# tomstrident/GAN-based-Video-Style-Transfer

Measured on AMD Instinct MI355X. Metric: frames/sec: CycleGAN train step (G+D+flow-warp loss) 256x256, higher is better.
Workload: dtype fp32; 1 GPU; C2: CycleGANCon optimize_parameters, resnet_9blocks G + basic PatchGAN D, ngf=ndf=64, 256x256, B_local=4, pool_size=50, flow-warp temporal loss; global_batch=4, height=256, width=256, parallelism=dp1

## Files before the change

gan-based-video-style-transfer_amd/csrc/common.h:

```cpp
#pragma once
#include <hip/hip_runtime.h>
#include <stdint.h>
#include <stdio.h>
#include <string.h>

#include "../../include/vst_hip.h"

typedef float f32x16 __attribute__((ext_vector_type(16)));
typedef float f32x4v __attribute__((ext_vector_type(4)));

namespace vst {

void set_error(const char* fmt, ...);

inline int check_launch(const char* what) {
  hipError_t e = hipGetLastError();
  if (e != hipSuccess) {
    set_error("%s: %s", what, hipGetErrorString(e));
    return VST_EHIP;
  }
  return VST_OK;
}

#define VST_NUM_CUS 256

#define VST_REQUIRE(cond, ...)            \
  do {                                    \
    if (!(cond)) {                        \
      ::vst::set_error(__VA_ARGS__);      \
      return VST_EINVAL;                  \
    }                                     \
  } while (0)

__device__ __forceinline__ int xcd_tile(int L, int T) {
  const int x = L & 7, k = L >> 3, q = T >> 3, r = T & 7;
  return x * q + (x < r ? x : r) + k;
}

__device__ __forceinline__ int reflect_idx(int i, int n) {
  i = i < 0 ? -i : i;
  return i >= n ? 2 * n - 2 - i : i;
}

__host__ __device__ __forceinline__ int dgrad_border_rows_of(int h, int w, int H, int W, int* b0) {
  const int sw = W - 2, sh = H - 2, S4 = ((2 * sw + 2 * sh + 3) / 4) * 4;
  const bool rh = h == 1 || h == H - 2, rw = w == 1 || w == W - 2;
  if (rh && rw) {
    *b0 = S4 + 4 * ((h == 1 ? 0 : 2) + (w == 1 ? 0 : 1));
    return 3;
  }
  const int kw = w == 0 ? 0 : (w == W - 1 ? sw - 1 : w - 1);
  const int kh = h == 0 ? 0 : (h == H - 1 ? sh - 1 : h - 1);
  if (h == 1) { *b0 = kw; return 1; }
  if (h == H - 2) { *b0 = sw + kw; return 1; }
  if (w == 1) { *b0 = 2 * sw + kh; return 1; }
  if (w == W - 2) { *b0 = 2 * sw + sh + kh; return 1; }
  return 0;
}

struct BorderSlabs {
  int ks, Mb, Lt, Ll;
};

__host__ __device__ __forceinline__ int dgrad_border_slab_rows(int n, int h, int w, int H, int W, int Lt, int Ll,
                                                               int* rows) {
  if (Ll == 0) {
    int b0;
    const int nr = dgrad_border_rows_of(h, w, H, W, &b0);
    for (int r = 0; r < nr; ++r) rows[r] = n * Lt + b0 + r;
    return nr;
  }
  int nr = 0;
  if (h == 1 || h == H - 2) {
    const int base = (h == 1 ? 0 : Lt) + n * (W + 2);
    rows[nr++] = base + w + 1;
    if (w == 1) rows[nr++] = base;
    if (w == W - 2) rows[nr++] = base + W + 1;
  }
  if (w == 1) rows[nr++] = 2 * Lt + n * H + h;
  if (w == W - 2) rows[nr++] = 2 * Lt + Ll + n * H + h;
  return nr;
}

__device__ __forceinline__ float apply_act(float v, int act, float slope) {
  if (act == VST_ACT_RELU) return v > 0.f ? v : 0.f;
  if (act == VST_ACT_LRELU) return v > 0.f ? v : v * slope;
  if (act == VST_ACT_TANH) return tanhf(v);
  return v;
}

__device__ __forceinline__ float act_grad_from_out(float y, int act, float slope) {
  if (act == VST_ACT_RELU) return y > 0.f ? 1.f : 0.f;
  if (act == VST_ACT_LRELU) return y > 0.f ? 1.f : slope;
  if (act == VST_ACT_TANH) return 1.f - y * y;
  return 1.f;
}

__device__ __forceinline__ float wave_sum(float v) {
#pragma unroll
  for (int o = 32; o > 0; o >>= 1) v += __shfl_xor(v, o, 64);
  return v;
}
__device__ __forceinline__ double wave_sum_d(double v) {
#pragma unroll
  for (int o = 32; o > 0; o >>= 1) v += __shfl_xor(v, o, 64);
  return v;
}

__device__ __forceinline__ void add_f4(float4& a, const float4& b) {
  a.x += b.x; a.y += b.y; a.z += b.z; a.w += b.w;
}

inline int ceil_div(long a, long b) { return (int)((a + b - 1) / b); }

int skinny_out_launch(int mode, const float* in, const float* wp, const float* bias,
                      const float* addend, float* out, int N, int Hi, int Wi, int Cin, int Ho,
                      int Wo, int R, int S, int st, int pad, int reflect, int act, float slope,
                      hipStream_t s, int co_real = 4);
void rk_fprop_launch(const float* x, const float* wp, const float* bias, float* y, int N, int H, int W,
                     int C, int Ho, int Wo, int Cop, int R, int S, int st, int padh, int padw, int reflect,
                     int act, float slope, int kind, int math, hipStream_t s);
long rk_cp_ld(long P);
bool bf_convT_phases_ok(int C, int Cop, int math);
int bf_convT_phases_launch(const float* x, const void* const ws[4], const float* bias, float* y, int N, int H, int W,
                           int C, int Cop, int act, float slope, int math, hipStream_t s, int full = 0);
int bf_fprop_launch(const float* x, const void* wsplit, long wps, const float* bias, float* y, int N,
                    int H, int W, int C, int Ho, int Wo, int Cop, int R, int S, int st, int padh, int padw,
                    int reflect, int act, float slope, int math, int kind, hipStream_t s,
                    double* part = nullptr, float* tws = nullptr, size_t tws_floats = 0, const float* addend = nullptr,
                    int oph = 0);
bool tap64_ok(int Cx, int R, int W, int math);
int tap64_launch(const float* x, const void* wsplit, long wps, const float* bias, float* y, int N, int H, int W,
                 int pad, int reflect, int act, float slope, int math, hipStream_t s);
bool c4_direct_ok(int C, int Cop, int R, int S, int st, int Ho, int Wo, int math);
int c4_direct_launch(const float* x, const void* wsplit, long wps, const float* bias, float* y, int N, int H, int W,
                     int Ho, int Wo, int R, int S, int pad, int reflect, int act, float slope, int math, double* part,
                     hipStream_t s);
bool bf_dgrad_refl1_ok(int N, int H, int W, int Cy, int Cx, int math);
size_t bf_dgrad_refl1_ws_floats(int N, int H, int W, int Cy, int Cx, int math);
size_t bf_dgrad_refl1_slabs(int N, int H, int W, int Cy, int Cx, int math, BorderSlabs* b);
int bf_dgrad_refl1_launch(const float* dy, const void* wsplit, long wps, const float* addend, float* dx, int N, int H,
                          int W, int Cy, int Cx, int math, hipStream_t s, float* ws, size_t ws_floats, bool add_border);
bool bf_dgrad_refl1_inb_ok(int N, int H, int W, int Cy, int Cx, int math);
int bf_dgrad_refl1_inb_slices(int H, int W);
int bf_dgrad_refl1_inb_launch(const float* dy, const void* wsplit, long wps, const float* addend, float* dx, int N,
                              int H, int W, int Cy, int Cx, int math, hipStream_t s, float* ws, size_t ws_floats,
                              const float* z, const float* st, double* part, int act, float slope,
                              const __bf16* apl = nullptr, long pps = 0);
size_t bf_fprop_ws_floats(long M, int Cop, int C, int R, int S, int math);
int bf_tail_ks(long M, int Cop, int m_split, int nk);
void bf_split_plan(long M, int Cop, int C, int R, int S, int math, int kind, int* m_first, int* ks_out);
void bf_plan(long M, int Cop, int math, int kind, int* kind_out, int* m_split_out, int* tail_out);
void bf_nhwc_to_planes(const float* x, void* y, long P, int Cs, int np, hipStream_t s, int row_in = 0,
                       int row_out = 0);
void bf_wgrad_launch(const float* xt, const void* dyp, float* slab, int N, int H, int W, int Cx, int Ho,
                     int Wo, int Cyp, int S, int pad, int st, int Mw, int chunk, int nsplit, int kind, int math,
                     hipStream_t s);
void bf_wgrad_geom(int kind, int math, int* bm, int* bn, int* bk, int* slots);
bool bf_wgrad_nhwc_ok(int kind, int Wo, int Cx, int Cyp);
void bf_wgrad_nhwc_launch(const float* x, const void* dy, long pps, bool bf32, float* slab, int N, int H, int W,
                          int Cx, int Ho, int Wo, int Cyp, int S, int pad, int st, int reflect, int Mw, int chunk,
                          int nsplit, int kind, hipStream_t s, float* dwd = nullptr, int dco = 0, int dacc = 0);

void rk_tile_geom(int kind, int math, int* bm, int* bn, int* bk, int* slots);
void rk_nhwc_to_cp(const float* x, float* y, long P, int Cs, int pack, hipStream_t s);
void rk_nhwc_to_cp_pad(const float* x, float* y, int N, int H, int W, int Cs, int pad, int reflect,
                       int phase, int pack, hipStream_t s, int extra = 0);
void rk_wgrad_launch(const float* xt, const float* dyt, float* slab, int N, int H, int W, int Cx,
                     int Ho, int Wo, int Cyp, int S, int pad, int st, int Mw, int chunk,
                     int nsplit, int kind, int math, hipStream_t s);
void rk_tconv_launch(const float* in, const float* wp, const float* bias, const float* addend,
                     float* out, int N, int Hi, int Wi, int Cy, int Ho, int Wo, int Cx, int R, int S,
                     int st, int pad, int reflect, int act, float slope, int kind, int math,
                     hipStream_t s);
extern const bool g_head;
bool head_ok(int Cin, int R, int S, int st, int reflect, int Wo);
int head_fwd_launch(const float* x, const float* wp, const float* bias, float* out, int N, int Hi, int Wi, int Cin,
                    int Ho, int Wo, int R, int S, int pad, int act, float slope, hipStream_t s);
size_t head_wgrad_ws_floats(int N, int Hi, int Cin, int R, int S);
bool head_tap_ok(int Cin);
size_t head_tap_ws_floats(int N, int Hi, int Wi);
int head_tap_fwd_launch(const float* x, const float* wp, const float* bias, float* out, float* ws, int N, int Hi,
                        int Wi, int Cin, int Ho, int Wo, int R, int S, int pad, int act, float slope, hipStream_t s);
int head_wgrad_launch(const float* x, const float* dy, float* dw, float* ws, int N, int Hi, int Wi, int Cin, int Ci,
                      int Ho, int Wo, int R, int S, int pad, long si, int accumulate, hipStream_t s,
                      float* db = nullptr);
extern const bool g_img_wgrad;
bool img_wgrad_ok(int Cx, int Cyp, int R, int S, int st, int reflect, int Ci, int Wo);
size_t img_wgrad_ws_floats(int N, int Ho, int Wo);
int img_wgrad_launch(const float* x, const float* dy, float* dw, float* db, float* ws, int N, int H, int W, int Ho,
                     int Wo, int Cyp, int R, int S, int st, int pad, int Co, int Ci, long so, long si, int accumulate,
                     hipStream_t s);
int head_dgrad_launch(const float* dy, const float* wp, const float* addend, float* dx, int N, int Hd, int Wd, int Cx,
                      int H, int W, int R, int S, int pad, hipStream_t s);
int skinny_wgrad_launch(const float* x, const float* dy, float* slab, int H, int W, int Cx, int Ho,
                        int Wo, int S, int st, int pad, int reflect, int Mw, int P, int chunk,
                        int nsplit, hipStream_t s);

}
```

gan-based-video-style-transfer_amd/csrc/conv_bf.hip:

```cpp
#include <type_traits>

#include "common.h"

#ifndef VST_BF_X6K3
#define VST_BF_X6K3 0
#endif
#ifndef VST_BF_MINB
#define VST_BF_MINB 1
#endif
#ifndef VST_BF_X6_256
#define VST_BF_X6_256 1
#endif
#ifndef VST_BF_KSLICE
#define VST_BF_KSLICE 1
#endif
#ifndef VST_BF_TAIL_KIND
#define VST_BF_TAIL_KIND 8
#endif
#ifndef VST_BF_TAIL
#define VST_BF_TAIL 1
#endif
#ifndef VST_BF_SCHED
#define VST_BF_SCHED 1
#endif
// ... 158 lines not shown
  }
}

template <class T>
__device__ __forceinline__ void mma_frag(const Frag<T>& f, f32x16 (&acc)[T::MI][T::NI]) {
#pragma unroll
  for (int i = 0; i < T::MI; ++i)
#pragma unroll
    for (int j = 0; j < T::NI; ++j) {
#if VST_BF_FAKE16
#define VST_MF(pA, pB)                                                                                   \
  {                                                                                                      \
    f32x4v q0 = {acc[i][j][0], acc[i][j][1], acc[i][j][2], acc[i][j][3]};                                 \
    f32x4v q1 = {acc[i][j][4], acc[i][j][5], acc[i][j][6], acc[i][j][7]};                                 \
    q0 = __builtin_amdgcn_mfma_f32_16x16x32_bf16(f.a[pA][i], f.b[pB][j], q0, 0, 0, 0);                  \
    q1 = __builtin_amdgcn_mfma_f32_16x16x32_bf16(f.b[pB][j], f.a[pA][i], q1, 0, 0, 0);                  \
    acc[i][j][0] = q0[0]; acc[i][j][1] = q0[1]; acc[i][j][2] = q0[2]; acc[i][j][3] = q0[3];              \
    acc[i][j][4] = q1[0]; acc[i][j][5] = q1[1]; acc[i][j][6] = q1[2]; acc[i][j][7] = q1[3];              \
  }
#else
#define VST_MF(pA, pB) acc[i][j] = __builtin_amdgcn_mfma_f32_32x32x16_bf16(f.a[pA][i], f.b[pB][j], acc[i][j], 0, 0, 0)
#endif
      if constexpr (T::NP == 3) {
        VST_MF(2, 0); VST_MF(0, 2); VST_MF(1, 1); VST_MF(1, 0); VST_MF(0, 1); VST_MF(0, 0);
      } else {
        VST_MF(1, 0); VST_MF(0, 1); VST_MF(0, 0);
      }
#undef VST_MF
    }
}

#ifndef VST_BF_GLDS_B
#define VST_BF_GLDS_B 1
#endif
template <class T>
__device__ __forceinline__ void store_stage(char* st, const float4 (&ra)[T::A_LD][2],
                                            const u32x4_t (&rbv)[T::B_LD][T::NP], int rb, int kq,
                                            bool with_b = true, bool with_a = true) {
  char* Bs = st + T::A_BYTES;
#pragma unroll
  for (int j = 0; j < T::A_LD; ++j) {
    if (!with_a) break;
    uint4 s[T::NP];
    split8<T::NP>(ra[j][0], ra[j][1], s);
    const int off = swz_off<T>(rb + T::RPP * j, kq);
#pragma unroll
    for (int p = 0; p < T::NP; ++p) *reinterpret_cast<uint4*>(st + p * T::A_PLANE + off) = s[p];
  }
  if (!with_b) return;
#pragma unroll
  for (int j = 0; j < T::B_LD; ++j) {
    const int off = swz_off<T>(rb + T::RPP * j, kq);
#pragma unroll
    for (int p = 0; p < T::NP; ++p) *reinterpret_cast<u32x4_t*>(Bs + p * T::B_PLANE + off) = rbv[j][p];
  }
}

template <class T>
__device__ __forceinline__ void sched_group(bool first, bool after_barrier) {
  constexpr int NM = T::MI * T::NI * (T::NP == 3 ? 6 : 3) * (VST_BF_FAKE16 ? 2 : 1);
  constexpr int NR = T::NP * (T::MI + T::NI);
  constexpr int NV = T::A_LD * 2 + T::B_LD * T::NP;
  constexpr int NW = T::A_LD * T::NP + T::B_LD * T::NP;
  if (first && !after_barrier) {
    if (VST_BF_SCHED < 2) return;
#pragma unroll
    for (int i = 0; i < NM; ++i) {
      __builtin_amdgcn_sched_group_barrier(0x008, 1, 0);
      if (i < NR) __builtin_amdgcn_sched_group_barrier(0x100, 1, 0);
      if (i < NV) __builtin_amdgcn_sched_group_barrier(0x020, 1, 0);
      __builtin_amdgcn_sched_group_barrier(0x002, 4, 0);
      if (i >= NM - NW - 1 && i < NM - 1) __builtin_amdgcn_sched_group_barrier(0x200, 1, 0);
    }
  } else {
#pragma unroll
    for (int i = 0; i < NM; ++i) {
      __builtin_amdgcn_sched_group_barrier(0x008, 1, 0);
      if (i < NR) __builtin_amdgcn_sched_group_barrier(0x100, 1, 0);
      __builtin_amdgcn_sched_group_barrier(0x002, 2, 0);
    }
  }
}

template <class T, class LoadAll, class Adv, class Prep>
__device__ __forceinline__ void main_loop(char* smem, int nk, f32x16 (&acc)[T::MI][T::NI],
                                          float4 (&ra)[2][T::A_LD][2], u32x4_t (&rbv)[2][T::B_LD][T::NP],
                                          int rb, int kq, LoadAll load_all, Adv adv, Prep prep) {
  constexpr int G = T::BK / 16;
  const int t = threadIdx.x, lane = t & 63, wave = t >> 6;
  const int wm0 = (wave / T::WAVES_N) * T::WM, wn0 = (wave % T::WAVES_N) * T::WN;
  if (nk <= 0) return;
  if (VST_BF_PRIO && wave >= T::NW / 2) __builtin_amdgcn_s_setprio(1);
  load_all(0);
  prep(0);
  store_stage<T>(smem, ra[0], rbv[0], rb, kq);
  adv(nk > 1);
  load_all(1);
  __syncthreads();
  Frag<T> fr[2];
  read_frag<T>(fr[0], smem, 0, wm0, wn0, lane);
  auto step = [&](int kt, auto par) __attribute__((always_inline)) {
    constexpr int P = decltype(par)::value;
    const char* cur = smem + P * T::STAGE;
    char* nxt = smem + (P ^ 1) * T::STAGE;
#pragma unroll
    for (int g = 0; g < G; ++g) {
      const int fi = (P * G + g) & 1;
      if (g + 1 < G) read_frag<T>(fr[fi ^ 1], cur, g + 1, wm0, wn0, lane);
      if (g == 0) {
        adv(kt + 2 < nk);
        load_all(P);
        if (!VST_BF_STORE_LATE) {
          prep(P ^ 1);
          store_stage<T>(nxt, ra[P ^ 1], rbv[P ^ 1], rb, kq);
        }
      }
      if (g == G - 1) {
        if (VST_BF_STORE_LATE) {
          prep(P ^ 1);
          store_stage<T>(nxt, ra[P ^ 1], rbv[P ^ 1], rb, kq);
        }
        __builtin_amdgcn_sched_barrier(0);
        __syncthreads();
        read_frag<T>(fr[fi ^ 1], nxt, 0, wm0, wn0, lane);
      }
      mma_frag<T>(fr[fi], acc);
      if (VST_BF_SCHED) sched_group<T>(g == 0, g == G - 1);
    }
  };
  int kt = 0;
  for (; kt + 1 < nk; kt += 2) {
    step(kt, std::integral_constant<int, 0>());
    step(kt + 1, std::integral_constant<int, 1>());
  }
  if (kt < nk) step(kt, std::integral_constant<int, 0>());
}

template <class T>
struct Plane16 {
  bf16x8_t a[T::MI16], b[T::NI16];
};

template <class T>
__device__ __forceinline__ void read_plane16(Plane16<T>& f, const char* __restrict__ st, int p, int wm0, int wn0,
                                             int lane) {
  const char* As = st + p * T::A_PLANE;
  const char* Bs = st + T::A_BYTES + p * T::B_PLANE;
  const int c = lane >> 4, li = lane & 15;
#pragma unroll
  for (int i = 0; i < T::MI16; ++i)
    f.a[i] = *reinterpret_cast<const bf16x8_t*>(As + swz_off<T>(wm0 + 16 * i + li, c));
#pragma unroll
  for (int j = 0; j < T::NI16; ++j)
    f.b[j] = *reinterpret_cast<const bf16x8_t*>(Bs + swz_off<T>(wn0 + 16 * j + li, c));
}

template <class T>
__device__ __forceinline__ void mma16(const Plane16<T>& A, const Plane16<T>& B, f32x4v (&acc)[T::MI16][T::NI16]) {
#pragma unroll
  for (int i = 0; i < T::MI16; ++i)
#pragma unroll
    for (int j = 0; j < T::NI16; ++j)
      acc[i][j] = __builtin_amdgcn_mfma_f32_16x16x32_bf16(A.a[i], B.b[j], acc[i][j], 0, 0, 0);
}

template <int NM, int NR, int NV, int NVALU, int NW>
__device__ __forceinline__ void sched16() {
#pragma unroll
  for (int i = 0; i < NM; ++i) {
    __builtin_amdgcn_sched_group_barrier(0x008, 1, 0);
    if (i < NR) __builtin_amdgcn_sched_group_barrier(0x100, 1, 0);
    if (i < NV) __builtin_amdgcn_sched_group_barrier(0x020, 1, 0);
    if (NVALU) __builtin_amdgcn_sched_group_barrier(0x002, NVALU, 0);
    if (i >= NM - NW - 1 && i < NM - 1) __builtin_amdgcn_sched_group_barrier(0x200, 1, 0);
  }
}

struct NoDma {
  static constexpr bool active = false, a_active = false;
  __device__ __forceinline__ void operator()(char*) const {}
};
template <class F, bool A = false>
struct DmaB {
  static constexpr bool active = true, a_active = A;
  F f;
  __device__ __forceinline__ void operator()(char* st) const { f(st); }
};
typedef __attribute__((address_space(3))) void lds_void;

template <class T, class LoadAll, class Adv, class Prep, class DmaB>
__device__ __forceinline__ void main_loop16(char* smem, int nk, f32x4v (&acc)[T::MI16][T::NI16],
                                            float4 (&ra)[2][T::A_LD][2], u32x4_t (&rbv)[2][T::B_LD][T::NP],
                                            int rb, int kq, LoadAll load_all, Adv adv, Prep prep, DmaB dmab) {
  const int t = threadIdx.x, lane = t & 63, wave = t >> 6;
  const int wm0 = (wave / T::WAVES_N) * T::WM, wn0 = (wave % T::WAVES_N) * T::WN;
  if (nk <= 0) return;
  constexpr int NM = T::MI16 * T::NI16, NR = T::MI16 + T::NI16;
  constexpr int NV = T::A_LD * 2 + T::B_LD * T::NP, NW = T::A_LD * T::NP + T::B_LD * T::NP;
  if (VST_M16_PRIO && wave >= T::NW / 2) __builtin_amdgcn_s_setprio(1);
  dmab(smem);
  load_all(0);
  prep(0);
  store_stage<T>(smem, ra[0], rbv[0], rb, kq, !dmab.active, !dmab.a_active);
  adv(nk > 1);
  load_all(1);
  __syncthreads();
  Plane16<T> hi, mid, lo;
  read_plane16<T>(mid, smem, 1, wm0, wn0, lane);
  auto step = [&](int kt, auto par) __attribute__((always_inline)) {
    constexpr int P = decltype(par)::value;
    const char* cur = smem + P * T::STAGE;
    char* nxt = smem + (P ^ 1) * T::STAGE;
    constexpr bool SA = VST_M16_STORE == 1, RA = VST_M16_RDLO == 1;
    dmab(nxt);
    if (VST_M16_LOADEARLY) {
      adv(kt + 2 < nk);
      load_all(P);
      __builtin_amdgcn_sched_barrier(0);
    }
    read_plane16<T>(hi, cur, 0, wm0, wn0, lane);
    if (RA) read_plane16<T>(lo, cur, 2, wm0, wn0, lane);
    if (!VST_M16_LOADEARLY) {
      adv(kt + 2 < nk);
      load_all(P);
    }
    if (SA) {
      prep(P ^ 1);
      store_stage<T>(nxt, ra[P ^ 1], rbv[P ^ 1], rb, kq, !dmab.active, !dmab.a_active);
    }
    mma16<T>(mid, mid, acc);
    if (VST_M16_SCHED) sched16<NM, RA ? 2 * NR : NR, NV, SA ? 4 : 0, SA ? NW : 0>();
    if (VST_M16_LOADFIRST) __builtin_amdgcn_sched_barrier(0);
    if (!RA) read_plane16<T>(lo, cur, 2, wm0, wn0, lane);
    if (!SA) {
      prep(P ^ 1);
      store_stage<T>(nxt, ra[P ^ 1], rbv[P ^ 1], rb, kq, !dmab.active, !dmab.a_active);
    }
    mma16<T>(mid, hi, acc);
    mma16<T>(hi, mid, acc);
    if (VST_M16_SCHED) sched16<2 * NM, RA ? 0 : NR, 0, SA ? 0 : 2, SA ? 0 : NW>();
    __builtin_amdgcn_sched_barrier(0);
    __syncthreads();
    read_plane16<T>(mid, nxt, 1, wm0, wn0, lane);
    mma16<T>(hi, hi, acc);
    mma16<T>(lo, hi, acc);
    mma16<T>(hi, lo, acc);
    if (VST_M16_SCHED) sched16<3 * NM, NR, 0, 0, 0>();
  };
  int kt = 0;
  for (; kt + 1 < nk; kt += 2) {
    step(kt, std::integral_constant<int, 0>());
    step(kt + 1, std::integral_constant<int, 1>());
  }
  if (kt < nk) step(kt, std::integral_constant<int, 0>());
}

template <int MI, int NI>
__device__ __forceinline__ void zero_acc4(f32x4v (&acc)[MI][NI]) {
#pragma unroll
  for (int i = 0; i < MI; ++i)
#pragma unroll
    for (int j = 0; j < NI; ++j) acc[i][j] = f32x4v{0.f, 0.f, 0.f, 0.f};
}

template <int MI, int NI>
__device__ __forceinline__ void zero_acc(f32x16 (&acc)[MI][NI]) {
#pragma unroll
  for (int i = 0; i < MI; ++i)
#pragma unroll
    for (int j = 0; j < NI; ++j)
#pragma unroll
      for (int r = 0; r < 16; ++r) acc[i][j][r] = 0.f;
}

__device__ __forceinline__ int remap_mtile(int bx, int nx) {
  if ((nx & 7) != 0) return bx;
  return (bx & 7) * (nx >> 3) + (bx >> 3);
}

__device__ __forceinline__ void tile_of(int L, int Mt, int Nt, int& mt, int& nt) {
  const int t = xcd_tile(L, Mt * Nt);
  mt = t / Nt;
  nt = t - mt * Nt;
}

struct InbArgs {
  const float* z;
  const float* st;
  double* part;
  int act;
  float slope;
  int ns;
};

__device__ __forceinline__ void inb_term(float g, float z, float mean, float rstd, int act, float slope, float& gd,
                                         float& xh) {
  xh = (z - mean) * rstd;
  float d = 1.f;
  if (act == VST_ACT_RELU) d = xh > 0.f ? 1.f : 0.f;
  else if (act == VST_ACT_LRELU) d = xh > 0.f ? 1.f : slope;
  gd = g * d;
}

__host__ __device__ __forceinline__ int dgrad_border_rows(int H, int W) {
  return ((2 * (W - 2) + 2 * (H - 2) + 3) / 4) * 4 + 16;
}

__host__ __device__ __forceinline__ void dgrad_border_pos(int b, int H, int W, int& qh, int& qw, int& th, int& tw) {
  const int sw = W - 2, sh = H - 2, S = 2 * sw + 2 * sh, S4 = (S + 3) / 4 * 4;
  qh = qw = th = tw = -100;
  if (b < 2 * sw) {
    const int k = b < sw ? b : b - sw;
    tw = k == 0 ? 0 : (k == sw - 1 ? W - 1 : k + 1);
    qw = tw;
    qh = b < sw ? -1 : H;
    th = b < sw ? 1 : H - 2;
    return;
  }
  if (b < S) {
    const int b2 = b - 2 * sw, k = b2 < sh ? b2 : b2 - sh;
    th = k == 0 ? 0 : (k == sh - 1 ? H - 1 : k + 1);
    qh = th;
    qw = b2 < sh ? -1 : W;
    tw = b2 < sh ? 1 : W - 2;
    return;
  }
  if (b < S4) return;
  const int g = (b - S4) >> 2, r = (b - S4) & 3;
  if (r == 3) return;
  const int top = g < 2, left = (g & 1) == 0;
  th = top ? 1 : H - 2;
  tw = left ? 1 : W - 2;
  const int ph = top ? -1 : H, pw = left ? -1 : W;
  if (r == 0) { qh = ph; qw = tw; }
  else if (r == 1) { qh = ph; qw = pw; }
  else { qh = th; qw = pw; }
}

__global__ __launch_bounds__(256) void dgrad_border_add_k(const float* __restrict__ slab, int ks, int Mb, int C,
                                                          float* __restrict__ dx, int H, int W, int NB) {
  const int t = threadIdx.x;
  const int c = blockIdx.y * 64 + (t & 15) * 4;
  const int m = blockIdx.x * 16 + (t >> 4);
  if (m >= Mb || c >= C) return;
  const int n = m / NB, b = m - n * NB;
  int qh, qw, th, tw;
  dgrad_border_pos(b, H, W, qh, qw, th, tw);
  if (th < 0) return;
  const int S4 = NB - 16;
  if (b >= S4 && ((b - S4) & 3) != 0) return;
  const int nr = b >= S4 ? 3 : 1;
  const long zst = (long)Mb * C;
  float4 v = make_float4(0.f, 0.f, 0.f, 0.f);
  for (int r = 0; r < nr; ++r) {
    const float* base = slab + (long)(m + r) * C + c;
    float4 u[16];
#pragma unroll
    for (int z = 0; z < 16; ++z)
      if (z < ks) u[z] = *reinterpret_cast<const float4*>(base + z * zst);
    float4 acc = make_float4(0.f, 0.f, 0.f, 0.f);
#pragma unroll
    for (int z = 0; z < 16; ++z)
      if (z < ks) add_f4(acc, u[z]);
    add_f4(v, acc);
  }
  float4* d = reinterpret_cast<float4*>(dx + (((long)n * H + th) * W + tw) * C + c);
  float4 o = *d;
  add_f4(o, v);
  *d = o;
}

__host__ __device__ __forceinline__ int border5_seg_rows(int n_img, int len, int bm) {
  return (n_img * len + bm - 1) / bm * bm;
}

__global__ __launch_bounds__(256) void dgrad_border5_add_k(const float* __restrict__ slab, int ks, int Mb, int C,
                                                           float* __restrict__ dx, int N, int H, int W, int Lt,
                                                           int Ll) {
  const int t = threadIdx.x;
  const int c = blockIdx.y * 64 + (t & 15) * 4;
  const int T = 2 * W + 2 * H;
  const int m = blockIdx.x * 16 + (t >> 4);
  if (m >= N * T || c >= C) return;
  const int n = m / T, b = m - n * T;
  int th, tw;
  if (b < 2 * W) {
    th = b < W ? 1 : H - 2;
    tw = b < W ? b : b - W;
  } else {
    const int b2 = b - 2 * W;
    th = b2 < H ? b2 : b2 - H;
    tw = b2 < H ? 1 : W - 2;
    if (th == 1 || th == H - 2) return;
  }
  int rows[3];
  const int nr = dgrad_border_slab_rows(n, th, tw, H, W, Lt, Ll, rows);
  const long zst = (long)Mb * C;
  float4 v = make_float4(0.f, 0.f, 0.f, 0.f);
  for (int r = 0; r < nr; ++r) {
    const float* base = slab + (long)rows[r] * C + c;
    float4 u[16];
#pragma unroll
    for (int z = 0; z < 16; ++z)
      if (z < ks) u[z] = *reinterpret_cast<const float4*>(base + z * zst);
    float4 acc = make_float4(0.f, 0.f, 0.f, 0.f);
#pragma unroll
    for (int z = 0; z < 16; ++z)
      if (z < ks) add_f4(acc, u[z]);
    add_f4(v, acc);
  }
  float4* d = reinterpret_cast<float4*>(dx + (((long)n * H + th) * W + tw) * C + c);
  float4 o = *d;
  add_f4(o, v);
  *d = o;
}

__device__ __forceinline__ void border5_target(int b, int W, int H, int& th, int& tw, bool& live) {
  live = true;
  if (b < 2 * W) {
    th = b < W ? 1 : H - 2;
    tw = b < W ? b : b - W;
  } else {
    const int b2 = b - 2 * W;
    th = b2 < H ? b2 : b2 - H;
    tw = b2 < H ? 1 : W - 2;
    if (th == 1 || th == H - 2) live = false;
  }
}

__global__ __launch_bounds__(256) void dgrad_border5_add_inb_k(const float* __restrict__ slab, int ks, int Mb, int C,
                                                               float* __restrict__ dx, int H, int W, int Lt, int Ll,
                                                               InbArgs inb, int first_slice) {
  __shared__ double red[2][16][65];
  const int t = threadIdx.x, c4 = (t & 15) * 4, sub = t >> 4;
  const int c = blockIdx.z * 64 + c4, n = blockIdx.y;
  const int T = 2 * W + 2 * H;
  const int b = blockIdx.x * 16 + sub;
  double a0[4] = {0, 0, 0, 0}, a1[4] = {0, 0, 0, 0};
  int th = 0, tw = 0;
  bool live = false;
  if (b < T && c < C) border5_target(b, W, H, th, tw, live);
  if (live) {
    int rows[3];
    const int nr = dgrad_border_slab_rows(n, th, tw, H, W, Lt, Ll, rows);
    const long zst = (long)Mb * C;
    float4 v = make_float4(0.f, 0.f, 0.f, 0.f);
    for (int r = 0; r < nr; ++r) {
      const float* base = slab + (long)rows[r] * C + c;
      float4 u[16];
#pragma unroll
      for (int z = 0; z < 16; ++z)
        if (z < ks) u[z] = *reinterpret_cast<const float4*>(base + z * zst);
      float4 acc = make_float4(0.f, 0.f, 0.f, 0.f);
#pragma unroll
      for (int z = 0; z < 16; ++z)
        if (z < ks) add_f4(acc, u[z]);
      add_f4(v, acc);
    }
    const long e = (((long)n * H + th) * W + tw) * C + c;
    float4* d = reinterpret_cast<float4*>(dx + e);
    const float4 o0 = *d;
    float4 o = o0;
    add_f4(o, v);
    *d = o;
    const float4 zz = *reinterpret_cast<const float4*>(inb.z + e);
    const float4 s0 = reinterpret_cast<const float4*>(inb.st)[((long)n * C + c) / 2];
    const float4 s1 = reinterpret_cast<const float4*>(inb.st)[((long)n * C + c) / 2 + 1];
    const float mu[4] = {s0.x, s0.z, s1.x, s1.z}, rs[4] = {s0.y, s0.w, s1.y, s1.w};
    const float g0[4] = {o0.x, o0.y, o0.z, o0.w}, g1[4] = {o.x, o.y, o.z, o.w}, zv[4] = {zz.x, zz.y, zz.z, zz.w};
#pragma unroll
    for (int k = 0; k < 4; ++k) {
      float d0, d1, xh;
      inb_term(g0[k], zv[k], mu[k], rs[k], inb.act, inb.slope, d0, xh);
      inb_term(g1[k], zv[k], mu[k], rs[k], inb.act, inb.slope, d1, xh);
      a0[k] = (double)d1 - (double)d0;
      a1[k] = (double)d1 * xh - (double)d0 * xh;
    }
  }
#pragma unroll
  for (int k = 0; k < 4; ++k) {
    red[0][sub][c4 + k] = a0[k];
    red[1][sub][c4 + k] = a1[k];
  }
  __syncthreads();
  if (t < 192) {
    const int v = t >> 6, cc = t & 63, nn = blockIdx.z * 64 + cc;
    if (nn >= C) return;
    double acc = 0.0;
    if (v < 2)
      for (int q = 0; q < 16; ++q) acc += red[v][q][cc];
    inb.part[(((long)n * inb.ns + first_slice + blockIdx.x) * C + nn) * 3 + v] = acc;
  }
}

__device__ __forceinline__ int phase_row(int mm, int oph, int Ho, int Wo) {
  const bool full = oph > 4;
  const int q = full ? oph - 5 : oph - 1, a = q >> 1, b = q & 1;
  const int hw = Ho * Wo, n = mm / hw, rem = mm - n * hw, ph = rem / Wo, pw = rem - ph * Wo;
  const int H = full ? Ho - 1 : Ho - a, W = full ? Wo - 1 : Wo - b;
  const int i = ph - a, j = pw - b;
  if (i < 0 || j < 0 || i >= H || j >= W) return -1;
  return (n * 2 * H + 2 * i + a) * 2 * W + 2 * j + b;
}

__device__ __attribute__((aligned(256))) float g_zero_page[64];

template <class T, bool KSL, int REFL, bool SPLIT, bool APRE = false>
__device__ __forceinline__ void conv_fprop_bf_body(
    int bid, const float* __restrict__ x, const __bf16* __restrict__ ws, long wps, const float* __restrict__ bias,
    float* __restrict__ y, int H, int W, int C, int Ho, int Wo, int Cop, int S, int st, int padh,
    int padw, int reflect, int act, float slope, int M, int Ktot, int m_base, double* __restrict__ part,
    int spk, float* __restrict__ slab, const float* __restrict__ addend, int oph,
    InbArgs inb = InbArgs{}, const __bf16* __restrict__ apl = nullptr, long pps = 0) {
  static_assert(!SPLIT || KSL, "split-K needs the channel-slice-major K walk");
  static_assert(REFL < 4 || (SPLIT && KSL), "border rows run as split-K slabs");
  __shared__ __attribute__((aligned(16))) char smem[2 * T::STAGE];
  constexpr int A_LD = T::A_LD, B_LD = T::B_LD, RPP = T::RPP, NP = T::NP;
  const int t = threadIdx.x, lane = t & 63, wave = t >> 6;
  int mt_, nt_;
  const int Mt_ = (M - m_base + T::BM - 1) / T::BM, Nt_ = (Cop + T::BN - 1) / T::BN;
  const int zs = SPLIT ? bid / (Mt_ * Nt_) : 0;
  tile_of(SPLIT ? bid - zs * Mt_ * Nt_ : bid, Mt_, Nt_, mt_, nt_);
  const int m0 = m_base + mt_ * T::BM, n0 = nt_ * T::BN;
  const int kq = t % T::KC, rb = t / T::KC;
  const float* zp = g_zero_page;

  constexpr bool C4 = REFL == 3;
  const int seg = REFL != 5 ? 0 : (m0 < Ho ? 0 : (m0 < 2 * Ho ? 1 : (m0 < 2 * Ho + Wo ? 2 : 3)));
  const int Sx = REFL != 5 ? S : (seg < 2 ? 3 : 1);
  int hb[A_LD], wb[A_LD], pb[A_LD], aoff[A_LD], aoff2[C4 ? A_LD : 1];
#pragma unroll
  for (int j = 0; j < A_LD; ++j) {
    const int m = m0 + rb + RPP * j;
    const int mm = m < M ? m : 0;
    if constexpr (REFL == 5) {
      const int L = seg < 2 ? W + 2 : H;
      const int r = mm - (seg == 0 ? 0 : (seg == 1 ? Ho : (seg == 2 ? 2 * Ho : 2 * Ho + Wo)));
      const int n = r / L, k = r - n * L;
      const bool live = (unsigned)r < (unsigned)(st * L);
      hb[j] = !live ? -1000000 : (seg == 0 ? 0 : (seg == 1 ? H - 1 : k - 1));
      wb[j] = seg < 2 ? k - 2 : (seg == 2 ? 0 : W - 1);
      pb[j] = live ? n * H * W * C : 0;
      continue;
    }
    if constexpr (REFL == 4) {
      const int n = mm / Wo;
      int qh, qw, th, tw;
      dgrad_border_pos(mm - n * Wo, H, W, qh, qw, th, tw);
      hb[j] = qh - padh;
      wb[j] = qw - padw;
      pb[j] = n * H * W * C;
      continue;
    }
    const int hw = Ho * Wo;
    const int n = mm / hw, rem = mm - n * hw, ho = rem / Wo, wo = rem - ho * Wo;
    hb[j] = ho * st - padh;
    wb[j] = wo * st - padw;
    pb[j] = n * H * W * C;
  }
  const bool refl = REFL >= 2 ? reflect != 0 : REFL == 1;
  const int WC = W * C;
  auto tap_rows_to = [&](int* dst, int kr, int ks) __attribute__((always_inline)) {
#pragma unroll
    for (int j = 0; j < A_LD; ++j) {
      int hi = hb[j] + kr, wi = wb[j] + ks;
      if (refl) {
        hi = reflect_idx(hi, H);
        wi = reflect_idx(wi, W);
        dst[j] = pb[j] + __mul24(hi, WC) + __mul24(wi, C);
      } else {
        const bool ok = (unsigned)hi < (unsigned)H && (unsigned)wi < (unsigned)W;
        dst[j] = ok ? pb[j] + __mul24(hi, WC) + __mul24(wi, C) : -1;
      }
    }
  };
  auto tap_rows = [&](int kr, int ks) __attribute__((always_inline)) {
    tap_rows_to(aoff, kr, ks);
    if constexpr (C4) {
      const bool wrap = ks + 1 == S;
      tap_rows_to(aoff2, wrap ? kr + 1 : kr, wrap ? 0 : ks + 1);
    }
  };
  const __bf16* wrow[B_LD];
#pragma unroll
  for (int j = 0; j < B_LD; ++j) {
    const int n = n0 + rb + RPP * j;
    wrow[j] = ws + (long)(n < Cop ? n : Cop - 1) * (REFL == 5 ? 3 * Ktot : Ktot);
  }

  const int kq8 = 8 * kq;
  int tr = 0, ts = 0, ksb = 0;
  int kcur = kq8, kc = kq8 % C, kr = 0, ks = 0;
  const int Rk = KSL ? Ktot / (Sx * C) : 0;
  const int nk_all = (Ktot + T::BK - 1) / T::BK;
  int k0 = 0, nk = nk_all;
  if (SPLIT) {
    k0 = zs * spk;
    nk = min(spk, nk_all - k0);
    const int taps = Rk * Sx, tap = k0 % taps;
    tr = tap / Sx;
    ts = tap - tr * Sx;
    ksb = (k0 / taps) * T::BK;
  }
  if (KSL) {
    tap_rows(tr, ts);
  } else {
    const int rs = kq8 / C;
    kr = rs / S;
    ks = rs - kr * S;
    tap_rows(kr, ks);
  }

  float4 ra[2][A_LD][2];
  u32x4_t rbv[2][B_LD][NP];
  constexpr bool GLDS = VST_BF_GLDS_B && T::M16 && KSL && !C4 && REFL != 5;
  constexpr bool GLDS_A = (APRE || VST_BF_FAKE_ADMA) && GLDS;
  constexpr bool APRE_REG = APRE && !GLDS_A;
  static_assert(!APRE || GLDS_A || REFL == 5, "pre-split A: the x6 M16 channel-slice kernels with LDS-DMA B, or REFL 5");
  const __bf16* apl_ = VST_BF_FAKE_ADMA ? reinterpret_cast<const __bf16*>(x) : apl;
  const long pps_ = VST_BF_FAKE_ADMA ? (long)(M / (Ho * Wo)) * H * W * C / 2 : pps;
  auto load_all = [&](int set) __attribute__((always_inline)) {
    const bool kin = KSL || kcur < Ktot;
    const int ka = KSL ? ksb + kq8 : kc;
    const int tap5 = seg == 0 ? 6 + ts : (seg == 1 ? ts : 3 * tr + (seg == 2 ? 2 : 0));
    const int kb = KSL ? (REFL == 5 ? tap5 : tr * S + ts) * C + ksb + kq8 : (kin ? kcur : 0);
    if constexpr (C4) {
      const bool kin2 = kcur + 4 < Ktot;
#pragma unroll
      for (int j = 0; j < A_LD; ++j) {
        const float* p0 = (kin && aoff[j] >= 0) ? x + aoff[j] : zp;
        const float* p1 = (kin2 && aoff2[j] >= 0) ? x + aoff2[j] : zp;
        ra[set][j][0] = *reinterpret_cast<const float4*>(p0);
        ra[set][j][1] = *reinterpret_cast<const float4*>(p1);
      }
      const __bf16* zb = reinterpret_cast<const __bf16*>(zp);
#pragma unroll
      for (int j = 0; j < B_LD; ++j) {
#pragma unroll
        for (int p = 0; p < NP; ++p) {
          const __bf16* q = wrow[j] + p * wps + kb;
          const uint2 lo = *reinterpret_cast<const uint2*>(q);
          const uint2 hi = *reinterpret_cast<const uint2*>(kin2 ? q + 4 : zb);
          rbv[set][j][p] = u32x4_t{lo.x, lo.y, hi.x, hi.y};
        }
      }
      return;
    }
#pragma unroll
    for (int j = 0; j < A_LD; ++j) {
      if constexpr (GLDS_A) break;
      const bool tap0 = KSL && tr == 0 && ts == 0;
      const bool fake = VST_BF_FAKE_ZA == 1 || (VST_BF_FAKE_ZA == 2 && !tap0) || (VST_BF_FAKE_ZA == 3 && tap0);
      if constexpr (APRE_REG) {
        const bool live = kin && aoff[j] >= 0;
        const __bf16* q = live ? apl + aoff[j] + ka : reinterpret_cast<const __bf16*>(zp);
        const long ps = live ? pps : 0;
        const u32x4_t h = *reinterpret_cast<const u32x4_t*>(q), m = *reinterpret_cast<const u32x4_t*>(q + ps),
                      l = *reinterpret_cast<const u32x4_t*>(q + 2 * ps);
        float v[8];
#pragma unroll
        for (int e = 0; e < 4; ++e) {
          v[2 * e] = (__uint_as_float(h[e] << 16) + __uint_as_float(m[e] << 16)) + __uint_as_float(l[e] << 16);
          v[2 * e + 1] = (__uint_as_float(h[e] & 0xffff0000u) + __uint_as_float(m[e] & 0xffff0000u)) +
                         __uint_as_float(l[e] & 0xffff0000u);
        }
        ra[set][j][0] = make_float4(v[0], v[1], v[2], v[3]);
        ra[set][j][1] = make_float4(v[4], v[5], v[6], v[7]);
        continue;
      }
      const float* p = (kin && aoff[j] >= 0 && !fake) ? x + (VST_BF_FAKE_ZA == 4 ? 0 : aoff[j]) + ka : zp;
      ra[set][j][0] = *reinterpret_cast<const float4*>(p);
      ra[set][j][1] = *reinterpret_cast<const float4*>(p + 4);
    }
    if constexpr (GLDS) return;
#pragma unroll
    for (int j = 0; j < B_LD; ++j) {
#pragma unroll
      for (int p = 0; p < NP; ++p)
        rbv[set][j][p] = *reinterpret_cast<const u32x4_t*>(
            VST_BF_FAKE_ZB == 1 ? reinterpret_cast<const __bf16*>(zp)
                                : (VST_BF_FAKE_ZB == 2 ? ws : wrow[j]) + p * wps + kb);
    }
  };
  auto dma_b = [&](char* st) __attribute__((always_inline)) {
    if constexpr (GLDS_A) {
      const __bf16* zb = reinterpret_cast<const __bf16*>(zp);
#pragma unroll
      for (int j = 0; j < A_LD; ++j) {
        const int row = rb + RPP * j;
        const int csrc = (t % T::KC) ^ T::swz(row);
        const int wrow0 = __builtin_amdgcn_readfirstlane(row - (lane / T::KC));
        const bool live = aoff[j] >= 0;
        const __bf16* src = live ? apl_ + aoff[j] + ksb + 8 * csrc : zb + 8 * csrc;
#pragma unroll
        for (int p = 0; p < NP; ++p) {
#if defined(__HIP_DEVICE_COMPILE__)
          __builtin_amdgcn_global_load_lds(src + (live ? p * pps_ : 0), (lds_void*)(st + p * T::A_PLANE + wrow0 * T::ROWB),
                                           16, 0, 0);
#endif
        }
      }
    }
    const int kbase = (tr * S + ts) * C + ksb;
#pragma unroll
    for (int j = 0; j < B_LD; ++j) {
      const int row = rb + RPP * j;
      const int csrc = (t % T::KC) ^ T::swz(row);
      const int wrow0 = __builtin_amdgcn_readfirstlane(row - (lane / T::KC));
#pragma unroll
      for (int p = 0; p < NP; ++p) {
#if defined(__HIP_DEVICE_COMPILE__)
        __builtin_amdgcn_global_load_lds(wrow[j] + p * wps + kbase + 8 * csrc,
                                         (lds_void*)(st + T::A_BYTES + p * T::B_PLANE + wrow0 * T::ROWB), 16, 0, 0);
#endif
      }
    }
  };
  auto adv = [&](bool go) __attribute__((always_inline)) {
    if (KSL) {
      const int ts1 = ts + 1;
      const bool w1 = ts1 == Sx;
      const int tr1 = tr + (w1 ? 1 : 0);
      const bool w2 = w1 && tr1 == Rk;
      ts = go ? (w1 ? 0 : ts1) : ts;
      tr = go ? (w2 ? 0 : tr1) : tr;
      ksb = go ? ksb + (w2 ? T::BK : 0) : ksb;
      tap_rows(tr, ts);
      return;
    }
    if (!go) return;
    kcur += T::BK;
    kc += T::BK;
    if (kc >= C) {
      do {
        kc -= C;
        if (++ks == S) { ks = 0; ++kr; }
      } while (kc >= C);
      tap_rows(kr, ks);
    }
  };

  auto prep = [](int) __attribute__((always_inline)) {};
  const int wm0 = (wave / T::WAVES_N) * T::WM, wn0 = (wave % T::WAVES_N) * T::WN;
  if constexpr (T::M16) {
    f32x4v acc[T::MI16][T::NI16];
    zero_acc4(acc);
    if constexpr (GLDS)
      main_loop16<T>(smem, nk, acc, ra, rbv, rb, kq, load_all, adv, prep, DmaB<decltype(dma_b), GLDS_A>{dma_b});
    else
      main_loop16<T>(smem, nk, acc, ra, rbv, rb, kq, load_all, adv, prep, NoDma{});
    if constexpr (SPLIT) {
      float* sl = slab + (long)zs * (M - m_base) * Cop;
#pragma unroll
      for (int i = 0; i < T::MI16; ++i)
#pragma unroll
        for (int j = 0; j < T::NI16; ++j) {
          const int n = n0 + wn0 + 16 * j + (lane & 15);
#pragma unroll
          for (int r = 0; r < 4; ++r) {
            const int mm = m0 + wm0 + 16 * i + 4 * (lane >> 4) + r;
            if (n < Cop && mm < M) sl[(long)(mm - m_base) * Cop + n] = acc[i][j][r];
          }
        }
      return;
    }
    constexpr bool LFIT = T::BM * (T::BN + 16) * 4 <= 2 * T::STAGE;
    const bool LEPI = LFIT && (VST_BF_LDS_EPI || addend != nullptr || oph != 0 || inb.part != nullptr);
    constexpr int LDE = T::BN + 16;
    float* ept = reinterpret_cast<float*>(smem);
    constexpr int IC4 = T::BN / 4, IRW = 64 / (IC4 > 0 ? IC4 : 1);
    constexpr bool IOK = LFIT && 64 % IC4 == 0 && T::BM == 32 * T::NW && IC4 >= 4;
    float4 izr[IOK ? 32 / IRW : 1], iar[IOK ? 32 / IRW : 1];
    if constexpr (IOK) {
      if (inb.part) {
        const int n = n0 + 4 * (lane % IC4);
#pragma unroll
        for (int k = 0; k < 32 / IRW; ++k) {
          const int mm = m0 + 32 * wave + lane / IC4 + IRW * k;
          const bool ok = n < Cop && mm < M;
          izr[k] = ok ? *reinterpret_cast<const float4*>(inb.z + (long)mm * Cop + n) : make_float4(0.f, 0.f, 0.f, 0.f);
          iar[k] = (ok && addend) ? *reinterpret_cast<const float4*>(addend + (long)mm * Cop + n)
                                  : make_float4(0.f, 0.f, 0.f, 0.f);
        }
      }
    }
    if (LEPI) __syncthreads();
#pragma unroll
    for (int g = 0; g < T::MI16 / 2; ++g)
#pragma unroll
      for (int j = 0; j < T::NI16; ++j) {
        const int n = n0 + wn0 + 16 * j + (lane & 15);
        const bool nok = n < Cop;
        const float bv = (bias && nok) ? bias[n] : 0.f;
        double s1 = 0.0, s2 = 0.0;
#pragma unroll
        for (int h = 0; h < 2; ++h)
#pragma unroll
          for (int r = 0; r < 4; ++r) {
            const int mm = m0 + wm0 + 16 * (2 * g + h) + 4 * (lane >> 4) + r;
            const float ad = (!LEPI && addend && nok && mm < M) ? addend[(long)mm * Cop + n] : 0.f;
            const float v = apply_act(acc[2 * g + h][j][r] + bv, act, slope) + ad;
            if (LEPI)
              ept[(mm - m0) * LDE + (n - n0)] = v;
            else if (nok && mm < M && (!oph || phase_row(mm, oph, Ho, Wo) >= 0))
              y[(long)(oph ? phase_row(mm, oph, Ho, Wo) : mm) * Cop + n] = v;
            s1 += v;
            s2 += (double)v * v;
          }
        if (part) {
          s1 += __shfl_xor(s1, 16);
          s2 += __shfl_xor(s2, 16);
          s1 += __shfl_xor(s1, 32);
          s2 += __shfl_xor(s2, 32);
          const int g0 = m0 + wm0 + 32 * g;
          if (lane < 16 && nok && g0 < M) {
            const int hw = Ho * Wo, img = g0 / hw, z = (g0 - img * hw) >> 5;
            double* d = part + (((long)img * (hw >> 5) + z) * Cop + n) * 2;
            d[0] = s1;
            d[1] = s2;
          }
        }
      }
    if (LEPI) {
      __syncthreads();
      constexpr int C4 = T::BN / 4;
      if constexpr (IOK) {
        if (inb.part) {
          constexpr int RW = IRW;
          const int c = 4 * (lane % C4), n = n0 + c, hw = Ho * Wo;
          const int gm0 = m0 + 32 * wave;
          if (gm0 < M) {
            const int img = gm0 / hw;
            float4 s0 = make_float4(0.f, 0.f, 0.f, 0.f), s1 = s0;
            if (n < Cop) {
              s0 = reinterpret_cast<const float4*>(inb.st)[((long)img * Cop + n) / 2];
              s1 = reinterpret_cast<const float4*>(inb.st)[((long)img * Cop + n) / 2 + 1];
            }
            const float mu[4] = {s0.x, s0.z, s1.x, s1.z}, rs[4] = {s0.y, s0.w, s1.y, s1.w};
            double a0[4] = {0, 0, 0, 0}, a1[4] = {0, 0, 0, 0}, a2[4] = {0, 0, 0, 0};
#pragma unroll
            for (int k = 0; k < 32 / RW; ++k) {
              const int row = 32 * wave + lane / C4 + RW * k, mm = m0 + row;
              if (n < Cop && mm < M) {
                float4 v = *reinterpret_cast<const float4*>(ept + row * LDE + c);
                add_f4(v, iar[k]);
                *reinterpret_cast<float4*>(y + (long)mm * Cop + n) = v;
                const float gv[4] = {v.x, v.y, v.z, v.w}, zv[4] = {izr[k].x, izr[k].y, izr[k].z, izr[k].w};
#pragma unroll
                for (int e = 0; e < 4; ++e) {
                  float gd, xh;
                  inb_term(gv[e], zv[e], mu[e], rs[e], inb.act, inb.slope, gd, xh);
                  a0[e] += gd;
                  a1[e] += (double)gd * xh;
                  a2[e] += xh;
                }
              }
            }
#pragma unroll
            for (int off = C4; off < 64; off <<= 1)
#pragma unroll
              for (int e = 0; e < 4; ++e) {
                a0[e] += __shfl_xor(a0[e], off);
                a1[e] += __shfl_xor(a1[e], off);
                a2[e] += __shfl_xor(a2[e], off);
              }
            if (lane < C4 && n < Cop) {
              double* d = inb.part + (((long)img * inb.ns + ((gm0 - img * hw) >> 5)) * Cop + n) * 3;
#pragma unroll
              for (int e = 0; e < 4; ++e) {
                d[3 * e] = a0[e];
                d[3 * e + 1] = a1[e];
                d[3 * e + 2] = a2[e];
              }
            }
          }
          return;
        }
      }
#pragma unroll 4
      for (int idx = t; idx < T::BM * C4; idx += T::NT) {
        const int row = idx / C4, c = 4 * (idx - row * C4);
        const int mm = m0 + row, n = n0 + c;
        const int orow = oph ? phase_row(mm, oph, Ho, Wo) : mm;
        if (mm < M && n < Cop && orow >= 0) {
          float4 v = *reinterpret_cast<const float4*>(ept + row * LDE + c);
          if (addend) add_f4(v, *reinterpret_cast<const float4*>(addend + (long)mm * Cop + n));
          *reinterpret_cast<float4*>(y + (long)orow * Cop + n) = v;
        }
      }
    }
    return;
  }
  f32x16 acc[T::MI][T::NI];
  zero_acc(acc);
  main_loop<T>(smem, nk, acc, ra, rbv, rb, kq, load_all, adv, prep);
  if constexpr (SPLIT) {
    float* sl = slab + (long)zs * (M - m_base) * Cop;
#pragma unroll
    for (int i = 0; i < T::MI; ++i)
#pragma unroll
      for (int j = 0; j < T::NI; ++j) {
        const int n = n0 + wn0 + 32 * j + (lane & 31);
#pragma unroll
        for (int r = 0; r < 16; ++r) {
          const int mm = m0 + wm0 + 32 * i + (r & 3) + 8 * (r >> 2) + 4 * (lane >> 5);
          if (n < Cop && mm < M) sl[(long)(mm - m_base) * Cop + n] = acc[i][j][r];
        }
      }
    return;
  }

#pragma unroll
  for (int i = 0; i < T::MI; ++i)
#pragma unroll
    for (int j = 0; j < T::NI; ++j) {
      const int n = n0 + wn0 + 32 * j + (lane & 31);
      const bool nok = n < Cop;
      const float bv = (bias && nok) ? bias[n] : 0.f;
      double s1 = 0.0, s2 = 0.0;
#pragma unroll
      for (int r = 0; r < 16; ++r) {
        const int mm = m0 + wm0 + 32 * i + (r & 3) + 8 * (r >> 2) + 4 * (lane >> 5);
        const float ad = (addend && nok && mm < M) ? addend[(long)mm * Cop + n] : 0.f;
        const float v = apply_act(acc[i][j][r] + bv, act, slope) + ad;
        if (nok && mm < M && (!oph || phase_row(mm, oph, Ho, Wo) >= 0))
          y[(long)(oph ? phase_row(mm, oph, Ho, Wo) : mm) * Cop + n] = v;
        s1 += v;
        s2 += (double)v * v;
      }
      if (part) {
        s1 += __shfl_xor(s1, 32);
        s2 += __shfl_xor(s2, 32);
        const int g0 = m0 + wm0 + 32 * i;
        if (lane < 32 && nok && g0 < M) {
          const int hw = Ho * Wo, img = g0 / hw, z = (g0 - img * hw) >> 5;
          double* d = part + (((long)img * (hw >> 5) + z) * Cop + n) * 2;
          d[0] = s1;
          d[1] = s2;
        }
      }
    }
}

template <class T, bool KSL, int REFL, bool SPLIT = false, bool APRE = false>
__global__ __launch_bounds__(T::NT, T::MINB) void conv_fprop_bf_k(
    const float* __restrict__ x, const __bf16* __restrict__ ws, long wps, const float* __restrict__ bias,
    float* __restrict__ y, int H, int W, int C, int Ho, int Wo, int Cop, int S, int st, int padh,
    int padw, int reflect, int act, float slope, int M, int Ktot, int m_base, double* __restrict__ part,
    int spk = 0, float* __restrict__ slab = nullptr, const float* __restrict__ addend = nullptr, int oph = 0,
    const __bf16* __restrict__ apl = nullptr, long pps = 0) {
  conv_fprop_bf_body<T, KSL, REFL, SPLIT, APRE>(blockIdx.x, x, ws, wps, bias, y, H, W, C, Ho, Wo, Cop, S, st, padh,
                                                padw, reflect, act, slope, M, Ktot, m_base, part, spk, slab, addend, oph,
                                                InbArgs{}, apl, pps);
}

template <class T, bool APRE = false>
__global__ __launch_bounds__(T::NT, T::MINB) void conv_fprop_bf_inb_k(
    const float* __restrict__ x, const __bf16* __restrict__ ws, long wps, float* __restrict__ y, int H, int W, int C,
    int Cop, const float* __restrict__ addend, int M, int Ktot, InbArgs inb, const __bf16* __restrict__ apl = nullptr,
    long pps = 0) {
  conv_fprop_bf_body<T, true, 0, false, APRE>(blockIdx.x, x, ws, wps, nullptr, y, H, W, C, H, W, Cop, 3, 1, 1, 1, 0,
                                              VST_ACT_NONE, 0.f, M, Ktot, 0, nullptr, 0, nullptr, addend, 0, inb, apl, pps);
}

struct PhaseJobs {
  const __bf16* ws[4];
  int t0[5];
};

template <class T>
__global__ __launch_bounds__(T::NT, T::MINB) void conv_convT_phases_k(const float* __restrict__ x, PhaseJobs jobs,
                                                                      const float* __restrict__ bias,
                                                                      float* __restrict__ y, int N, int H, int W,
                                                                      int C, int Cop, int act, float slope,
                                                                      int full) {
  const int bid = blockIdx.x;
  const int j = bid < jobs.t0[1] ? 0 : (bid < jobs.t0[2] ? 1 : (bid < jobs.t0[3] ? 2 : 3));
  const int ph = j == 0 ? 3 : (j == 1 ? 1 : (j == 2 ? 2 : 0));
  const int a = ph >> 1, b = ph & 1;
  const int t0 = j == 0 ? jobs.t0[0] : (j == 1 ? jobs.t0[1] : (j == 2 ? jobs.t0[2] : jobs.t0[3]));
  const __bf16* ws = j == 0 ? jobs.ws[0] : (j == 1 ? jobs.ws[1] : (j == 2 ? jobs.ws[2] : jobs.ws[3]));
  const int R = full ? 2 : 1 + a, S = full ? 2 : 1 + b, pah = full ? 1 : a, paw = full ? 1 : b;
  const int Ho = H + (full ? 1 : a), Wo = W + (full ? 1 : b), M = N * Ho * Wo, K = R * S * C;
  const int tiles = (M + T::BM - 1) / T::BM * ((Cop + T::BN - 1) / T::BN);
  if (bid - t0 >= tiles) return;
  conv_fprop_bf_body<T, true, 0, false>(bid - t0, x, ws, (long)Cop * K, bias, y, H, W, C, Ho, Wo, Cop, S, 1, pah,
                                        paw, 0, act, slope, M, K, 0, nullptr, 0, nullptr, nullptr,
                                        (full ? 5 : 1) + 2 * a + b);
}

template <class T, bool W1>
__global__ __launch_bounds__(T::NT, T::MINB) void conv_wgrad_bf_k(
    const float* __restrict__ xt, const __bf16* __restrict__ dyp, long dps, float* __restrict__ slab, int H,
    int W, int Cx, int Ho, int Wo, int Cyp, int S, int pad, int st, int Mw, int P, int chunk, long ldx,
    long ldy) {
  __shared__ __attribute__((aligned(16))) char smem[2 * T::STAGE];
  constexpr int A_LD = T::A_LD, B_LD = T::B_LD, RPP = T::RPP, NP = T::NP;
  typedef float f4u __attribute__((ext_vector_type(4), aligned(4)));
  const int t = threadIdx.x, lane = t & 63, wave = t >> 6;
  const int Mt = (Mw + T::BM - 1) / T::BM, Nt = (Cyp + T::BN - 1) / T::BN, Zt = (P + chunk - 1) / chunk;
  int mx, ny, zz;
  {
    const int tt = xcd_tile(blockIdx.x, Mt * Nt * Zt);
    zz = tt / (Mt * Nt);
    const int rem = tt - zz * Mt * Nt;
    ny = rem / Mt;
    mx = rem - ny * Mt;
  }
  const int m0 = mx * T::BM, n0 = ny * T::BN;
  const int pbeg = zz * chunk, pend = min(P, pbeg + chunk);
  const int kq = t % T::KC, rb = t / T::KC;
  const float* zp = g_zero_page;
  const __bf16* zpb = reinterpret_cast<const __bf16*>(g_zero_page);
  const int Hp = H + 2 * pad, Wp = W + 2 * pad;
  const float* xrow[A_LD];
#pragma unroll
  for (int j = 0; j < A_LD; ++j) {
    const int m = m0 + rb + RPP * j;
    const int mm = m < Mw ? m : Mw - 1;
    const int tap = mm / Cx, ci = mm - tap * Cx;
    const int r = tap / S, s_ = tap - r * S;
    xrow[j] = xt + (long)ci * ldx + r * Wp + (st == 1 ? s_ : (s_ & 1) * (Wp >> 1) + (s_ >> 1));
  }
  const __bf16* drow[B_LD];
#pragma unroll
  for (int j = 0; j < B_LD; ++j) {
    const int n = n0 + rb + RPP * j;
    drow[j] = dyp + (long)(n < Cyp ? n : Cyp - 1) * ldy;
  }
  int kp = pbeg + 8 * kq, pho, pwo;
  long poff;
  {
    const int hw = Ho * Wo;
    const int pn = kp / hw;
    const int rem = kp - pn * hw;
    pho = rem / Wo;
    pwo = rem - pho * Wo;
    poff = ((long)pn * Hp + st * pho) * Wp + pwo;
  }
  float4 ra[2][A_LD][2];
  u32x4_t rbv[2][B_LD][NP];
  auto load_all = [&](int set) __attribute__((always_inline)) {
    const bool live = kp < pend;
#pragma unroll
    for (int j = 0; j < A_LD; ++j) {
      const float* p = live ? xrow[j] + poff : zp;
      const f4u u0 = *reinterpret_cast<const f4u*>(p);
      const f4u u1 = *reinterpret_cast<const f4u*>(p + 4);
      ra[set][j][0] = make_float4(u0.x, u0.y, u0.z, u0.w);
      ra[set][j][1] = make_float4(u1.x, u1.y, u1.z, u1.w);
    }
#pragma unroll
    for (int j = 0; j < B_LD; ++j) {
      const __bf16* q = live ? drow[j] + kp : zpb;
      const long ps = live ? dps : 0;
#pragma unroll
      for (int p = 0; p < NP; ++p) rbv[set][j][p] = *reinterpret_cast<const u32x4_t*>(q + p * ps);
    }
  };
  const long row_step = (long)st * Wp - Wo, img_step = (long)(Hp - st * Ho) * Wp;
  auto adv = [&](bool go) __attribute__((always_inline)) {
    if (W1 && VST_WG_SELECT) {
      const int pw1 = pwo + T::BK;
      const bool e1 = pw1 >= Wo;
      const int ph1 = pho + (e1 ? 1 : 0);
      const bool e2 = ph1 == Ho;
      const long po1 = poff + T::BK + (e1 ? row_step : 0) + (e2 ? img_step : 0);
      kp = go ? kp + T::BK : kp;
      pwo = go ? (e1 ? pw1 - Wo : pw1) : pwo;
      pho = go ? (e2 ? 0 : ph1) : pho;
      poff = go ? po1 : poff;
      return;
    }
    if (!go) return;
    kp += T::BK;
    pwo += T::BK;
    poff += T::BK;
    while (pwo >= Wo) {
      pwo -= Wo;
      poff += st * Wp - Wo;
      if (++pho == Ho) { pho = 0; poff += (long)(Hp - st * Ho) * Wp; }
    }
  };
  const int nk = pend > pbeg ? (pend - pbeg + T::BK - 1) / T::BK : 0;
  const int wm0 = (wave / T::WAVES_N) * T::WM, wn0 = (wave % T::WAVES_N) * T::WN;
  float* sl = slab + (long)zz * Mw * Cyp;
  if constexpr (T::M16) {
    f32x4v acc[T::MI16][T::NI16];
    zero_acc4(acc);
    main_loop16<T>(smem, nk, acc, ra, rbv, rb, kq, load_all, adv, [](int) {}, NoDma{});
#pragma unroll
    for (int i = 0; i < T::MI16; ++i)
#pragma unroll
      for (int j = 0; j < T::NI16; ++j) {
        const int n = n0 + wn0 + 16 * j + (lane & 15);
        if (n >= Cyp) continue;
#pragma unroll
        for (int r = 0; r < 4; ++r) {
          const int mm = m0 + wm0 + 16 * i + 4 * (lane >> 4) + r;
          if (mm < Mw) sl[(long)mm * Cyp + n] = acc[i][j][r];
        }
      }
    return;
  }
  f32x16 acc[T::MI][T::NI];
  zero_acc(acc);
  main_loop<T>(smem, nk, acc, ra, rbv, rb, kq, load_all, adv, [](int) {});

#pragma unroll
  for (int i = 0; i < T::MI; ++i)
#pragma unroll
    for (int j = 0; j < T::NI; ++j) {
      const int n = n0 + wn0 + 32 * j + (lane & 31);
      if (n >= Cyp) continue;
#pragma unroll
      for (int r = 0; r < 16; ++r) {
        const int mm = m0 + wm0 + 32 * i + (r & 3) + 8 * (r >> 2) + 4 * (lane >> 5);
        if (mm < Mw) sl[(long)mm * Cyp + n] = acc[i][j][r];
      }
    }
}

constexpr int KM_PITCH = 272, KM_GROUP = 32 * KM_PITCH;
__device__ __forceinline__ int km_off(int grp, int row, int col) { return grp * KM_GROUP + KM_PITCH * row + 2 * col; }
template <class T>
struct KmGeom {
  static constexpr int A_PLANE = (T::BM / 128) * KM_GROUP, B_PLANE = (T::BN / 128) * KM_GROUP;
  static constexpr int A_BYTES = T::NP * A_PLANE, STAGE = T::NP * (A_PLANE + B_PLANE);
  static_assert(2 * STAGE <= 160 * 1024, "LDS");
};

template <class T>
__device__ __forceinline__ void store_stage_km(char* st, const float4 (&ra)[T::A_LD][2],
                                               const u32x4_t (&rbv)[T::B_LD][T::NP], int t) {
  using G = KmGeom<T>;
  char* Bs = st + G::A_BYTES;
  constexpr int AC = T::BM / 8, BC = T::BN / 8;
#pragma unroll
  for (int j = 0; j < T::A_LD; ++j) {
    const int c = t + T::NT * j, k = c / AC, mc = c % AC;
    uint4 sp[T::NP];
    split8<T::NP>(ra[j][0], ra[j][1], sp);
    const int off = km_off(mc >> 4, k, 8 * (mc & 15));
#pragma unroll
    for (int p = 0; p < T::NP; ++p) *reinterpret_cast<uint4*>(st + p * G::A_PLANE + off) = sp[p];
  }
#pragma unroll
  for (int j = 0; j < T::B_LD; ++j) {
    const int c = t + T::NT * j, k = c / BC, nc = c % BC;
    const int off = km_off(nc >> 4, k, 8 * (nc & 15));
#pragma unroll
    for (int p = 0; p < T::NP; ++p) *reinterpret_cast<u32x4_t*>(Bs + p * G::B_PLANE + off) = rbv[j][p];
  }
}

template <class T>
__device__ __forceinline__ void store_stage_km(char* st, const float4 (&ra)[T::A_LD][2],
                                               const float4 (&rbf)[T::B_LD][2], int t) {
  using G = KmGeom<T>;
  char* Bs = st + G::A_BYTES;
  constexpr int AC = T::BM / 8, BC = T::BN / 8;
#pragma unroll
  for (int j = 0; j < T::A_LD; ++j) {
    const int c = t + T::NT * j, k = c / AC, mc = c % AC;
    uint4 sp[T::NP];
    split8<T::NP>(ra[j][0], ra[j][1], sp);
    const int off = km_off(mc >> 4, k, 8 * (mc & 15));
#pragma unroll
    for (int p = 0; p < T::NP; ++p) *reinterpret_cast<uint4*>(st + p * G::A_PLANE + off) = sp[p];
  }
#pragma unroll
  for (int j = 0; j < T::B_LD; ++j) {
    const int c = t + T::NT * j, k = c / BC, nc = c % BC;
    uint4 sp[T::NP];
    split8<T::NP>(rbf[j][0], rbf[j][1], sp);
    const int off = km_off(nc >> 4, k, 8 * (nc & 15));
#pragma unroll
    for (int p = 0; p < T::NP; ++p) *reinterpret_cast<uint4*>(Bs + p * G::B_PLANE + off) = sp[p];
  }
}

typedef __bf16 bf16x4_t __attribute__((ext_vector_type(4)));
typedef __attribute__((address_space(3))) bf16x4_t lds_bf16x4;

__device__ __forceinline__ bf16x8_t read_km16(const char* __restrict__ img, int cb, int lane) {
  const int g = lane >> 4, q = (lane >> 2) & 3, pp = lane & 3;
  const char* a0 = img + km_off(cb >> 7, 8 * g + q, (cb & 127) + 4 * pp);
  const char* a1 = a0 + 4 * KM_PITCH;
  bf16x4_t lo = {}, hi = {};
#if defined(__HIP_DEVICE_COMPILE__)
  lo = __builtin_amdgcn_ds_read_tr16_b64_v4bf16((lds_bf16x4*)(a0));
  hi = __builtin_amdgcn_ds_read_tr16_b64_v4bf16((lds_bf16x4*)(a1));
#endif
  return __builtin_shufflevector(lo, hi, 0, 1, 2, 3, 4, 5, 6, 7);
}

template <class T>
__device__ __forceinline__ void read_plane16_km(Plane16<T>& f, const char* __restrict__ st, int p, int wm0, int wn0,
                                                int lane) {
  using G = KmGeom<T>;
  const char* As = st + p * G::A_PLANE;
  const char* Bs = st + G::A_BYTES + p * G::B_PLANE;
#pragma unroll
  for (int i = 0; i < T::MI16; ++i) f.a[i] = read_km16(As, wm0 + 16 * i, lane);
#pragma unroll
  for (int j = 0; j < T::NI16; ++j) f.b[j] = read_km16(Bs, wn0 + 16 * j, lane);
}

template <class T, class RB, class LoadAll, class Adv>
__device__ __forceinline__ void main_loop16_km(char* smem, int nk, f32x4v (&acc)[T::MI16][T::NI16],
                                               float4 (&ra)[2][T::A_LD][2], RB (&rbv)[2], LoadAll load_all,
                                               Adv adv) {
  constexpr int STAGE = KmGeom<T>::STAGE;
  const int t = threadIdx.x, lane = t & 63, wave = t >> 6;
  const int wm0 = (wave / T::WAVES_N) * T::WM, wn0 = (wave % T::WAVES_N) * T::WN;
  if (nk <= 0) return;
  load_all(0);
  store_stage_km<T>(smem, ra[0], rbv[0], t);
  adv(nk > 1);
  load_all(1);
  __syncthreads();
  Plane16<T> hi, mid, lo;
  read_plane16_km<T>(mid, smem, 1, wm0, wn0, lane);
  auto step = [&](int kt, auto par) __attribute__((always_inline)) {
    constexpr int P = decltype(par)::value;
    const char* cur = smem + P * STAGE;
    char* nxt = smem + (P ^ 1) * STAGE;
    read_plane16_km<T>(hi, cur, 0, wm0, wn0, lane);
    adv(kt + 2 < nk);
    load_all(P);
    mma16<T>(mid, mid, acc);
    read_plane16_km<T>(lo, cur, 2, wm0, wn0, lane);
    store_stage_km<T>(nxt, ra[P ^ 1], rbv[P ^ 1], t);
    mma16<T>(mid, hi, acc);
    mma16<T>(hi, mid, acc);
    __builtin_amdgcn_sched_barrier(0);
    __syncthreads();
    read_plane16_km<T>(mid, nxt, 1, wm0, wn0, lane);
    mma16<T>(hi, hi, acc);
    mma16<T>(lo, hi, acc);
    mma16<T>(hi, lo, acc);
  };
  int kt = 0;
  for (; kt + 1 < nk; kt += 2) {
    step(kt, std::integral_constant<int, 0>());
    step(kt + 1, std::integral_constant<int, 1>());
  }
  if (kt < nk) step(kt, std::integral_constant<int, 0>());
}

template <class T, bool BF32>
__global__ __launch_bounds__(T::NT, T::MINB) void conv_wgrad_nhwc_k(
    const float* __restrict__ x, const void* __restrict__ dyv, long pps, float* __restrict__ slab, int H, int W,
    int Cx, int Ho, int Wo, int Cyp, int S, int pad, int st, int reflect, int Mw, int P, int chunk,
    float* __restrict__ dwd, int dco, int dacc) {
  static_assert(T::M16 && T::BK == 32 && T::BM % 128 == 0 && T::BN % 128 == 0, "k-major images of 128 columns");
  static_assert((T::NT % (T::BM / 8)) == 0 && (T::NT % (T::BN / 8)) == 0, "a thread's chunk column is fixed");
  __shared__ __attribute__((aligned(16))) char smem[2 * KmGeom<T>::STAGE];
  constexpr int A_LD = T::A_LD, B_LD = T::B_LD, NP = T::NP, AC = T::BM / 8, BC = T::BN / 8;
  const int t = threadIdx.x, lane = t & 63, wave = t >> 6;
  const int Mt = (Mw + T::BM - 1) / T::BM, Nt = (Cyp + T::BN - 1) / T::BN, Zt = (P + chunk - 1) / chunk;
  int mx, ny, zz;
  {
    const int tt = xcd_tile(blockIdx.x, Mt * Nt * Zt);
    zz = tt / (Mt * Nt);
// ... 160 lines not shown
  __syncthreads();
  if (t < 192) {
    const int v = t >> 6, c = t & 63, nn = blockIdx.y * 64 + c;
    if (nn >= Cop) return;
    double acc = 0.0;
    for (int q = 0; q < 16; ++q) acc += red[v][q][c];
    inb.part[(((long)img * inb.ns + ((g0 - img * hw) >> 5)) * Cop + nn) * 3 + v] = acc;
  }
}

__global__ __launch_bounds__(256) void fprop_splitk_reduce_k(const float* __restrict__ slab, int ks, int m_base, int M,
                                                             int Cop, const float* __restrict__ bias, int act,
                                                             float slope, float* __restrict__ y,
                                                             double* __restrict__ part, int hw,
                                                             const float* __restrict__ addend = nullptr) {
  __shared__ double red[2][16][65];
  const int t = threadIdx.x, c4 = (t & 15) * 4, sub = t >> 4;
  const int n = blockIdx.y * 64 + c4;
  const long rows = M - m_base, zst = rows * Cop;
  const int r0 = blockIdx.x * 32;
  double s1[4] = {0, 0, 0, 0}, s2[4] = {0, 0, 0, 0};
  if (n < Cop) {
    const float4 bv = bias ? make_float4(bias[n], bias[n + 1], bias[n + 2], bias[n + 3]) : make_float4(0.f, 0.f, 0.f, 0.f);
#pragma unroll
    for (int h = 0; h < 2; ++h) {
      const long r = r0 + sub + 16 * h;
      if (r >= rows) break;
      float4 v = bv;
      for (int z0 = 0; z0 < ks; z0 += 8) {
        float4 q[8];
#pragma unroll
        for (int u = 0; u < 8; ++u)
          q[u] = z0 + u < ks ? *reinterpret_cast<const float4*>(slab + (z0 + u) * zst + r * Cop + n)
                             : make_float4(0.f, 0.f, 0.f, 0.f);
#pragma unroll
        for (int u = 0; u < 8; ++u) {
          if (z0 + u >= ks) break;
          add_f4(v, q[u]);
        }
      }
      float o[4] = {apply_act(v.x, act, slope), apply_act(v.y, act, slope), apply_act(v.z, act, slope),
                    apply_act(v.w, act, slope)};
      if (addend) {
        const float4 a = *reinterpret_cast<const float4*>(addend + (m_base + r) * Cop + n);
        o[0] += a.x;
        o[1] += a.y;
        o[2] += a.z;
        o[3] += a.w;
      }
      *reinterpret_cast<float4*>(y + (m_base + r) * Cop + n) = make_float4(o[0], o[1], o[2], o[3]);
#pragma unroll
      for (int e = 0; e < 4; ++e) {
        s1[e] += o[e];
        s2[e] += (double)o[e] * o[e];
      }
    }
  }
  if (!part) return;
#pragma unroll
  for (int e = 0; e < 4; ++e) {
    red[0][sub][c4 + e] = s1[e];
    red[1][sub][c4 + e] = s2[e];
  }
  __syncthreads();
  if (t < 128) {
    const int v = t >> 6, c = t & 63, nn = blockIdx.y * 64 + c;
    if (nn >= Cop) return;
    double acc = 0.0;
    for (int q = 0; q < 16; ++q) acc += red[v][q][c];
    const int g0 = m_base + r0, img = g0 / hw, zg = (g0 - img * hw) >> 5;
    part[(((long)img * (hw >> 5) + zg) * Cop + nn) * 2 + v] = acc;
  }
}

template <int NP>
__global__ __launch_bounds__(256) void nhwc_to_cp_planes_k(const float* __restrict__ x, __bf16* __restrict__ y,
                                                           long P, int Cs, long ld, int rin, int rout) {
  __shared__ float tile[64][65];
  const long p0 = (long)blockIdx.x * 64;
  const int c0 = blockIdx.y * 64;
  const int t = threadIdx.x;
#pragma unroll
  for (int it = 0; it < 4; ++it) {
    const int idx = t + 256 * it, pr = idx >> 4, c4 = (idx & 15) * 4;
    float4 v = make_float4(0.f, 0.f, 0.f, 0.f);
    long q = p0 + pr;
    bool ok = q < P && c0 + c4 < Cs;
    if (rout > 0) {
      const long row = q / rout;
      const int col = (int)(q - row * rout);
      ok = ok && col < rin;
      q = row * rin + col;
    }
    if (ok) v = *reinterpret_cast<const float4*>(x + q * Cs + c0 + c4);
    tile[pr][c4] = v.x;
    tile[pr][c4 + 1] = v.y;
    tile[pr][c4 + 2] = v.z;
    tile[pr][c4 + 3] = v.w;
  }
  __syncthreads();
  const long plane = (long)Cs * ld;
#pragma unroll
  for (int it = 0; it < 4; ++it) {
    const int idx = t + 256 * it, cr = idx >> 4, p4 = (idx & 15) * 4;
    if (c0 + cr >= Cs || p0 + p4 >= P) continue;
    float r[4] = {tile[p4][cr], tile[p4 + 1][cr], tile[p4 + 2][cr], tile[p4 + 3][cr]};
    __bf16* dst = y + (long)(c0 + cr) * ld + p0 + p4;
#pragma unroll
    for (int p = 0; p < NP; ++p) {
      const uint32_t q0 = pack2(r[0], r[1]), q1 = pack2(r[2], r[3]);
      if (p0 + p4 + 3 < P) {
        *reinterpret_cast<uint2*>(dst + p * plane) = make_uint2(q0, q1);
      } else {
        const uint16_t h[4] = {(uint16_t)q0, (uint16_t)(q0 >> 16), (uint16_t)q1, (uint16_t)(q1 >> 16)};
        for (int e = 0; e < 4 && p0 + p4 + e < P; ++e)
          reinterpret_cast<uint16_t*>(dst + p * plane)[e] = h[e];
      }
      if (p + 1 < NP) {
        r[0] -= __uint_as_float(q0 << 16);
        r[1] -= __uint_as_float(q0 & 0xffff0000u);
        r[2] -= __uint_as_float(q1 << 16);
        r[3] -= __uint_as_float(q1 & 0xffff0000u);
      }
    }
  }
}

__global__ void split3_k(const float* __restrict__ w, __bf16* __restrict__ out, long n) {
  const long i = (long)blockIdx.x * blockDim.x + threadIdx.x;
  if (i >= n) return;
  const float v = w[i];
  const __bf16 h = (__bf16)v;
  const float r = v - (float)h;
  const __bf16 m = (__bf16)r;
  out[i] = h;
  out[n + i] = m;
  out[2 * n + i] = (__bf16)(r - (float)m);
}

}

#define VST_BF_DISPATCH(kind, np, L)                                   \
  switch (kind) {                                                      \
    case 1: L(128, 64, 64, 32, 32, np) break;                          \
    case 2: L(128, 128, 64, 64, 32, np) break;                         \
    case 3: L(64, 128, 32, 64, 32, np) break;                          \
    case 4: L(128, 128, 64, 32, (np == 3 ? 32 : 64), np) break;        \
    case 5: L(128, 64, 64, 32, 64, np) break;                          \
    case 6: L(64, 64, 32, 32, 32, np) break;                           \
    case 7: L(256, 128, 64, 64, 32, np) break;                         \
    case 8: L(64, 64, 32, 32, (np == 3 ? 32 : 64), np) break;          \
    case 9: L(128, 128, 64, 64, 16, np) break;                         \
    case 10: L(256, 64, 64, 64, 32, np) break;                         \
    default: L(128, 128, 64, 32, 32, np) break;                        \
  }

int bf_pick(long M, int Nc, int override_kind) {
  if (override_kind >= 0 && override_kind <= 9) return override_kind;
  if (Nc <= 64) return M / 128 >= 256 ? 1 : 6;
  const long n128 = (Nc + 127) / 128;
  if ((M / 128) * n128 >= 200) return 0;
  if ((M / 64) * n128 >= 200) return 3;
  return 6;
}

static void bf_geom(int kind, int np, int* bm, int* bn, int* slots) {
  int BM = 128, BN = 128, BK = 32;
  switch (kind) {
    case 1: BN = 64; break;
    case 2: break;
    case 3: BM = 64; break;
    case 4: BK = np == 3 ? 32 : 64; break;
    case 5: BN = 64; BK = 64; break;
    case 6: BM = 64; BN = 64; break;
    case 7: BM = 256; break;
    case 8: BM = 64; BN = 64; BK = np == 3 ? 32 : 64; break;
    case 9: BK = 16; break;
    case 10: BM = 256; BN = 64; break;
    default: break;
  }
  const int stage = np * (BM + BN) * BK * 2;
  int sl = (160 * 1024) / (2 * stage);
  const int waves = (kind == 0 || kind == 4 || kind == 7) ? 8 : 4;
  if (sl * waves > 32) sl = 32 / waves;
  *bm = BM;
  *bn = BN;
  *slots = sl < 1 ? 1 : sl;
}

void bf_plan(long M, int Cop, int math, int kind, int* kind_out, int* m_split_out, int* tail_out) {
  int kd = bf_pick(M, Cop, kind);
  int m_split = 0, tail_kind = VST_BF_TAIL_KIND;
#if VST_BF_X6_256
  if (kind < 0 && kd == 0 && math == VST_MATH_BF16X6) {
    const long nt = (Cop + 127) / 128;
    const long b256 = (long)((M + 255) / 256) * nt;
    if (b256 % VST_NUM_CUS == 0 || b256 >= 4 * VST_NUM_CUS) {
      kd = 7;
    } else if (b256 > VST_NUM_CUS && (VST_NUM_CUS % nt) == 0) {
      const long ms = (long)(b256 / VST_NUM_CUS) * (VST_NUM_CUS / nt) * 256;
      const long rest = M - ms;
      static const int cand[4] = {8, 3, 1, 0};
      static const double eff[4] = {0.6, 0.75, 0.75, 0.85};
      double best = (double)((b256 + VST_NUM_CUS - 1) / VST_NUM_CUS);
      int bk = -1;
      for (int c = 0; c < 4; ++c) {
        int bm, bn, sl;
        bf_geom(cand[c], 3, &bm, &bn, &sl);
        const long blocks = ((rest + bm - 1) / bm) * ((Cop + bn - 1) / bn);
        const long rounds = (blocks + (long)sl * VST_NUM_CUS - 1) / ((long)sl * VST_NUM_CUS);
        const double cost = (double)(ms / 256 * nt) / VST_NUM_CUS + rounds * (bm * bn) / (256.0 * 128.0) / eff[c];
        if (cost < best - 1e-9) { best = cost; bk = cand[c]; }
      }
      if (VST_BF_TAIL_FORCE >= 0) bk = VST_BF_TAIL_FORCE;
      kd = 7;
      if (bk >= 0) {
        m_split = (int)ms;
        tail_kind = bk;
      }
    } else if (b256 < VST_NUM_CUS && b256 > VST_BF_FULLSPLIT_MAX) {
      const long r128 = ((M + 127) / 128 * nt + VST_NUM_CUS - 1) / VST_NUM_CUS;
      if (2.25 < 1.5 * r128) kd = 7;
    }
  }
#endif
#if VST_BF_TAIL
  if (kind < 0 && kd == 0 && math != VST_MATH_BF16X6) {
    const long nt = (Cop + 127) / 128, blocks = (long)((M + 127) / 128) * nt;
    const long per = blocks / VST_NUM_CUS, tail = blocks - per * VST_NUM_CUS;
    if (per >= 1 && tail > 0 && 4 * tail <= VST_NUM_CUS && (per * VST_NUM_CUS) % nt == 0) {
      m_split = (int)(per * VST_NUM_CUS / nt) * 128;
      tail_kind = VST_BF_TAIL_KIND;
    }
  }
#endif
  *kind_out = kd;
  *m_split_out = m_split;
  *tail_out = m_split ? tail_kind : -1;
}

int bf_tail_ks(long M, int Cop, int m_split, int nk) {
  const long rest = M - m_split;
  if (m_split <= 0 || rest <= 0) return 0;
  const long Tt = ((rest + 255) / 256) * ((Cop + 127) / 128);
  double best = 1e30;
  int bk = 0;
  for (int ks = 2; ks <= 16; ++ks) {
    const int steps = (nk + ks - 1) / ks;
    if ((long)(ks - 1) * steps >= nk) continue;
    const long rounds = (Tt * ks + VST_NUM_CUS - 1) / VST_NUM_CUS;
    const double us = rounds * (steps * 2.25 + 4.0) + (double)(ks + 1) * rest * Cop * 4.0 / 4.0e6 + 3.0;
    if (us < best) {
      best = us;
      bk = ks;
    }
  }
  return bk;
}

void bf_split_plan(long M, int Cop, int C, int R, int S, int math, int kind, int* m_first, int* ks_out) {
  *m_first = 0;
  *ks_out = 0;
  if (math != VST_MATH_BF16X6 || !VST_BF_KSLICE || C % 32 || !VST_BF_SPLITK || kind >= 0) return;
  const int nk = (R * S * C + 31) / 32;
  int kd, m_split, tail_kind;
  bf_plan(M, Cop, math, -1, &kd, &m_split, &tail_kind);
  if (kd == 7 && m_split) {
    *m_first = m_split;
    *ks_out = bf_tail_ks(M, Cop, m_split, nk);
    return;
  }
  const long b256 = ((M + 255) / 256) * ((Cop + 127) / 128);
  if (kd == 7 || b256 > VST_BF_FULLSPLIT_MAX) return;
  int bm, bn, sl;
  bf_geom(kd, 3, &bm, &bn, &sl);
  const long blocks = ((M + bm - 1) / bm) * ((Cop + bn - 1) / bn);
  const long rounds_small = (blocks + (long)sl * VST_NUM_CUS - 1) / ((long)sl * VST_NUM_CUS);
  const double t_small = (kd == 0 || kd == 2 || kd == 4 || kd == 9) ? 1.5 : (kd == 3 ? 1.8 : 1.2);
  const double small_us = rounds_small * nk * t_small + 3.0;
  double best = 0.85 * small_us;
  int bk = 0;
  for (int ks = 2; ks <= 32; ++ks) {
    const int steps = (nk + ks - 1) / ks;
    if (steps < 4 || (long)(ks - 1) * steps >= nk) continue;
    const long rounds = (b256 * ks + VST_NUM_CUS - 1) / VST_NUM_CUS;
    const double us = rounds * (steps * 2.25 + 4.0) + (double)(ks + 1) * M * Cop * 4.0 / 4.0e6 + 3.0;
    if (us < best) {
      best = us;
      bk = ks;
    }
  }
  *ks_out = bk;
}

size_t bf_fprop_ws_floats(long M, int Cop, int C, int R, int S, int math) {
  int mf, ks;
  bf_split_plan(M, Cop, C, R, S, math, -1, &mf, &ks);
  return ks ? (size_t)ks * (M - mf) * Cop : 0;
}

int bf_fprop_launch(const float* x, const void* wsplit, long wps, const float* bias, float* y, int N,
                    int H, int W, int C, int Ho, int Wo, int Cop, int R, int S, int st, int padh, int padw,
                    int reflect, int act, float slope, int math, int kind, hipStream_t s, double* part,
                    float* tws, size_t tws_floats, const float* addend, int oph) {
  if (oph) tws = nullptr;
  VST_REQUIRE(!(part && addend), "conv fprop: IN partials together with an addend are not supported");
  const int M = N * Ho * Wo, K = R * S * C;
  if (kind < 0 && padh == padw && !addend && !oph && c4_direct_ok(C, Cop, R, S, st, Ho, Wo, math))
    return c4_direct_launch(x, wsplit, wps, bias, y, N, H, W, Ho, Wo, R, S, padh, reflect, act, slope, math, part, s);
  const __bf16* ws = reinterpret_cast<const __bf16*>(wsplit);
  int kd, m_split, tail_kind;
  bf_plan(M, Cop, math, kind, &kd, &m_split, &tail_kind);
  int ks = 0, m_first = 0;
  if (tws) {
    bf_split_plan(M, Cop, C, R, S, math, kind, &m_first, &ks);
    if ((size_t)ks * (M - m_first) * Cop > tws_floats) ks = 0;
    if (ks && !m_first) {
      m_split = 0;
      kd = -1;
    }
  }
#define VST_BF(BM_, BN_, WM_, WN_, BK_, NP_)                                                       \
  {                                                                                                 \
    using T = bf::Tile<BM_, BN_, WM_, WN_, BK_, NP_>;                                              \
    const dim3 grid(ceil_div(Mend - mb, BM_) * ceil_div(Cop, BN_));                                 \
    if (C == 4)                                                                                     \
      hipLaunchKernelGGL((bf::conv_fprop_bf_k<T, false, 3>), grid, dim3(T::NT), 0, s, x, ws, wps, bias, y, \
                         H, W, C, Ho, Wo, Cop, S, st, padh, padw, reflect, act, slope, Mend, K, mb, part, 0,      \
                         nullptr, addend, oph);                                                          \
    else if (VST_BF_KSLICE && C % BK_ == 0 && reflect)                                              \
      hipLaunchKernelGGL((bf::conv_fprop_bf_k<T, true, 1>), grid, dim3(T::NT), 0, s, x, ws, wps, bias, y, \
                         H, W, C, Ho, Wo, Cop, S, st, padh, padw, reflect, act, slope, Mend, K, mb, part, 0,      \
                         nullptr, addend, oph);                                                          \
    else if (VST_BF_KSLICE && C % BK_ == 0)                                                         \
      hipLaunchKernelGGL((bf::conv_fprop_bf_k<T, true, 0>), grid, dim3(T::NT), 0, s, x, ws, wps, bias, y, \
                         H, W, C, Ho, Wo, Cop, S, st, padh, padw, reflect, act, slope, Mend, K, mb, part, 0,      \
                         nullptr, addend, oph);                                                          \
    else                                                                                            \
      hipLaunchKernelGGL((bf::conv_fprop_bf_k<T, false, 2>), grid, dim3(T::NT), 0, s, x, ws, wps, bias, y, \
                         H, W, C, Ho, Wo, Cop, S, st, padh, padw, reflect, act, slope, Mend, K, mb, part, 0,      \
                         nullptr, addend, oph);                                                          \
  }
  for (int ph = (ks && !m_first) ? 1 : 0; ph < ((m_split || (ks && !m_first)) ? 2 : 1); ++ph) {
    const int mb = ph ? m_split : 0, Mend = (m_split && !ph) ? m_split : M;
    const int kp = ph ? tail_kind : kd;
    if (ph == 1 && ks) {
      using T = bf::Tile<256, 128, 64, 64, 32, 3>;
      const int nk = (K + T::BK - 1) / T::BK, spk = (nk + ks - 1) / ks;
      const dim3 grid(ceil_div(M - mb, 256) * ceil_div(Cop, 128) * ks);
      if (reflect)
        hipLaunchKernelGGL((bf::conv_fprop_bf_k<T, true, 1, true>), grid, dim3(T::NT), 0, s, x, ws, wps, bias, y, H,
                           W, C, Ho, Wo, Cop, S, st, padh, padw, reflect, act, slope, M, K, mb, part, spk, tws,
                           nullptr);
      else
        hipLaunchKernelGGL((bf::conv_fprop_bf_k<T, true, 0, true>), grid, dim3(T::NT), 0, s, x, ws, wps, bias, y, H,
                           W, C, Ho, Wo, Cop, S, st, padh, padw, reflect, act, slope, M, K, mb, part, spk, tws,
                           nullptr);
      hipLaunchKernelGGL(bf::fprop_splitk_reduce_k, dim3(ceil_div(M - mb, 32), ceil_div(Cop, 64)), dim3(256), 0, s,
                         tws, ks, mb, M, Cop, bias, act, slope, y, part, Ho * Wo, addend);
      continue;
    }
    if (math == VST_MATH_BF16X6) {
      VST_BF_DISPATCH(kp, 3, VST_BF)
    } else {
      VST_BF_DISPATCH(kp, 2, VST_BF)
    }
  }
#undef VST_BF
  return check_launch("conv2d_fwd(bf16 split)");
}


static void bf_border_plan(int N, int H, int W, int Cy, int Cx, int math, int* ks_out, long* mb_out) {
  const int NB = bf::dgrad_border_rows(H, W);
  const long Mb = (long)N * NB;
  const int bm = math == VST_MATH_BF16X6 ? 256 : 128;
  const long tiles = ((Mb + bm - 1) / bm) * ((Cx + 127) / 128);
  const int nk = (9 * Cy + 31) / 32;
  int ks = (int)(VST_NUM_CUS / (tiles > 0 ? tiles : 1));
  ks = ks < 1 ? 1 : (ks > 16 ? 16 : ks);
  while (ks > 1 && (ks - 1) * ((nk + ks - 1) / ks) >= nk) --ks;
  *ks_out = ks;
  *mb_out = Mb;
}

static constexpr bool g_border5 = true;
static constexpr int g_border_ks = 0;
static void bf_border5_plan(int N, int H, int W, int Cy, int Cx, int* ks_out, int* lt, int* ll) {
  *lt = bf::border5_seg_rows(N, W + 2, 128);
  *ll = bf::border5_seg_rows(N, H, 128);
  const long tiles = (long)(2 * *lt + 2 * *ll) / 128 * ((Cx + 127) / 128);
  const int nk = (3 * Cy + 31) / 32;
  int ks = g_border_ks > 0 ? g_border_ks : (int)(VST_NUM_CUS / (tiles > 0 ? tiles : 1));
  if (g_border_ks <= 0 && ks > nk / 4) ks = nk / 4;
  ks = ks < 1 ? 1 : (ks > 16 ? 16 : ks);
  while (ks > 1 && (ks - 1) * ((nk + ks - 1) / ks) >= nk) --ks;
  *ks_out = ks;
}

bool bf_dgrad_refl1_ok(int N, int H, int W, int Cy, int Cx, int math) {
  return math != VST_MATH_F32 && VST_BF_KSLICE && Cy % 32 == 0 && Cx % 4 == 0 && H >= 4 && W >= 4 && N > 0;
}

size_t bf_dgrad_refl1_slabs(int N, int H, int W, int Cy, int Cx, int math, BorderSlabs* b) {
  if (g_border5) {
    bf_border5_plan(N, H, W, Cy, Cx, &b->ks, &b->Lt, &b->Ll);
    b->Mb = 2 * b->Lt + 2 * b->Ll;
  } else {
    long Mb;
    bf_border_plan(N, H, W, Cy, Cx, math, &b->ks, &Mb);
    b->Mb = (int)Mb;
    b->Lt = bf::dgrad_border_rows(H, W);
    b->Ll = 0;
  }
  return bf_fprop_ws_floats((long)N * H * W, Cx, Cy, 3, 3, math);
}

size_t bf_dgrad_refl1_ws_floats(int N, int H, int W, int Cy, int Cx, int math) {
  int ks, ks5, lt, ll;
  long Mb;
  bf_border_plan(N, H, W, Cy, Cx, math, &ks, &Mb);
  bf_border5_plan(N, H, W, Cy, Cx, &ks5, &lt, &ll);
  const size_t b4 = (size_t)ks * Mb * Cx, b5 = g_border5 ? (size_t)ks5 * (2 * lt + 2 * ll) * Cx : 0;
  return bf_fprop_ws_floats((long)N * H * W, Cx, Cy, 3, 3, math) + (b4 > b5 ? b4 : b5);
}

int bf_dgrad_refl1_launch(const float* dy, const void* wsplit, long wps, const float* addend, float* dx, int N, int H,
                          int W, int Cy, int Cx, int math, hipStream_t s, float* ws, size_t ws_floats, bool add_border) {
  int ks;
  long Mb;
  bf_border_plan(N, H, W, Cy, Cx, math, &ks, &Mb);
  const size_t main_ws = bf_fprop_ws_floats((long)N * H * W, Cx, Cy, 3, 3, math);
  VST_REQUIRE(ws_floats >= main_ws + (size_t)ks * Mb * Cx, "dgrad_refl: workspace too small");
  if (int e = bf_fprop_launch(dy, wsplit, wps, nullptr, dx, N, H, W, Cy, H, W, Cx, 3, 3, 1, 1, 1, 0, VST_ACT_NONE, 0.f,
                              math, -1, s, nullptr, main_ws ? ws : nullptr, main_ws, addend))
    return e;
  float* slab = ws + main_ws;
  const __bf16* wb = reinterpret_cast<const __bf16*>(wsplit);
  if (g_border5) {
    int ks5, lt, ll;
    bf_border5_plan(N, H, W, Cy, Cx, &ks5, &lt, &ll);
    const int Mt = 2 * lt + 2 * ll, K = 3 * Cy;
    VST_REQUIRE(ws_floats >= main_ws + (size_t)ks5 * Mt * Cx, "dgrad_refl: workspace too small");
#define VST_B5(NP_)                                                                                            {                                                                                                             using T = bf::Tile<128, 128, 64, 32, 32, NP_>;                                                              const int nk = (K + T::BK - 1) / T::BK, spk = (nk + ks5 - 1) / ks5;                                         const dim3 grid(Mt / 128 * ceil_div(Cx, 128) * ks5);                                                        hipLaunchKernelGGL((bf::conv_fprop_bf_k<T, true, 5, true>), grid, dim3(T::NT), 0, s, dy, wb, wps, nullptr,                          dx, H, W, Cy, lt, ll, Cx, 3, N, 1, 1, 0, VST_ACT_NONE, 0.f, Mt, K, 0, nullptr, spk,                           slab, nullptr);                                                                        }
    if (math == VST_MATH_BF16X6)
      VST_B5(3)
    else
      VST_B5(2)
#undef VST_B5
    const int T = 2 * W + 2 * H;
    if (add_border)
      hipLaunchKernelGGL(bf::dgrad_border5_add_k, dim3(ceil_div((long)N * T, 16), ceil_div(Cx, 64)), dim3(256), 0, s,
                       slab, ks5, Mt, Cx, dx, N, H, W, lt, ll);
    return check_launch("conv2d_dgrad_refl");
  }
  const int NB = bf::dgrad_border_rows(H, W), K = 9 * Cy;
  if (math == VST_MATH_BF16X6) {
    using T = bf::Tile<256, 128, 64, 64, 32, 3>;
    const int nk = (K + T::BK - 1) / T::BK, spk = (nk + ks - 1) / ks;
    const dim3 grid(ceil_div(Mb, 256) * ceil_div(Cx, 128) * ks);
    hipLaunchKernelGGL((bf::conv_fprop_bf_k<T, true, 4, true>), grid, dim3(T::NT), 0, s, dy, wb, wps, nullptr, dx, H,
                       W, Cy, H, NB, Cx, 3, 1, 1, 1, 0, VST_ACT_NONE, 0.f, (int)Mb, K, 0, nullptr, spk, slab, nullptr);
  } else {
    using T = bf::Tile<128, 128, 64, 32, 32, 2>;
    const int nk = (K + T::BK - 1) / T::BK, spk = (nk + ks - 1) / ks;
    const dim3 grid(ceil_div(Mb, 128) * ceil_div(Cx, 128) * ks);
    hipLaunchKernelGGL((bf::conv_fprop_bf_k<T, true, 4, true>), grid, dim3(T::NT), 0, s, dy, wb, wps, nullptr, dx, H,
                       W, Cy, H, NB, Cx, 3, 1, 1, 1, 0, VST_ACT_NONE, 0.f, (int)Mb, K, 0, nullptr, spk, slab, nullptr);
  }
  if (add_border)
    hipLaunchKernelGGL(bf::dgrad_border_add_k, dim3(ceil_div(Mb, 16), ceil_div(Cx, 64)), dim3(256), 0, s, slab, ks,
                       (int)Mb, Cx, dx, H, W, NB);
  return check_launch("conv2d_dgrad_refl");
}

int bf_dgrad_refl1_inb_slices(int H, int W) { return H * W / 32 + (2 * W + 2 * H + 15) / 16; }

bool bf_dgrad_refl1_inb_ok(int N, int H, int W, int Cy, int Cx, int math) {
  if (math != VST_MATH_BF16X6 || !g_border5 || !bf_dgrad_refl1_ok(N, H, W, Cy, Cx, math) || (H * W) % 32) return false;
  int kd, m_split, tail_kind, m_first, fks;
  const long M = (long)N * H * W;
  if (M > (1L << 30)) return false;
  bf_plan(M, Cx, math, -1, &kd, &m_split, &tail_kind);
  bf_split_plan(M, Cx, Cy, 3, 3, math, -1, &m_first, &fks);
  if (fks && !m_first) return true;
  return kd == 7 && (!m_split || (fks && m_first == m_split));
}

int bf_dgrad_refl1_inb_launch(const float* dy, const void* wsplit, long wps, const float* addend, float* dx, int N,
                              int H, int W, int Cy, int Cx, int math, hipStream_t s, float* ws, size_t ws_floats,
                              const float* z, const float* st, double* part, int act, float slope,
                              const __bf16* apl, long pps) {
  VST_REQUIRE(bf_dgrad_refl1_inb_ok(N, H, W, Cy, Cx, math), "conv2d_dgrad_refl_in_epi: unsupported shape / arithmetic");
  const long M = (long)N * H * W;
  int kd, m_split, tail_kind, m_first, fks;
  bf_plan(M, Cx, math, -1, &kd, &m_split, &tail_kind);
  bf_split_plan(M, Cx, Cy, 3, 3, math, -1, &m_first, &fks);
  const size_t main_ws = bf_fprop_ws_floats(M, Cx, Cy, 3, 3, math);
  int ks5, lt, ll;
  bf_border5_plan(N, H, W, Cy, Cx, &ks5, &lt, &ll);
  const int Mt = 2 * lt + 2 * ll, K5 = 3 * Cy, K = 9 * Cy;
  VST_REQUIRE(ws_floats >= main_ws + (size_t)ks5 * Mt * Cx, "conv2d_dgrad_refl_in_epi: workspace too small");
  const bf::InbArgs inb{z, st, part, act, slope, bf_dgrad_refl1_inb_slices(H, W)};
  const __bf16* wb = reinterpret_cast<const __bf16*>(wsplit);
  using T = bf::Tile<256, 128, 64, 64, 32, 3>;
  const long mb = (fks && !m_first) ? 0 : (m_split ? m_split : M);
  if (mb > 0) {
    const dim3 grid(ceil_div(mb, 256) * ceil_div(Cx, 128));
    if (apl)
      hipLaunchKernelGGL((bf::conv_fprop_bf_inb_k<T, true>), grid, dim3(T::NT), 0, s, dy, wb, wps, dx, H, W, Cy, Cx,
                         addend, (int)mb, K, inb, apl, pps);
    else
      hipLaunchKernelGGL((bf::conv_fprop_bf_inb_k<T>), grid, dim3(T::NT), 0, s, dy, wb, wps, dx, H, W, Cy, Cx, addend,
                         (int)mb, K, inb);
  }
  if (mb < M) {
    const int nk = (K + T::BK - 1) / T::BK, spk = (nk + fks - 1) / fks;
    const dim3 grid(ceil_div(M - mb, 256) * ceil_div(Cx, 128) * fks);
    if (apl)
      hipLaunchKernelGGL((bf::conv_fprop_bf_k<T, true, 0, true, true>), grid, dim3(T::NT), 0, s, dy, wb, wps, nullptr, dx,
                         H, W, Cy, H, W, Cx, 3, 1, 1, 1, 0, VST_ACT_NONE, 0.f, (int)M, K, (int)mb, nullptr, spk, ws,
                         nullptr, 0, apl, pps);
    else
      hipLaunchKernelGGL((bf::conv_fprop_bf_k<T, true, 0, true>), grid, dim3(T::NT), 0, s, dy, wb, wps, nullptr, dx, H,
                         W, Cy, H, W, Cx, 3, 1, 1, 1, 0, VST_ACT_NONE, 0.f, (int)M, K, (int)mb, nullptr, spk, ws,
                         nullptr);
    hipLaunchKernelGGL(bf::fprop_splitk_reduce_inb_k, dim3(ceil_div(M - mb, 32), ceil_div(Cx, 64)), dim3(256), 0, s, ws,
                       fks, (int)mb, (int)M, Cx, dx, H * W, addend, inb);
  }
  float* slab = ws + main_ws;
  {
    using T5 = bf::Tile<128, 128, 64, 32, 32, 3>;
    const int nk = (K5 + T5::BK - 1) / T5::BK, spk = (nk + ks5 - 1) / ks5;
    const dim3 grid(Mt / 128 * ceil_div(Cx, 128) * ks5);
    if (apl)
      hipLaunchKernelGGL((bf::conv_fprop_bf_k<T5, true, 5, true, true>), grid, dim3(T5::NT), 0, s, dy, wb, wps, nullptr,
                         dx, H, W, Cy, lt, ll, Cx, 3, N, 1, 1, 0, VST_ACT_NONE, 0.f, Mt, K5, 0, nullptr, spk, slab,
                         nullptr, 0, apl, pps);
    else
      hipLaunchKernelGGL((bf::conv_fprop_bf_k<T5, true, 5, true>), grid, dim3(T5::NT), 0, s, dy, wb, wps, nullptr, dx,
                         H, W, Cy, lt, ll, Cx, 3, N, 1, 1, 0, VST_ACT_NONE, 0.f, Mt, K5, 0, nullptr, spk, slab, nullptr);
  }
  hipLaunchKernelGGL(bf::dgrad_border5_add_inb_k, dim3(ceil_div(2 * W + 2 * H, 16), N, ceil_div(Cx, 64)), dim3(256), 0,
                     s, slab, ks5, Mt, Cx, dx, H, W, lt, ll, inb, H * W / 32);
  return check_launch("conv2d_dgrad_refl_in_epi");
}

bool bf_convT_phases_ok(int C, int Cop, int math) {
  return math != VST_MATH_F32 && VST_BF_KSLICE && C % 32 == 0 && Cop % 4 == 0;
}

static constexpr int g_convt_tile = -1;

int bf_convT_phases_launch(const float* x, const void* const ws[4], const float* bias, float* y, int N, int H, int W,
                           int C, int Cop, int act, float slope, int math, hipStream_t s, int full) {
  VST_REQUIRE(bf_convT_phases_ok(C, Cop, math), "convT phases: unsupported shape / arithmetic");
  const int bn = Cop <= 64 ? 64 : 128;
  auto grid_of = [&](int bm_, bf::PhaseJobs* jb) {
    int tt = 0;
    for (int j = 0; j < 4; ++j) {
      const int ph = j == 0 ? 3 : (j == 1 ? 1 : (j == 2 ? 2 : 0)), a = ph >> 1, b = ph & 1;
      if (jb) {
        jb->ws[j] = reinterpret_cast<const __bf16*>(ws[ph]);
        jb->t0[j] = tt;
      }
      const long rows = (long)N * (H + (full ? 1 : a)) * (W + (full ? 1 : b));
      const long tiles = (rows + bm_ - 1) / bm_ * ((Cop + bn - 1) / bn);
      tt += (int)((tiles + 7) / 8 * 8);
    }
    if (jb) jb->t0[4] = tt;
    return tt;
  };
  int tk = math != VST_MATH_BF16X6 ? 0 : (g_convt_tile >= 0 ? g_convt_tile : (bn == 128 ? 1 : 2));
  if (math == VST_MATH_BF16X6 && g_convt_tile < 0 && bn == 128) {
    const long r256 = (grid_of(256, nullptr) + VST_NUM_CUS - 1) / VST_NUM_CUS;
    const long r128 = (grid_of(128, nullptr) + VST_NUM_CUS - 1) / VST_NUM_CUS;
    tk = r256 * 2.25 <= r128 * 1.5 ? 1 : 0;
  }
  const int bm = (tk == 1 && bn == 128) ? 256 : ((tk == 2 && bn == 64) ? 64 : 128);
  bf::PhaseJobs jobs;
  const int t = grid_of(bm, &jobs);
#define VST_CTB(BM_, BN_, WM_, WN_)                                                                       \
  {                                                                                                        \
    using T = bf::Tile<BM_, BN_, WM_, WN_, 32, 3>;                                                         \
    hipLaunchKernelGGL(bf::conv_convT_phases_k<T>, dim3(t), dim3(T::NT), 0, s, x, jobs, bias, y, N, H, W, C, Cop, \
                       act, slope, full);                                                                  \
  }
#define VST_CT(BN_, WN_, NP_)                                                                             \
  {                                                                                                        \
    using T = bf::Tile<128, BN_, 64, WN_, 32, NP_>;                                                        \
    hipLaunchKernelGGL(bf::conv_convT_phases_k<T>, dim3(t), dim3(T::NT), 0, s, x, jobs, bias, y, N, H, W, C, Cop, \
                       act, slope, full);                                                                  \
  }
  if (math == VST_MATH_BF16X6 && tk == 1) {
    if (bn == 64) VST_CT(64, 32, 3) else VST_CTB(256, 128, 64, 64)
  } else if (math == VST_MATH_BF16X6 && tk == 2) {
    if (bn == 64) VST_CTB(64, 64, 32, 32) else VST_CTB(128, 128, 64, 64)
  } else if (math == VST_MATH_BF16X6) {
    if (bn == 64) VST_CT(64, 32, 3) else VST_CT(128, 32, 3)
  } else {
    if (bn == 64) VST_CT(64, 32, 2) else VST_CT(128, 32, 2)
  }
#undef VST_CT
#undef VST_CTB
  return check_launch("conv2d_convT_s2");
}

void bf_nhwc_to_planes(const float* x, void* y, long P, int Cs, int np, hipStream_t s, int row_in, int row_out) {
  const dim3 g((unsigned)((P + 63) / 64), ceil_div(Cs, 64));
  __bf16* yb = reinterpret_cast<__bf16*>(y);
  if (np == 3)
    hipLaunchKernelGGL(bf::nhwc_to_cp_planes_k<3>, g, dim3(256), 0, s, x, yb, P, Cs, rk_cp_ld(P), row_in, row_out);
  else
    hipLaunchKernelGGL(bf::nhwc_to_cp_planes_k<2>, g, dim3(256), 0, s, x, yb, P, Cs, rk_cp_ld(P), row_in, row_out);
}

void bf_wgrad_launch(const float* xt, const void* dyp, float* slab, int N, int H, int W, int Cx, int Ho,
                     int Wo, int Cyp, int S, int pad, int st, int Mw, int chunk, int nsplit, int kind, int math,
                     hipStream_t s) {
  const int P = N * Ho * Wo;
  const long ldx = rk_cp_ld((long)N * (H + 2 * pad) * (W + 2 * pad)), ldy = rk_cp_ld(P);
  const __bf16* d = reinterpret_cast<const __bf16*>(dyp);
  const long dps = (long)Cyp * ldy;
#define VST_BW(BM_, BN_, WM_, WN_, BK_, NP_)                                                          \
  {                                                                                                 \
    using T = bf::Tile<BM_, BN_, WM_, WN_, BK_, NP_>;                                              \
    const dim3 grid(ceil_div(Mw, BM_) * ceil_div(Cyp, BN_) * nsplit);                              \
    if (Wo >= BK_)                                                                                  \
      hipLaunchKernelGGL((bf::conv_wgrad_bf_k<T, true>), grid, dim3(T::NT), 0, s, xt, d, dps, slab, H, W, \
                         Cx, Ho, Wo, Cyp, S, pad, st, Mw, P, chunk, ldx, ldy);                      \
    else                                                                                            \
      hipLaunchKernelGGL((bf::conv_wgrad_bf_k<T, false>), grid, dim3(T::NT), 0, s, xt, d, dps, slab, H, W, \
                         Cx, Ho, Wo, Cyp, S, pad, st, Mw, P, chunk, ldx, ldy);                      \
  }
  if (math == VST_MATH_BF16X6) {
    VST_BF_DISPATCH(kind, 3, VST_BW)
  } else {
    VST_BF_DISPATCH(kind, 2, VST_BW)
  }
#undef VST_BW
}

bool bf_wgrad_nhwc_ok(int kind, int Wo, int Cx, int Cyp) {
  return VST_BF_MF16 && (kind == 7 || kind == 0) && Wo % 32 == 0 && Cx % 8 == 0 && Cyp % 8 == 0;
}

void bf_wgrad_nhwc_launch(const float* x, const void* dy, long pps, bool bf32, float* slab, int N, int H, int W,
                          int Cx, int Ho, int Wo, int Cyp, int S, int pad, int st, int reflect, int Mw, int chunk,
                          int nsplit, int kind, hipStream_t s, float* dwd, int dco, int dacc) {
  const int P = N * Ho * Wo;
#define VST_WN(BM_, WN_)                                                                                         \
  {                                                                                                              \
    using T = bf::Tile<BM_, 128, 64, WN_, 32, 3>;                                                                \
    const dim3 grid(ceil_div(Mw, T::BM) * ceil_div(Cyp, T::BN) * nsplit);                                       \
    if (bf32)                                                                                                    \
      hipLaunchKernelGGL((bf::conv_wgrad_nhwc_k<T, true>), grid, dim3(T::NT), 0, s, x, dy, pps, slab, H, W, Cx,  \
                         Ho, Wo, Cyp, S, pad, st, reflect, Mw, P, chunk, dwd, dco, dacc);                        \
    else                                                                                                         \
      hipLaunchKernelGGL((bf::conv_wgrad_nhwc_k<T, false>), grid, dim3(T::NT), 0, s, x, dy, pps, slab, H, W, Cx, \
                         Ho, Wo, Cyp, S, pad, st, reflect, Mw, P, chunk, dwd, dco, dacc);                        \
  }
  if (kind == 7) VST_WN(256, 64) else VST_WN(128, 32)
#undef VST_WN
}

void bf_wgrad_geom(int kind, int math, int* bm, int* bn, int* bk, int* slots) {
  int sl;
  bf_geom(kind, math == VST_MATH_BF16X6 ? 3 : 2, bm, bn, &sl);
  *bk = 32;
  *slots = sl * VST_NUM_CUS;
}

}

using namespace vst;

extern "C" const char* vst_build_info(void) {
#define VST_STR2(x) #x
#define VST_STR(x) VST_STR2(x)
#if VST_BF_MF16
#define VST_X6_MFMA "16x16x32"
#else
#define VST_X6_MFMA "32x32x16"
#endif
  return "x6_mfma=" VST_X6_MFMA " x3_mfma=32x32x16 kslice=" VST_STR(VST_BF_KSLICE) " x6_256=" VST_STR(VST_BF_X6_256)
         " m16_store=" VST_STR(VST_M16_STORE) " m16_sched=" VST_STR(VST_M16_SCHED);
#undef VST_X6_MFMA
#undef VST_STR
#undef VST_STR2
}

extern "C" int vst_weight_split(const float* w, void* out, long n, void* stream) {
  VST_REQUIRE(w && out && n > 0, "weight_split: bad args");
  hipLaunchKernelGGL(bf::split3_k, dim3(ceil_div(n, 256)), dim3(256), 0, (hipStream_t)stream, w,
                     reinterpret_cast<__bf16*>(out), n);
  return check_launch("weight_split");
}

extern "C" size_t vst_conv2d_dgrad_refl_ws_bytes(int N, int H, int W, int Cy, int Cx, int math) {
  if (!bf_dgrad_refl1_ok(N, H, W, Cy, Cx, math)) return 0;
  return bf_dgrad_refl1_ws_floats(N, H, W, Cy, Cx, math) * sizeof(float);
}

extern "C" int vst_conv2d_dgrad_refl(const float* dy, const void* wsplit, const float* addend, float* dx, float* ws,
                                     size_t ws_bytes, int N, int H, int W, int Cy, int Cx, int math, void* stream) {
  VST_REQUIRE(dy && wsplit && dx && ws, "conv2d_dgrad_refl: null pointer");
  if (!bf_dgrad_refl1_ok(N, H, W, Cy, Cx, math)) {
    ::vst::set_error("conv2d_dgrad_refl: needs split-bf16 math, Cy %% 32 == 0, Cx %% 4 == 0, H, W >= 4");
    return VST_EUNSUPPORTED;
  }
  return bf_dgrad_refl1_launch(dy, wsplit, (long)Cx * 9 * Cy, addend, dx, N, H, W, Cy, Cx, math, (hipStream_t)stream,
                               ws, ws_bytes / sizeof(float), true);
}
```

gan-based-video-style-transfer_amd/csrc/norm.hip:

```cpp
#include "common.h"

namespace vst {

constexpr int NRED = 256;
#ifndef IN_TARGET_BLOCKS
#define IN_TARGET_BLOCKS 512
#endif

struct RedGeom {
  int LP, PG, SP, nsplit;
};

static bool red_geom(int N, int HW, int C, RedGeom& g) {
  if (C % 4) return false;
  g.LP = C / 4;
  if (g.LP > NRED) return false;
  g.PG = NRED / g.LP;
  long sp = ((long)N * HW + IN_TARGET_BLOCKS - 1) / IN_TARGET_BLOCKS;
  if (sp < 2L * g.PG) sp = 2L * g.PG;
  sp = (sp + g.PG - 1) / g.PG * g.PG;
  if (sp > HW) sp = HW;
  g.SP = (int)sp;
  g.nsplit = ceil_div(HW, g.SP);
  return true;
// ... 850 lines not shown
template <bool STATS, bool HAS_D>
__global__ void skip_apply_k(const float4* __restrict__ y, const float* __restrict__ stats,
                             float4* __restrict__ d, float* __restrict__ cat, long total4, int HW, int C4,
                             int Cs, int c0, float slope) {
  const long i = (long)blockIdx.x * blockDim.x + threadIdx.x;
  if (i >= total4) return;
  const int c4 = i % C4;
  const long pix = i / C4;
  float4 v = y[i];
  if (STATS) skip_z4(v, stats, (pix / HW) * C4 + c4);
  if (HAS_D)
    d[i] = make_float4(v.x > 0.f ? v.x : v.x * slope, v.y > 0.f ? v.y : v.y * slope,
                       v.z > 0.f ? v.z : v.z * slope, v.w > 0.f ? v.w : v.w * slope);
  *reinterpret_cast<float4*>(cat + pix * Cs + c0 + 4 * c4) =
      make_float4(v.x > 0.f ? v.x : 0.f, v.y > 0.f ? v.y : 0.f, v.z > 0.f ? v.z : 0.f, v.w > 0.f ? v.w : 0.f);
}

template <bool STATS>
__global__ __launch_bounds__(NRED) void skip_partial_k(const float* __restrict__ gd, const float* __restrict__ gcat,
                                                       const float* __restrict__ y, const float* __restrict__ stats,
                                                       double* __restrict__ part, int HW, int C, int Cs, int c0,
                                                       int LP, int PG, int SP, int nsplit, float slope) {
  constexpr int NV = STATS ? 3 : 1;
  struct Row {
    float4 y, gd, gs;
  };
  const int c4 = (int)threadIdx.x % LP, n = blockIdx.y;
  const float4* yb = reinterpret_cast<const float4*>(y) + (long)n * HW * LP + c4;
  const float4* db = gd ? reinterpret_cast<const float4*>(gd) + (long)n * HW * LP + c4 : nullptr;
  const float* sb = gcat + (long)n * HW * Cs + c0 + 4 * c4;
  const long nc4 = (long)n * LP + c4;
  slice_partials<NV>(
      [=](long p) {
        return Row{yb[p * LP], db ? db[p * LP] : make_float4(0.f, 0.f, 0.f, 0.f),
                   *reinterpret_cast<const float4*>(sb + p * Cs)};
      },
      [=](const Row& r, double(&acc)[NV][4]) {
        float4 v = r.y;
        if (STATS) skip_z4(v, stats, nc4);
        const float zz[4] = {v.x, v.y, v.z, v.w};
        const float ga[4] = {r.gd.x, r.gd.y, r.gd.z, r.gd.w}, gb[4] = {r.gs.x, r.gs.y, r.gs.z, r.gs.w};
#pragma unroll
        for (int j = 0; j < 4; ++j) {
          const float g = skip_g(ga[j], gb[j], zz[j], slope);
          acc[0][j] += g;
          if constexpr (STATS) {
            acc[1][j] += (double)g * zz[j];
            acc[2][j] += zz[j];
          }
        }
      },
      part, HW, C, LP, PG, SP, nsplit);
}

template <int CPB>
__global__ void skip_db_finalize_k(const double* __restrict__ part, double* __restrict__ dbn, int C, int nsplit) {
  double a[1];
  const int n = blockIdx.y;
  if (!fold_slices<1, CPB>(part, n, C, nsplit, a)) return;
  dbn[n * C + blockIdx.x * CPB + (threadIdx.x % CPB)] = a[0];
}

template <bool STATS, bool HAS_GD>
__global__ void skip_bwd_apply_k(const float4* __restrict__ gd, const float* __restrict__ gcat,
                                 const float4* __restrict__ y, const float* __restrict__ stats,
                                 const float2* __restrict__ coef, float4* __restrict__ dy, long total4, int HW,
                                 int C4, int Cs, int c0, float slope, const double* __restrict__ dbn,
                                 float* __restrict__ db, int N, int accumulate_db) {
  if (db && blockIdx.x * blockDim.x < 4 * C4)
    in_bias_grad_blocks(dbn, db, N, 4 * C4, accumulate_db, blockIdx.x * blockDim.x + threadIdx.x);
  const long i = (long)blockIdx.x * blockDim.x + threadIdx.x;
  if (i >= total4) return;
  const int c4 = i % C4;
  const long pix = i / C4;
  const long nc4 = (pix / HW) * C4 + c4;
  float4 v = y[i];
  if (STATS) skip_z4(v, stats, nc4);
  const float4 a = HAS_GD ? gd[i] : make_float4(0.f, 0.f, 0.f, 0.f);
  const float4 b = *reinterpret_cast<const float4*>(gcat + pix * Cs + c0 + 4 * c4);
  float4 o = make_float4(skip_g(a.x, b.x, v.x, slope), skip_g(a.y, b.y, v.y, slope), skip_g(a.z, b.z, v.z, slope),
                         skip_g(a.w, b.w, v.w, slope));
  if (STATS) {
    const float4* st = reinterpret_cast<const float4*>(stats) + nc4 * 2;
    const float4 s0 = st[0], s1 = st[1];
    const float4 k01 = reinterpret_cast<const float4*>(coef)[nc4 * 2];
    const float4 k23 = reinterpret_cast<const float4*>(coef)[nc4 * 2 + 1];
    o.x = s0.y * (o.x - k01.x - v.x * k01.y);
    o.y = s0.w * (o.y - k01.z - v.y * k01.w);
    o.z = s1.y * (o.z - k23.x - v.z * k23.y);
    o.w = s1.w * (o.w - k23.z - v.w * k23.w);
  }
  dy[i] = o;
}

}

using namespace vst;

struct BwdWs {
  double* part;
  float2* tab;
  double* sums;
  size_t bytes;
  BwdWs(float* ws, int N, int nsplit, int C, int nv, int ntab, int nsum) {
    const size_t otab = (size_t)N * nsplit * C * nv * sizeof(double), osum = otab + (size_t)N * C * ntab * sizeof(float2);
    part = reinterpret_cast<double*>(ws);
    tab = reinterpret_cast<float2*>(reinterpret_cast<char*>(ws) + otab);
    sums = reinterpret_cast<double*>(reinterpret_cast<char*>(ws) + osum);
    bytes = osum + (size_t)N * C * nsum * sizeof(double) + 256;
  }
};

template <class K4, class K16, class... Args>
static void launch_fin(K4 k4, K16 k16, int C, int N, int nsplit, hipStream_t s, Args... args) {
  if (fin_cpb(C, N, nsplit) == 4)
    hipLaunchKernelGGL(k4, dim3(ceil_div(C, 4), N), dim3(256), 0, s, args...);
  else
    hipLaunchKernelGGL(k16, dim3(ceil_div(C, 16), N), dim3(256), 0, s, args...);
}

extern "C" size_t vst_instnorm_ws_bytes(int N, int HW, int C) {
  RedGeom g;
  if (!red_geom(N, HW, C, g)) return 0;
  return BwdWs(nullptr, N, g.nsplit, C, 3, 1, 1).bytes;
}

extern "C" size_t vst_instnorm_skip_ws_bytes(int N, int HW, int C) {
  return N <= 0 || HW <= 0 ? 0 : vst_instnorm_ws_bytes(N, HW, C);
}

static int skip_args(const char* what, bool ptrs, int N, int HW, int C, int Cs, int c0, RedGeom& g) {
  VST_REQUIRE(ptrs && N > 0 && HW > 0 && C > 0 && Cs > 0 && c0 >= 0, "%s: null pointer or non-positive size", what);
  if (C % 4 || c0 % 4 || Cs % 4 || (long)c0 + C > Cs || C > 4 * NRED || !red_geom(N, HW, C, g)) {
    set_error("%s: C %% 4 == 0, c0 %% 4 == 0, Cs %% 4 == 0, c0 + C <= Cs and C <= 1024 (C %d, c0 %d, Cs %d)", what,
              C, c0, Cs);
    return VST_EUNSUPPORTED;
  }
  return VST_OK;
}

extern "C" int vst_instnorm_skip_fwd(const float* y, const float* stats, float* d, float* cat, int N, int HW, int C,
                                     int Cs, int c0, float slope, void* stream) {
  RedGeom g;
  if (const int rc = skip_args("instnorm_skip_fwd", y && cat, N, HW, C, Cs, c0, g)) return rc;
  const long total4 = (long)N * HW * C / 4;
  auto launch = [&](auto kern) {
    hipLaunchKernelGGL(kern, dim3(ceil_div(total4, 256)), dim3(256), 0, (hipStream_t)stream,
                       reinterpret_cast<const float4*>(y), stats, reinterpret_cast<float4*>(d), cat, total4, HW, C / 4,
                       Cs, c0, slope);
  };
  if (stats) d ? launch(skip_apply_k<true, true>) : launch(skip_apply_k<true, false>);
  else d ? launch(skip_apply_k<false, true>) : launch(skip_apply_k<false, false>);
  return check_launch("instnorm_skip_fwd");
}

extern "C" int vst_instnorm_skip_bwd(const float* g_d, const float* g_cat, int Cs, int c0, const float* y,
                                     const float* stats, float* dy, float* db, int accumulate_db, float* ws, int N,
                                     int HW, int C, float slope, void* stream) {
  RedGeom g;
  if (const int rc = skip_args("instnorm_skip_bwd", g_cat && y && dy && (ws || (!stats && !db)), N, HW, C, Cs, c0, g))
    return rc;
  hipStream_t s = (hipStream_t)stream;
  const BwdWs w(ws, N, g.nsplit, C, 3, 1, 1);
  if (stats) {
    hipLaunchKernelGGL(skip_partial_k<true>, dim3(g.nsplit, N), dim3(NRED), 0, s, g_d, g_cat, y, stats, w.part, HW, C,
                       Cs, c0, g.LP, g.PG, g.SP, g.nsplit, slope);
    launch_fin(in_bwd_finalize_k<4>, in_bwd_finalize_k<16>, C, N, g.nsplit, s, w.part, stats, w.tab, w.sums, N, HW, C,
               g.nsplit);
  } else if (db) {
    hipLaunchKernelGGL(skip_partial_k<false>, dim3(g.nsplit, N), dim3(NRED), 0, s, g_d, g_cat, y, stats, w.part, HW, C,
                       Cs, c0, g.LP, g.PG, g.SP, g.nsplit, slope);
    launch_fin(skip_db_finalize_k<4>, skip_db_finalize_k<16>, C, N, g.nsplit, s, w.part, w.sums, C, g.nsplit);
  }
  const long total4 = (long)N * HW * C / 4;
  const int blocks = std::max(ceil_div(total4, 256), ceil_div(C, 256));
  auto launch = [&](auto kern) {
    hipLaunchKernelGGL(kern, dim3(blocks), dim3(256), 0, s, reinterpret_cast<const float4*>(g_d), g_cat,
                       reinterpret_cast<const float4*>(y), stats, w.tab, reinterpret_cast<float4*>(dy), total4, HW,
                       C / 4, Cs, c0, slope, w.sums, db, N, accumulate_db);
  };
  if (stats) g_d ? launch(skip_bwd_apply_k<true, true>) : launch(skip_bwd_apply_k<true, false>);
  else g_d ? launch(skip_bwd_apply_k<false, true>) : launch(skip_bwd_apply_k<false, false>);
  return check_launch("instnorm_skip_bwd");
}

extern "C" int vst_instnorm_stats(const float* x, float* stats, float* ws, int N, int HW, int C,
                                  float eps, void* stream) {
  RedGeom g;
  VST_REQUIRE(x && stats && ws && N > 0 && HW > 0 && red_geom(N, HW, C, g),
              "instnorm_stats: bad args (C must be a multiple of 4, at most 1024)");
  hipStream_t s = (hipStream_t)stream;
  double* part = reinterpret_cast<double*>(ws);
  hipLaunchKernelGGL(in_partial_k<0>, dim3(g.nsplit, N), dim3(NRED), 0, s, x, (const float*)nullptr,
                     (const float*)nullptr, part, HW, C, g.LP, g.PG, g.SP, g.nsplit, 0, 0.f);
  launch_fin(in_finalize_k<4>, in_finalize_k<16>, C, N, g.nsplit, s, part, stats, N, HW, C, g.nsplit, eps);
  return check_launch("instnorm_stats");
}

extern "C" int vst_instnorm_finalize(const double* part, float* stats, int N, int HW, int C, int nsplit,
                                     float eps, void* stream) {
  VST_REQUIRE(part && stats && N > 0 && HW > 0 && C > 0 && nsplit > 0, "instnorm_finalize: bad args");
  launch_fin(in_finalize_k<4>, in_finalize_k<16>, C, N, nsplit, (hipStream_t)stream, part, stats, N, HW, C, nsplit, eps);
  return check_launch("instnorm_finalize");
}

extern "C" int vst_instnorm_act_fwd(const float* x, const float* stats, const float* residual,
                                    float* y, int N, int HW, int C, int act, float slope,
                                    void* stream) {
  VST_REQUIRE(x && stats && y && C % 4 == 0, "instnorm_act_fwd: bad args");
  const long total4 = (long)N * HW * C / 4;
  hipLaunchKernelGGL(in_apply_k, dim3(ceil_div(total4, 256)), dim3(256), 0, (hipStream_t)stream,
                     reinterpret_cast<const float4*>(x), stats, reinterpret_cast<const float4*>(residual),
                     reinterpret_cast<float4*>(y), total4, HW, C / 4, act, slope);
  return check_launch("instnorm_act_fwd");
}

extern "C" int vst_instnorm_act_fwd_cp(const float* x, const float* stats, const float* residual, float* y,
                                       float* xt, int N, int H, int W, int C, int act, float slope, int pad,
                                       int pad_mode, int stride, void* stream) {
  VST_REQUIRE(x && stats && y && xt && C % 4 == 0 && pad >= 0 && (stride == 1 || stride == 2),
              "instnorm_act_fwd_cp: bad args");
  VST_REQUIRE(pad_mode == VST_PAD_ZERO || (pad < H && pad < W), "instnorm_act_fwd_cp: reflect pad >= size");
  VST_REQUIRE(stride == 1 || (W + 2 * pad) % 2 == 0, "instnorm_act_fwd_cp: stride 2 needs W + 2 pad even");
  const long P = (long)N * (H + 2 * pad) * (W + 2 * pad);
  hipLaunchKernelGGL(in_apply_cp_pad_k, dim3(ceil_div(P, 64), ceil_div(C, 64)), dim3(256), 0, (hipStream_t)stream,
                     x, stats, residual, y, xt, N, H, W, C, pad, pad_mode == VST_PAD_REFLECT, stride == 2,
                     rk_cp_ld(P), act, slope);
  return check_launch("instnorm_act_fwd_cp");
}

extern "C" int vst_instnorm_act_fwd_planes(const float* x, const float* stats, const float* residual, float* y,
                                           void* planes, int N, int H, int W, int C, int act, float slope, int pad,
                                           int pad_mode, int wx, void* stream) {
  VST_REQUIRE(x && stats && y && planes && C % 4 == 0 && pad >= 0 && wx >= 0, "instnorm_act_fwd_planes: bad args");
  VST_REQUIRE(pad_mode == VST_PAD_ZERO || (pad < H && pad < W), "instnorm_act_fwd_planes: reflect pad >= size");
  const long P = (long)N * (H + 2 * pad) * (W + 2 * pad + wx);
  hipLaunchKernelGGL(in_apply_cp_pad_k, dim3(ceil_div(P, 64), ceil_div(C, 64)), dim3(256), 0, (hipStream_t)stream,
                     x, stats, residual, y, nullptr, N, H, W, C, pad, pad_mode == VST_PAD_REFLECT, 0, rk_cp_ld(P), act,
                     slope, wx, reinterpret_cast<__bf16*>(planes));
  return check_launch("instnorm_act_fwd_planes");
}

static int in_bwd_tail(const float* gy, const float* x, const float* stats, float* dx, float* db, float* ws,
                       int N, int HW, int C, int act, float slope, int accumulate_db, void* planes, long ldp,
                       const RedGeom& g, hipStream_t s, void* apl = nullptr) {
  const BwdWs w(ws, N, g.nsplit, C, 3, 1, 1);
  launch_fin(in_bwd_finalize_k<4>, in_bwd_finalize_k<16>, C, N, g.nsplit, s, w.part, stats, w.tab, w.sums, N, HW, C,
             g.nsplit);
  if (planes) {
    const long P = (long)N * HW;
    hipLaunchKernelGGL(in_bwd_apply_planes_k, dim3(ceil_div(P, 64), ceil_div(C, 64)), dim3(256), 0, s, gy, x, stats,
                       w.tab, dx, reinterpret_cast<__bf16*>(planes), P, HW, C, ldp, act, slope, w.sums, db, N,
                       accumulate_db, reinterpret_cast<__bf16*>(apl));
    return check_launch("instnorm_act_bwd_planes");
  }
  const long total4 = (long)N * HW * C / 4;
  VST_REQUIRE(!db || total4 >= C, "instnorm_act_bwd: fewer elements than channels");
  hipLaunchKernelGGL(in_bwd_apply_k, dim3(ceil_div(total4, 256)), dim3(256), 0, s,
                     reinterpret_cast<const float4*>(gy), reinterpret_cast<const float4*>(x), stats,
                     w.tab, reinterpret_cast<float4*>(dx), total4, HW, C / 4, act, slope, w.sums, db, N,
                     accumulate_db, reinterpret_cast<__bf16*>(apl));
  return check_launch("instnorm_act_bwd");
}

extern "C" int vst_instnorm_act_bwd_planes(const float* gy, const float* x, const float* stats, float* dx,
                                           float* db, float* ws, int N, int HW, int C, int act, float slope,
                                           int accumulate_db, void* planes, long ldp, void* stream) {
  RedGeom g;
  VST_REQUIRE(gy && x && stats && dx && ws && red_geom(N, HW, C, g), "instnorm_act_bwd: bad args");
  VST_REQUIRE(!planes || ldp >= (long)N * HW, "instnorm_act_bwd: plane stride %ld < N*HW", ldp);
  hipStream_t s = (hipStream_t)stream;
  double* part = reinterpret_cast<double*>(ws);
  hipLaunchKernelGGL(in_partial_k<1>, dim3(g.nsplit, N), dim3(NRED), 0, s, x, gy, stats, part, HW, C,
                     g.LP, g.PG, g.SP, g.nsplit, act, slope);
  return in_bwd_tail(gy, x, stats, dx, db, ws, N, HW, C, act, slope, accumulate_db, planes, ldp, g, s);
}

extern "C" int vst_instnorm_act_bwd(const float* gy, const float* x, const float* stats, float* dx,
                                    float* db, float* ws, int N, int HW, int C, int act, float slope,
                                    int accumulate_db, void* stream) {
  return vst_instnorm_act_bwd_planes(gy, x, stats, dx, db, ws, N, HW, C, act, slope, accumulate_db, nullptr,
                                     0, stream);
}

extern "C" int vst_instnorm_act_bwd_planes_apre(const float* gy, const float* x, const float* stats, float* dx,
                                                float* db, float* ws, int N, int HW, int C, int act, float slope,
                                                int accumulate_db, void* planes, long ldp, void* apl, void* stream) {
  RedGeom g;
  VST_REQUIRE(gy && x && stats && dx && ws && apl && red_geom(N, HW, C, g), "instnorm_act_bwd_apre: bad args");
  VST_REQUIRE(!planes || ldp >= (long)N * HW, "instnorm_act_bwd_apre: plane stride %ld < N*HW", ldp);
  hipStream_t s = (hipStream_t)stream;
  double* part = reinterpret_cast<double*>(ws);
  hipLaunchKernelGGL(in_partial_k<1>, dim3(g.nsplit, N), dim3(NRED), 0, s, x, gy, stats, part, HW, C,
                     g.LP, g.PG, g.SP, g.nsplit, act, slope);
  return in_bwd_tail(gy, x, stats, dx, db, ws, N, HW, C, act, slope, accumulate_db, planes, ldp, g, s, apl);
}

static size_t in_epi_ws_bytes_al(int N, int H, int W, int C) {
  return (BwdWs(nullptr, N, bf_dgrad_refl1_inb_slices(H, W), C, 3, 1, 1).bytes + 255) / 256 * 256;
}

extern "C" size_t vst_conv2d_dgrad_refl_in_epi_ws_bytes(int N, int H, int W, int Cy, int Cx, int math) {
  if (Cx % 4 || !bf_dgrad_refl1_inb_ok(N, H, W, Cy, Cx, math)) return 0;
  return in_epi_ws_bytes_al(N, H, W, Cx) + bf_dgrad_refl1_ws_floats(N, H, W, Cy, Cx, math) * sizeof(float);
}

extern "C" int vst_conv2d_dgrad_refl_epi_part(const float* dy, const void* dy_apl, const void* wsplit,
                                              const float* addend, float* gout, const float* x, const float* stats,
                                              float* ws, size_t ws_bytes, int N, int H, int W, int Cy, int Cx, int act,
                                              float slope, int math, void* stream) {
  const size_t need = vst_conv2d_dgrad_refl_in_epi_ws_bytes(N, H, W, Cy, Cx, math);
  VST_REQUIRE(dy && wsplit && gout && x && stats && ws, "conv2d_dgrad_refl_in_epi: null pointer");
  VST_REQUIRE(need > 0 && ws_bytes >= need,
              "conv2d_dgrad_refl_in_epi: unsupported shape or workspace too small (%zu of %zu bytes)", ws_bytes, need);
  const size_t inb = in_epi_ws_bytes_al(N, H, W, Cx);
  float* dws = reinterpret_cast<float*>(reinterpret_cast<char*>(ws) + inb);
  return bf_dgrad_refl1_inb_launch(dy, wsplit, (long)Cx * 9 * Cy, addend, gout, N, H, W, Cy, Cx, math,
                                   (hipStream_t)stream, dws, (ws_bytes - inb) / sizeof(float), x, stats,
                                   reinterpret_cast<double*>(ws), act, slope, reinterpret_cast<const __bf16*>(dy_apl),
                                   (long)N * H * W * Cy);
}

extern "C" int vst_instnorm_act_bwd_epi_tail(const float* gout, const float* x, const float* stats, float* dx,
                                             float* db, float* ws, int N, int H, int W, int Cx, int act, float slope,
                                             int accumulate_db, void* planes, long ldp, void* apl, void* stream) {
  VST_REQUIRE(gout && x && stats && dx && ws && Cx % 4 == 0 && (H * W) % 32 == 0, "instnorm_act_bwd_epi_tail: bad args");
  VST_REQUIRE(!planes || ldp >= (long)N * H * W, "instnorm_act_bwd_epi_tail: plane stride %ld < N*HW", ldp);
  RedGeom g{};
  g.nsplit = bf_dgrad_refl1_inb_slices(H, W);
  return in_bwd_tail(gout, x, stats, dx, db, ws, N, H * W, Cx, act, slope, accumulate_db, planes, ldp, g,
                     (hipStream_t)stream, apl);
}

extern "C" int vst_conv2d_dgrad_refl_in_epi(const float* dy, const void* wsplit, const float* addend, float* gout,
                                            const float* x, const float* stats, float* dx, float* db, float* ws,
                                            size_t ws_bytes, int N, int H, int W, int Cy, int Cx, int act, float slope,
                                            int accumulate_db, void* planes, long ldp, int math, void* stream) {
  VST_REQUIRE(dx, "conv2d_dgrad_refl_in_epi: null pointer");
  if (int e = vst_conv2d_dgrad_refl_epi_part(dy, nullptr, wsplit, addend, gout, x, stats, ws, ws_bytes, N, H, W, Cy,
                                             Cx, act, slope, math, stream))
    return e;
  return vst_instnorm_act_bwd_epi_tail(gout, x, stats, dx, db, ws, N, H, W, Cx, act, slope, accumulate_db, planes, ldp,
                                       nullptr, stream);
}

extern "C" int vst_act_bwd(const float* gy, const float* y, float* dx, long n, int act, float slope,
                           void* stream) {
  VST_REQUIRE(gy && y && dx, "act_bwd: null pointer");
  hipLaunchKernelGGL(act_bwd_k, dim3(ceil_div(n, 256)), dim3(256), 0, (hipStream_t)stream, gy, y, dx,
                     n, act, slope);
  return check_launch("act_bwd");
}

extern "C" size_t vst_channel_sum_ws_bytes(long NHW, int Cs) {
  RedGeom g;
  if (Cs % 4 || !red_geom(1, (int)NHW, std::min(Cs, 4 * NRED), g)) return 0;
  return (size_t)g.nsplit * Cs * sizeof(double);
}

extern "C" int vst_channel_sum(const float* x, float* db, float* ws, long NHW, int Cs, int Cl,
                               int accumulate, void* stream) {
  RedGeom g;
  VST_REQUIRE(x && db && ws && Cl <= Cs && NHW > 0 && Cs % 4 == 0 &&
                  red_geom(1, (int)NHW, std::min(Cs, 4 * NRED), g),
              "channel_sum: bad args");
  hipStream_t s = (hipStream_t)stream;
  double* part = reinterpret_cast<double*>(ws);
  const int cs4 = Cs / 4;
  for (int c4off = 0; c4off < cs4; c4off += g.LP)
    hipLaunchKernelGGL(chsum_partial_k, dim3(g.nsplit), dim3(NRED), 0, s, x, part, NHW, g.LP, g.PG, g.SP, cs4,
                       c4off, std::min(g.LP, cs4 - c4off));
  hipLaunchKernelGGL(chsum_final_k, dim3(ceil_div(Cs, 64)), dim3(256), 0, s, part, db, g.nsplit, Cs, Cl,
                     accumulate);
  return check_launch("channel_sum");
}

extern "C" size_t vst_instnorm_affine_ws_bytes(int N, int HW, int C) {
  RedGeom g;
  if (!red_geom(N, HW, C, g)) return 0;
  return BwdWs(nullptr, N, g.nsplit, C, 4, 1, 4).bytes;
}

extern "C" int vst_instnorm_affine_fwd(const float* x, const float* stats, const float* gamma,
                                       const float* beta, const float* gate, float gate_mult,
                                       const float* residual, float* y, int N, int HW, int C, int act,
                                       float slope, void* stream) {
  VST_REQUIRE(x && stats && gamma && beta && y && C % 4 == 0 && N > 0 && HW > 0,
              "instnorm_affine_fwd: bad args");
  const long total4 = (long)N * HW * C / 4;
  hipLaunchKernelGGL(in_aff_apply_k, dim3(ceil_div(total4, 256)), dim3(256), 0, (hipStream_t)stream,
                     reinterpret_cast<const float4*>(x), stats, gamma, beta, gate, gate_mult,
                     reinterpret_cast<const float4*>(residual), reinterpret_cast<float4*>(y), total4, HW,
                     C / 4, act, slope);
  return check_launch("instnorm_affine_fwd");
}

extern "C" int vst_instnorm_affine_bwd(const float* gy, const float* x, const float* stats,
                                       const float* gamma, const float* beta, const float* gate,
                                       float gate_mult, float* dx, float* dgamma, float* dbeta,
                                       float* dgate, float* dbias, float* ws, int N, int HW, int C,
                                       int act, float slope, int accumulate, void* stream) {
  RedGeom g;
  VST_REQUIRE(gy && x && stats && gamma && beta && dx && ws && red_geom(N, HW, C, g),
              "instnorm_affine_bwd: bad args (C must be a multiple of 4, at most 1024)");
  hipStream_t s = (hipStream_t)stream;
  const BwdWs w(ws, N, g.nsplit, C, 4, 1, 4);
  hipLaunchKernelGGL(in_aff_partial_k, dim3(g.nsplit, N), dim3(NRED), 0, s, x, gy, stats, gamma, beta,
                     gate, gate_mult, w.part, HW, C, g.LP, g.PG, g.SP, g.nsplit, act, slope);
  hipLaunchKernelGGL(in_aff_finalize_k, dim3(ceil_div(C, 64), N), dim3(256), 0, s, w.part, stats, gamma,
                     w.tab, w.sums, N, HW, C, g.nsplit);
  hipLaunchKernelGGL(in_aff_param_grad_k, dim3(1), dim3(256), 0, s, w.sums, dgamma, dbeta, dbias, gate,
                     gate_mult, dgate, N, C, accumulate);
  const long total4 = (long)N * HW * C / 4;
  hipLaunchKernelGGL(in_aff_bwd_apply_k, dim3(ceil_div(total4, 256)), dim3(256), 0, s,
                     reinterpret_cast<const float4*>(gy), reinterpret_cast<const float4*>(x), stats, gamma,
                     beta, gate, gate_mult, w.tab, reinterpret_cast<float4*>(dx), total4, HW, C / 4, act,
                     slope);
  return check_launch("instnorm_affine_bwd");
}

extern "C" size_t vst_cond_instnorm_ws_bytes(int N, int HW, int C) {
  RedGeom g;
  if (N <= 0 || HW <= 0 || !red_geom(N, HW, C, g)) return 0;
  return BwdWs(nullptr, N, g.nsplit, C, 3, 2, 3).bytes;
}

static bool cond_args_ok(int N, int HW, int C, int Cl, int S, int act, RedGeom& g) {
  return N > 0 && HW > 0 && red_geom(N, HW, C, g) && Cl > 0 && Cl <= C && S >= 1 &&
         (act == VST_ACT_NONE || act == VST_ACT_RELU);
}

extern "C" int vst_cond_instnorm_fwd(const float* x, const float* stats, const int* sid, const float* embed,
                                     const float* bn_weight, const float* bn_bias, float* y, float* ws, int N,
                                     int HW, int C, int Cl, int S, int act, void* stream) {
  RedGeom g;
  VST_REQUIRE(x && stats && sid && embed && bn_weight && bn_bias && y && ws && cond_args_ok(N, HW, C, Cl, S, act, g),
              "cond_instnorm_fwd: bad args (C a multiple of 4, at most 1024; 0 < Cl <= C; S >= 1; act none | relu)");
  hipStream_t s = (hipStream_t)stream;
  float2* tab = reinterpret_cast<float2*>(ws);
  hipLaunchKernelGGL(cond_coef_k, dim3(ceil_div((long)N * C, 256)), dim3(256), 0, s, stats, sid, embed, bn_weight,
                     bn_bias, tab, N, C, Cl, S);
  const long total4 = (long)N * HW * C / 4;
  hipLaunchKernelGGL(cond_apply_k, dim3(ceil_div(total4, 256)), dim3(256), 0, s, reinterpret_cast<const float4*>(x),
                     reinterpret_cast<const float4*>(tab), reinterpret_cast<float4*>(y), total4, HW, C / 4, act);
  return check_launch("cond_instnorm_fwd");
}

extern "C" int vst_cond_instnorm_bwd(const float* gy, const float* x, const float* stats, const int* sid,
                                     const float* embed, const float* bn_weight, const float* bn_bias, float* dx,
                                     float* dembed, float* dbn_weight, float* dbn_bias, float* dbias, float* ws,
                                     int N, int HW, int C, int Cl, int S, int act, int accumulate, void* stream) {
  RedGeom g;
  VST_REQUIRE(gy && x && stats && sid && embed && bn_weight && bn_bias && dx && ws &&
                  cond_args_ok(N, HW, C, Cl, S, act, g),
              "cond_instnorm_bwd: bad args (C a multiple of 4, at most 1024; 0 < Cl <= C; S >= 1; act none | relu)");
  hipStream_t s = (hipStream_t)stream;
  const BwdWs w(ws, N, g.nsplit, C, 3, 2, 3);
  float2 *tab = w.tab, *coef = w.tab + (size_t)N * C;
  hipLaunchKernelGGL(cond_partial_k, dim3(g.nsplit, N), dim3(NRED), 0, s, x, gy, stats, sid, embed, bn_weight,
                     bn_bias, w.part, HW, C, Cl, S, g.LP, g.PG, g.SP, g.nsplit, act);
  hipLaunchKernelGGL(cond_finalize_k, dim3(ceil_div(C, 64), N), dim3(256), 0, s, w.part, stats, sid, embed,
                     bn_weight, bn_bias, tab, coef, w.sums, N, HW, C, Cl, S, g.nsplit);
  if (dembed || dbn_weight || dbn_bias || dbias)
    hipLaunchKernelGGL(cond_param_grad_k, dim3(1), dim3(256), 0, s, w.sums, sid, embed, bn_weight, bn_bias, dembed,
                       dbn_weight, dbn_bias, dbias, N, C, Cl, S, accumulate);
  const long total4 = (long)N * HW * C / 4;
  hipLaunchKernelGGL(cond_bwd_apply_k, dim3(ceil_div(total4, 256)), dim3(256), 0, s,
                     reinterpret_cast<const float4*>(gy), reinterpret_cast<const float4*>(x),
                     reinterpret_cast<const float4*>(stats), reinterpret_cast<const float4*>(tab),
                     reinterpret_cast<const float4*>(coef), reinterpret_cast<float4*>(dx), total4, HW, C / 4, act);
  return check_launch("cond_instnorm_bwd");
}

extern "C" size_t vst_adain_ws_bytes(int N, int HW, int C) {
  RedGeom g;
  if (N <= 0 || HW <= 0 || !red_geom(N, HW, C, g)) return 0;
  return BwdWs(nullptr, N, g.nsplit, C, 3, 2, 3).bytes;
}

static bool adain_args_ok(int N, int HW, int C, int act, RedGeom& g) {
  return N > 0 && HW > 0 && C > 0 && red_geom(N, HW, C, g) && (act == VST_ACT_NONE || act == VST_ACT_LRELU);
}

extern "C" int vst_adain_fwd(const float* x, const float* stats, const float* h, float* y, float* ws, int N, int HW,
                             int C, int act, float slope, void* stream) {
  RedGeom g;
  VST_REQUIRE(x && stats && h && y && ws && adain_args_ok(N, HW, C, act, g),
              "adain_fwd: bad args (C a multiple of 4, at most 1024; act none | lrelu)");
  hipStream_t s = (hipStream_t)stream;
  float2* tab = reinterpret_cast<float2*>(ws);
  hipLaunchKernelGGL(adain_coef_k, dim3(ceil_div((long)N * C, 256)), dim3(256), 0, s, stats, h, tab, N, C);
  const long total4 = (long)N * HW * C / 4;
  hipLaunchKernelGGL(adain_apply_k, dim3(ceil_div(total4, 256)), dim3(256), 0, s, reinterpret_cast<const float4*>(x),
                     reinterpret_cast<const float4*>(tab), reinterpret_cast<float4*>(y), total4, HW, C / 4, act,
                     slope);
  return check_launch("adain_fwd");
}

extern "C" int vst_adain_bwd(const float* gy, const float* x, const float* stats, const float* h, float* dx,
                             float* dh, float* dbias, float* ws, int N, int HW, int C, int act, float slope,
                             int accumulate, void* stream) {
  RedGeom g;
  VST_REQUIRE(gy && x && stats && h && dx && ws && adain_args_ok(N, HW, C, act, g),
              "adain_bwd: bad args (C a multiple of 4, at most 1024; act none | lrelu)");
  hipStream_t s = (hipStream_t)stream;
  const BwdWs w(ws, N, g.nsplit, C, 3, 2, 3);
  float2 *tab = w.tab, *coef = w.tab + (size_t)N * C;
  hipLaunchKernelGGL(adain_coef_k, dim3(ceil_div((long)N * C, 256)), dim3(256), 0, s, stats, h, tab, N, C);
  hipLaunchKernelGGL(adain_partial_k, dim3(g.nsplit, N), dim3(NRED), 0, s, x, gy, stats, tab, w.part, HW, C, g.LP,
                     g.PG, g.SP, g.nsplit, act, slope);
  hipLaunchKernelGGL(adain_finalize_k, dim3(ceil_div(C, 64), N), dim3(256), 0, s, w.part, tab, coef, w.sums, N, HW, C,
                     g.nsplit);
  if (dh || dbias)
    hipLaunchKernelGGL(adain_param_grad_k, dim3(ceil_div((long)N * C, 256)), dim3(256), 0, s, w.sums, dh, dbias, N, C,
                       accumulate);
  const long total4 = (long)N * HW * C / 4;
  hipLaunchKernelGGL(adain_bwd_apply_k, dim3(ceil_div(total4, 256)), dim3(256), 0, s,
                     reinterpret_cast<const float4*>(gy), reinterpret_cast<const float4*>(x),
                     reinterpret_cast<const float4*>(stats), reinterpret_cast<const float4*>(tab),
                     reinterpret_cast<const float4*>(coef), reinterpret_cast<float4*>(dx), total4, HW, C / 4, act,
                     slope);
  return check_launch("adain_bwd");
}

extern "C" int vst_instnorm_running_update(const float* stats, float* running_mean, float* running_var,
                                           int N, int C, int HW, float momentum, float eps,
                                           void* stream) {
  VST_REQUIRE(stats && running_mean && running_var && N > 0 && C > 0, "instnorm_running_update: bad args");
  hipLaunchKernelGGL(in_running_update_k, dim3(ceil_div(C, 256)), dim3(256), 0, (hipStream_t)stream, stats,
                     running_mean, running_var, N, C, HW, momentum, eps);
  return check_launch("instnorm_running_update");
}

extern "C" int vst_instnorm_stats_from_running(const float* running_mean, const float* running_var,
                                               float* stats, int N, int C, float eps, void* stream) {
  VST_REQUIRE(running_mean && running_var && stats && N > 0 && C > 0, "instnorm_stats_from_running: bad args");
  hipLaunchKernelGGL(in_stats_from_running_k, dim3(ceil_div((long)N * C, 256)), dim3(256), 0,
                     (hipStream_t)stream, running_mean, running_var, stats, N, C, eps);
  return check_launch("instnorm_stats_from_running");
}
```

Measured before the change: 79.46 frames/s.

## Fold reflect-pad border gradients into dy before dgrad GEMM

Replaces the separate border-row split-K GEMM pass and border-add kernels of the reflect-pad-1 conv dgrad with a small pre-pass. That pre-pass sums the mirrored dy pixels into a compact fold buffer, which the main implicit-GEMM kernel then gathers (REFL==6) while walking whole taps. This removes one extra GEMM launch, its slab workspace and the border-add/reduction kernels, and drops the extra inb stat slices. In exchange the main kernel's A-gather gets more index logic, and the fold buffer adds workspace and a pass over border pixels.

```diff
diff --git a/gan-based-video-style-transfer_amd/csrc/common.h b/gan-based-video-style-transfer_amd/csrc/common.h
--- a/gan-based-video-style-transfer_amd/csrc/common.h
+++ b/gan-based-video-style-transfer_amd/csrc/common.h
@@ -42,44 +42,57 @@
   return i >= n ? 2 * n - 2 - i : i;
 }
 
-__host__ __device__ __forceinline__ int dgrad_border_rows_of(int h, int w, int H, int W, int* b0) {
-  const int sw = W - 2, sh = H - 2, S4 = ((2 * sw + 2 * sh + 3) / 4) * 4;
-  const bool rh = h == 1 || h == H - 2, rw = w == 1 || w == W - 2;
-  if (rh && rw) {
-    *b0 = S4 + 4 * ((h == 1 ? 0 : 2) + (w == 1 ? 0 : 1));
-    return 3;
+__host__ __device__ __forceinline__ int dgrad_fold_pixels(int H, int W) { return 2 * W + 2 * H + 4; }
+
+struct DgradFoldTap {
+  int isel, jsel;
+  int qr, qc, qx;
+};
+
+__host__ __device__ __forceinline__ DgradFoldTap dgrad_fold_tap(int kr, int ks, int H, int W) {
+  DgradFoldTap t;
+  t.isel = kr == 2 ? 1 : (kr == 0 ? H - 2 : -1);
+  t.jsel = ks == 2 ? 1 : (ks == 0 ? W - 2 : -1);
+  t.qr = kr == 2 ? 0 : W;
+  t.qc = 2 * W + (ks == 2 ? 0 : H);
+  t.qx = 2 * W + 2 * H + (kr == 2 ? 0 : 2) + (ks == 2 ? 0 : 1);
+  return t;
+}
+
+__host__ __device__ __forceinline__ int dgrad_fold_pixel_tap(const DgradFoldTap& t, int i, int j, int hi, int wi) {
+  const bool rf = i == t.isel, cf = j == t.jsel;
+  const int q = cf ? (rf ? t.qx : t.qc + hi) : t.qr + wi;
+  return (rf | cf) ? q : -1;
+}
+
+__host__ __device__ __forceinline__ int dgrad_fold_pixel(int i, int j, int hi, int wi, int H, int W) {
+  return dgrad_fold_pixel_tap(dgrad_fold_tap(hi - i + 1, wi - j + 1, H, W), i, j, hi, wi);
+}
+
+__host__ __device__ __forceinline__ int dgrad_fold_sources(int q, int H, int W, int* hs, int* ws) {
+  if (q < 2 * W) {
+    const bool top = q < W;
+    hs[0] = top ? 2 : H - 3;
+    hs[1] = top ? 0 : H - 1;
+    ws[0] = ws[1] = top ? q : q - W;
+    return 2;
   }
-  const int kw = w == 0 ? 0 : (w == W - 1 ? sw - 1 : w - 1);
-  const int kh = h == 0 ? 0 : (h == H - 1 ? sh - 1 : h - 1);
-  if (h == 1) { *b0 = kw; return 1; }
-  if (h == H - 2) { *b0 = sw + kw; return 1; }
-  if (w == 1) { *b0 = 2 * sw + kh; return 1; }
-  if (w == W - 2) { *b0 = 2 * sw + sh + kh; return 1; }
-  return 0;
-}
-
-struct BorderSlabs {
-  int ks, Mb, Lt, Ll;
-};
-
-__host__ __device__ __forceinline__ int dgrad_border_slab_rows(int n, int h, int w, int H, int W, int Lt, int Ll,
-                                                               int* rows) {
-  if (Ll == 0) {
-    int b0;
-    const int nr = dgrad_border_rows_of(h, w, H, W, &b0);
-    for (int r = 0; r < nr; ++r) rows[r] = n * Lt + b0 + r;
-    return nr;
+  if (q < 2 * W + 2 * H) {
+    const int r = q - 2 * W;
+    const bool left = r < H;
+    ws[0] = left ? 2 : W - 3;
+    ws[1] = left ? 0 : W - 1;
+    hs[0] = hs[1] = left ? r : r - H;
+    return 2;
   }
-  int nr = 0;
-  if (h == 1 || h == H - 2) {
-    const int base = (h == 1 ? 0 : Lt) + n * (W + 2);
-    rows[nr++] = base + w + 1;
-    if (w == 1) rows[nr++] = base;
-    if (w == W - 2) rows[nr++] = base + W + 1;
-  }
-  if (w == 1) rows[nr++] = 2 * Lt + n * H + h;
-  if (w == W - 2) rows[nr++] = 2 * Lt + Ll + n * H + h;
-  return nr;
+  const int g = q - 2 * W - 2 * H;
+  const bool top = g < 2, left = (g & 1) == 0;
+  const int hn = top ? 2 : H - 3, hf = top ? 0 : H - 1, wn = left ? 2 : W - 3, wf = left ? 0 : W - 1;
+  hs[0] = hn; ws[0] = wn;
+  hs[1] = hf; ws[1] = wn;
+  hs[2] = hn; ws[2] = wf;
+  hs[3] = hf; ws[3] = wf;
+  return 4;
 }
 
 __device__ __forceinline__ float apply_act(float v, int act, float slope) {
@@ -128,7 +141,7 @@
                     int H, int W, int C, int Ho, int Wo, int Cop, int R, int S, int st, int padh, int padw,
                     int reflect, int act, float slope, int math, int kind, hipStream_t s,
                     double* part = nullptr, float* tws = nullptr, size_t tws_floats = 0, const float* addend = nullptr,
-                    int oph = 0);
+                    int oph = 0, const float* fold = nullptr);
 bool tap64_ok(int Cx, int R, int W, int math);
 int tap64_launch(const float* x, const void* wsplit, long wps, const float* bias, float* y, int N, int H, int W,
                  int pad, int reflect, int act, float slope, int math, hipStream_t s);
@@ -138,9 +151,9 @@
                      hipStream_t s);
 bool bf_dgrad_refl1_ok(int N, int H, int W, int Cy, int Cx, int math);
 size_t bf_dgrad_refl1_ws_floats(int N, int H, int W, int Cy, int Cx, int math);
-size_t bf_dgrad_refl1_slabs(int N, int H, int W, int Cy, int Cx, int math, BorderSlabs* b);
+size_t bf_dgrad_refl1_inb_ws_floats(int N, int H, int W, int Cy, int Cx, int math);
 int bf_dgrad_refl1_launch(const float* dy, const void* wsplit, long wps, const float* addend, float* dx, int N, int H,
-                          int W, int Cy, int Cx, int math, hipStream_t s, float* ws, size_t ws_floats, bool add_border);
+                          int W, int Cy, int Cx, int math, hipStream_t s, float* ws, size_t ws_floats);
 bool bf_dgrad_refl1_inb_ok(int N, int H, int W, int Cy, int Cx, int math);
 int bf_dgrad_refl1_inb_slices(int H, int W);
 int bf_dgrad_refl1_inb_launch(const float* dy, const void* wsplit, long wps, const float* addend, float* dx, int N,
diff --git a/gan-based-video-style-transfer_amd/csrc/conv_bf.hip b/gan-based-video-style-transfer_amd/csrc/conv_bf.hip
--- a/gan-based-video-style-transfer_amd/csrc/conv_bf.hip
+++ b/gan-based-video-style-transfer_amd/csrc/conv_bf.hip
@@ -484,194 +484,51 @@
   gd = g * d;
 }
 
-__host__ __device__ __forceinline__ int dgrad_border_rows(int H, int W) {
-  return ((2 * (W - 2) + 2 * (H - 2) + 3) / 4) * 4 + 16;
-}
-
-__host__ __device__ __forceinline__ void dgrad_border_pos(int b, int H, int W, int& qh, int& qw, int& th, int& tw) {
-  const int sw = W - 2, sh = H - 2, S = 2 * sw + 2 * sh, S4 = (S + 3) / 4 * 4;
-  qh = qw = th = tw = -100;
-  if (b < 2 * sw) {
-    const int k = b < sw ? b : b - sw;
-    tw = k == 0 ? 0 : (k == sw - 1 ? W - 1 : k + 1);
-    qw = tw;
-    qh = b < sw ? -1 : H;
-    th = b < sw ? 1 : H - 2;
-    return;
-  }
-  if (b < S) {
-    const int b2 = b - 2 * sw, k = b2 < sh ? b2 : b2 - sh;
-    th = k == 0 ? 0 : (k == sh - 1 ? H - 1 : k + 1);
-    qh = th;
-    qw = b2 < sh ? -1 : W;
-    tw = b2 < sh ? 1 : W - 2;
-    return;
-  }
-  if (b < S4) return;
-  const int g = (b - S4) >> 2, r = (b - S4) & 3;
-  if (r == 3) return;
-  const int top = g < 2, left = (g & 1) == 0;
-  th = top ? 1 : H - 2;
-  tw = left ? 1 : W - 2;
-  const int ph = top ? -1 : H, pw = left ? -1 : W;
-  if (r == 0) { qh = ph; qw = tw; }
-  else if (r == 1) { qh = ph; qw = pw; }
-  else { qh = th; qw = pw; }
-}
-
-__global__ __launch_bounds__(256) void dgrad_border_add_k(const float* __restrict__ slab, int ks, int Mb, int C,
-                                                          float* __restrict__ dx, int H, int W, int NB) {
-  const int t = threadIdx.x;
-  const int c = blockIdx.y * 64 + (t & 15) * 4;
-  const int m = blockIdx.x * 16 + (t >> 4);
-  if (m >= Mb || c >= C) return;
-  const int n = m / NB, b = m - n * NB;
-  int qh, qw, th, tw;
-  dgrad_border_pos(b, H, W, qh, qw, th, tw);
-  if (th < 0) return;
-  const int S4 = NB - 16;
-  if (b >= S4 && ((b - S4) & 3) != 0) return;
-  const int nr = b >= S4 ? 3 : 1;
-  const long zst = (long)Mb * C;
-  float4 v = make_float4(0.f, 0.f, 0.f, 0.f);
-  for (int r = 0; r < nr; ++r) {
-    const float* base = slab + (long)(m + r) * C + c;
-    float4 u[16];
-#pragma unroll
-    for (int z = 0; z < 16; ++z)
-      if (z < ks) u[z] = *reinterpret_cast<const float4*>(base + z * zst);
-    float4 acc = make_float4(0.f, 0.f, 0.f, 0.f);
-#pragma unroll
-    for (int z = 0; z < 16; ++z)
-      if (z < ks) add_f4(acc, u[z]);
-    add_f4(v, acc);
-  }
-  float4* d = reinterpret_cast<float4*>(dx + (((long)n * H + th) * W + tw) * C + c);
-  float4 o = *d;
-  add_f4(o, v);
-  *d = o;
-}
-
-__host__ __device__ __forceinline__ int border5_seg_rows(int n_img, int len, int bm) {
-  return (n_img * len + bm - 1) / bm * bm;
-}
-
-__global__ __launch_bounds__(256) void dgrad_border5_add_k(const float* __restrict__ slab, int ks, int Mb, int C,
-                                                           float* __restrict__ dx, int N, int H, int W, int Lt,
-                                                           int Ll) {
-  const int t = threadIdx.x;
-  const int c = blockIdx.y * 64 + (t & 15) * 4;
-  const int T = 2 * W + 2 * H;
-  const int m = blockIdx.x * 16 + (t >> 4);
-  if (m >= N * T || c >= C) return;
-  const int n = m / T, b = m - n * T;
-  int th, tw;
-  if (b < 2 * W) {
-    th = b < W ? 1 : H - 2;
-    tw = b < W ? b : b - W;
+template <bool PL>
+__global__ __launch_bounds__(256) void dgrad_fold_k(const float* __restrict__ dy, const __bf16* __restrict__ apl,
+                                                    long pps, float* __restrict__ fold, __bf16* __restrict__ fpl,
+                                                    long fps, int N, int H, int W, int C) {
+  const int c8n = C >> 3, P = dgrad_fold_pixels(H, W);
+  const long idx = (long)blockIdx.x * 256 + threadIdx.x;
+  if (idx >= (long)N * P * c8n) return;
+  const int c = (int)(idx % c8n) * 8;
+  const long m = idx / c8n;
+  const int n = (int)(m / P), q = (int)(m - (long)n * P);
+  int hs[4], ws[4];
+  const int ns = dgrad_fold_sources(q, H, W, hs, ws);
+  float v[8];
+#pragma unroll
+  for (int k = 0; k < 4; ++k) {
+    if (k >= ns) break;
+    const long e = (((long)n * H + hs[k]) * W + ws[k]) * C + c;
+    float u[8];
+    if constexpr (PL) {
+      const u32x4_t h = *reinterpret_cast<const u32x4_t*>(apl + e), md = *reinterpret_cast<const u32x4_t*>(apl + pps + e),
+                    l = *reinterpret_cast<const u32x4_t*>(apl + 2 * pps + e);
+#pragma unroll
+      for (int i = 0; i < 4; ++i) {
+        u[2 * i] = (__uint_as_float(h[i] << 16) + __uint_as_float(md[i] << 16)) + __uint_as_float(l[i] << 16);
+        u[2 * i + 1] = (__uint_as_float(h[i] & 0xffff0000u) + __uint_as_float(md[i] & 0xffff0000u)) +
+                       __uint_as_float(l[i] & 0xffff0000u);
+      }
+    } else {
+      const float4 a = *reinterpret_cast<const float4*>(dy + e), b = *reinterpret_cast<const float4*>(dy + e + 4);
+      u[0] = a.x; u[1] = a.y; u[2] = a.z; u[3] = a.w;
+      u[4] = b.x; u[5] = b.y; u[6] = b.z; u[7] = b.w;
+    }
+#pragma unroll
+    for (int i = 0; i < 8; ++i) v[i] = k == 0 ? u[i] : v[i] + u[i];
+  }
+  const float4 o0 = make_float4(v[0], v[1], v[2], v[3]), o1 = make_float4(v[4], v[5], v[6], v[7]);
+  const long o = m * C + c;
+  if constexpr (PL) {
+    uint4 pl[3];
+    split8<3>(o0, o1, pl);
+#pragma unroll
+    for (int p = 0; p < 3; ++p) *reinterpret_cast<uint4*>(fpl + p * fps + o) = pl[p];
   } else {
-    const int b2 = b - 2 * W;
-    th = b2 < H ? b2 : b2 - H;
-    tw = b2 < H ? 1 : W - 2;
-    if (th == 1 || th == H - 2) return;
-  }
-  int rows[3];
-  const int nr = dgrad_border_slab_rows(n, th, tw, H, W, Lt, Ll, rows);
-  const long zst = (long)Mb * C;
-  float4 v = make_float4(0.f, 0.f, 0.f, 0.f);
-  for (int r = 0; r < nr; ++r) {
-    const float* base = slab + (long)rows[r] * C + c;
-    float4 u[16];
-#pragma unroll
-    for (int z = 0; z < 16; ++z)
-      if (z < ks) u[z] = *reinterpret_cast<const float4*>(base + z * zst);
-    float4 acc = make_float4(0.f, 0.f, 0.f, 0.f);
-#pragma unroll
-    for (int z = 0; z < 16; ++z)
-      if (z < ks) add_f4(acc, u[z]);
-    add_f4(v, acc);
-  }
-  float4* d = reinterpret_cast<float4*>(dx + (((long)n * H + th) * W + tw) * C + c);
-  float4 o = *d;
-  add_f4(o, v);
-  *d = o;
-}
-
-__device__ __forceinline__ void border5_target(int b, int W, int H, int& th, int& tw, bool& live) {
-  live = true;
-  if (b < 2 * W) {
-    th = b < W ? 1 : H - 2;
-    tw = b < W ? b : b - W;
-  } else {
-    const int b2 = b - 2 * W;
-    th = b2 < H ? b2 : b2 - H;
-    tw = b2 < H ? 1 : W - 2;
-    if (th == 1 || th == H - 2) live = false;
-  }
-}
-
-__global__ __launch_bounds__(256) void dgrad_border5_add_inb_k(const float* __restrict__ slab, int ks, int Mb, int C,
-                                                               float* __restrict__ dx, int H, int W, int Lt, int Ll,
-                                                               InbArgs inb, int first_slice) {
-  __shared__ double red[2][16][65];
-  const int t = threadIdx.x, c4 = (t & 15) * 4, sub = t >> 4;
-  const int c = blockIdx.z * 64 + c4, n = blockIdx.y;
-  const int T = 2 * W + 2 * H;
-  const int b = blockIdx.x * 16 + sub;
-  double a0[4] = {0, 0, 0, 0}, a1[4] = {0, 0, 0, 0};
-  int th = 0, tw = 0;
-  bool live = false;
-  if (b < T && c < C) border5_target(b, W, H, th, tw, live);
-  if (live) {
-    int rows[3];
-    const int nr = dgrad_border_slab_rows(n, th, tw, H, W, Lt, Ll, rows);
-    const long zst = (long)Mb * C;
-    float4 v = make_float4(0.f, 0.f, 0.f, 0.f);
-    for (int r = 0; r < nr; ++r) {
-      const float* base = slab + (long)rows[r] * C + c;
-      float4 u[16];
-#pragma unroll
-      for (int z = 0; z < 16; ++z)
-        if (z < ks) u[z] = *reinterpret_cast<const float4*>(base + z * zst);
-      float4 acc = make_float4(0.f, 0.f, 0.f, 0.f);
-#pragma unroll
-      for (int z = 0; z < 16; ++z)
-        if (z < ks) add_f4(acc, u[z]);
-      add_f4(v, acc);
-    }
-    const long e = (((long)n * H + th) * W + tw) * C + c;
-    float4* d = reinterpret_cast<float4*>(dx + e);
-    const float4 o0 = *d;
-    float4 o = o0;
-    add_f4(o, v);
-    *d = o;
-    const float4 zz = *reinterpret_cast<const float4*>(inb.z + e);
-    const float4 s0 = reinterpret_cast<const float4*>(inb.st)[((long)n * C + c) / 2];
-    const float4 s1 = reinterpret_cast<const float4*>(inb.st)[((long)n * C + c) / 2 + 1];
-    const float mu[4] = {s0.x, s0.z, s1.x, s1.z}, rs[4] = {s0.y, s0.w, s1.y, s1.w};
-    const float g0[4] = {o0.x, o0.y, o0.z, o0.w}, g1[4] = {o.x, o.y, o.z, o.w}, zv[4] = {zz.x, zz.y, zz.z, zz.w};
-#pragma unroll
-    for (int k = 0; k < 4; ++k) {
-      float d0, d1, xh;
-      inb_term(g0[k], zv[k], mu[k], rs[k], inb.act, inb.slope, d0, xh);
-      inb_term(g1[k], zv[k], mu[k], rs[k], inb.act, inb.slope, d1, xh);
-      a0[k] = (double)d1 - (double)d0;
-      a1[k] = (double)d1 * xh - (double)d0 * xh;
-    }
-  }
-#pragma unroll
-  for (int k = 0; k < 4; ++k) {
-    red[0][sub][c4 + k] = a0[k];
-    red[1][sub][c4 + k] = a1[k];
-  }
-  __syncthreads();
-  if (t < 192) {
-    const int v = t >> 6, cc = t & 63, nn = blockIdx.z * 64 + cc;
-    if (nn >= C) return;
-    double acc = 0.0;
-    if (v < 2)
-      for (int q = 0; q < 16; ++q) acc += red[v][q][cc];
-    inb.part[(((long)n * inb.ns + first_slice + blockIdx.x) * C + nn) * 3 + v] = acc;
+    *reinterpret_cast<float4*>(fold + o) = o0;
+    *reinterpret_cast<float4*>(fold + o + 4) = o1;
   }
 }
 
@@ -693,9 +550,10 @@
     float* __restrict__ y, int H, int W, int C, int Ho, int Wo, int Cop, int S, int st, int padh,
     int padw, int reflect, int act, float slope, int M, int Ktot, int m_base, double* __restrict__ part,
     int spk, float* __restrict__ slab, const float* __restrict__ addend, int oph,
-    InbArgs inb = InbArgs{}, const __bf16* __restrict__ apl = nullptr, long pps = 0) {
+    InbArgs inb = InbArgs{}, const __bf16* __restrict__ apl = nullptr, long pps = 0,
+    const void* __restrict__ fold = nullptr, long fps = 0) {
   static_assert(!SPLIT || KSL, "split-K needs the channel-slice-major K walk");
-  static_assert(REFL < 4 || (SPLIT && KSL), "border rows run as split-K slabs");
+  static_assert(REFL != 6 || KSL, "the folded gather walks whole taps");
   __shared__ __attribute__((aligned(16))) char smem[2 * T::STAGE];
   constexpr int A_LD = T::A_LD, B_LD = T::B_LD, RPP = T::RPP, NP = T::NP;
   const int t = threadIdx.x, lane = t & 63, wave = t >> 6;
@@ -708,41 +566,24 @@
   const float* zp = g_zero_page;
 
   constexpr bool C4 = REFL == 3;
-  const int seg = REFL != 5 ? 0 : (m0 < Ho ? 0 : (m0 < 2 * Ho ? 1 : (m0 < 2 * Ho + Wo ? 2 : 3)));
-  const int Sx = REFL != 5 ? S : (seg < 2 ? 3 : 1);
-  int hb[A_LD], wb[A_LD], pb[A_LD], aoff[A_LD], aoff2[C4 ? A_LD : 1];
+  constexpr bool FOLD = REFL == 6;
+  const int FP = FOLD ? dgrad_fold_pixels(H, W) : 0;
+  int hb[A_LD], wb[A_LD], pb[A_LD], fb[FOLD ? A_LD : 1], aoff[A_LD], aoff2[C4 ? A_LD : 1];
 #pragma unroll
   for (int j = 0; j < A_LD; ++j) {
     const int m = m0 + rb + RPP * j;
     const int mm = m < M ? m : 0;
-    if constexpr (REFL == 5) {
-      const int L = seg < 2 ? W + 2 : H;
-      const int r = mm - (seg == 0 ? 0 : (seg == 1 ? Ho : (seg == 2 ? 2 * Ho : 2 * Ho + Wo)));
-      const int n = r / L, k = r - n * L;
-      const bool live = (unsigned)r < (unsigned)(st * L);
-      hb[j] = !live ? -1000000 : (seg == 0 ? 0 : (seg == 1 ? H - 1 : k - 1));
-      wb[j] = seg < 2 ? k - 2 : (seg == 2 ? 0 : W - 1);
-      pb[j] = live ? n * H * W * C : 0;
-      continue;
-    }
-    if constexpr (REFL == 4) {
-      const int n = mm / Wo;
-      int qh, qw, th, tw;
-      dgrad_border_pos(mm - n * Wo, H, W, qh, qw, th, tw);
-      hb[j] = qh - padh;
-      wb[j] = qw - padw;
-      pb[j] = n * H * W * C;
-      continue;
-    }
     const int hw = Ho * Wo;
     const int n = mm / hw, rem = mm - n * hw, ho = rem / Wo, wo = rem - ho * Wo;
     hb[j] = ho * st - padh;
     wb[j] = wo * st - padw;
     pb[j] = n * H * W * C;
+    if constexpr (FOLD) fb[j] = -2 - n * FP * C;
   }
   const bool refl = REFL >= 2 ? reflect != 0 : REFL == 1;
   const int WC = W * C;
   auto tap_rows_to = [&](int* dst, int kr, int ks) __attribute__((always_inline)) {
+    const DgradFoldTap ft = FOLD ? dgrad_fold_tap(kr, ks, H, W) : DgradFoldTap{};
 #pragma unroll
     for (int j = 0; j < A_LD; ++j) {
       int hi = hb[j] + kr, wi = wb[j] + ks;
@@ -752,6 +593,12 @@
         dst[j] = pb[j] + __mul24(hi, WC) + __mul24(wi, C);
       } else {
         const bool ok = (unsigned)hi < (unsigned)H && (unsigned)wi < (unsigned)W;
+        if constexpr (FOLD) {
+          const int q = dgrad_fold_pixel_tap(ft, hb[j] + 1, wb[j] + 1, hi, wi);
+          const int plain = pb[j] + __mul24(hi, WC) + __mul24(wi, C), folded = fb[j] - __mul24(q, C);
+          dst[j] = ok ? (q >= 0 ? folded : plain) : -1;
+          continue;
+        }
         dst[j] = ok ? pb[j] + __mul24(hi, WC) + __mul24(wi, C) : -1;
       }
     }
@@ -767,21 +614,21 @@
 #pragma unroll
   for (int j = 0; j < B_LD; ++j) {
     const int n = n0 + rb + RPP * j;
-    wrow[j] = ws + (long)(n < Cop ? n : Cop - 1) * (REFL == 5 ? 3 * Ktot : Ktot);
+    wrow[j] = ws + (long)(n < Cop ? n : Cop - 1) * Ktot;
   }
 
   const int kq8 = 8 * kq;
   int tr = 0, ts = 0, ksb = 0;
   int kcur = kq8, kc = kq8 % C, kr = 0, ks = 0;
-  const int Rk = KSL ? Ktot / (Sx * C) : 0;
+  const int Rk = KSL ? Ktot / (S * C) : 0;
   const int nk_all = (Ktot + T::BK - 1) / T::BK;
   int k0 = 0, nk = nk_all;
   if (SPLIT) {
     k0 = zs * spk;
     nk = min(spk, nk_all - k0);
-    const int taps = Rk * Sx, tap = k0 % taps;
-    tr = tap / Sx;
-    ts = tap - tr * Sx;
+    const int taps = Rk * S, tap = k0 % taps;
+    tr = tap / S;
+    ts = tap - tr * S;
     ksb = (k0 / taps) * T::BK;
   }
   if (KSL) {
@@ -795,17 +642,15 @@
 
   float4 ra[2][A_LD][2];
   u32x4_t rbv[2][B_LD][NP];
-  constexpr bool GLDS = VST_BF_GLDS_B && T::M16 && KSL && !C4 && REFL != 5;
+  constexpr bool GLDS = VST_BF_GLDS_B && T::M16 && KSL && !C4;
   constexpr bool GLDS_A = (APRE || VST_BF_FAKE_ADMA) && GLDS;
-  constexpr bool APRE_REG = APRE && !GLDS_A;
-  static_assert(!APRE || GLDS_A || REFL == 5, "pre-split A: the x6 M16 channel-slice kernels with LDS-DMA B, or REFL 5");
+  static_assert(!APRE || GLDS_A, "pre-split A: the x6 M16 channel-slice kernels with LDS-DMA B");
   const __bf16* apl_ = VST_BF_FAKE_ADMA ? reinterpret_cast<const __bf16*>(x) : apl;
   const long pps_ = VST_BF_FAKE_ADMA ? (long)(M / (Ho * Wo)) * H * W * C / 2 : pps;
   auto load_all = [&](int set) __attribute__((always_inline)) {
     const bool kin = KSL || kcur < Ktot;
     const int ka = KSL ? ksb + kq8 : kc;
-    const int tap5 = seg == 0 ? 6 + ts : (seg == 1 ? ts : 3 * tr + (seg == 2 ? 2 : 0));
-    const int kb = KSL ? (REFL == 5 ? tap5 : tr * S + ts) * C + ksb + kq8 : (kin ? kcur : 0);
+    const int kb = KSL ? (tr * S + ts) * C + ksb + kq8 : (kin ? kcur : 0);
     if constexpr (C4) {
       const bool kin2 = kcur + 4 < Ktot;
 #pragma unroll
@@ -833,21 +678,13 @@
       if constexpr (GLDS_A) break;
       const bool tap0 = KSL && tr == 0 && ts == 0;
       const bool fake = VST_BF_FAKE_ZA == 1 || (VST_BF_FAKE_ZA == 2 && !tap0) || (VST_BF_FAKE_ZA == 3 && tap0);
-      if constexpr (APRE_REG) {
-        const bool live = kin && aoff[j] >= 0;
-        const __bf16* q = live ? apl + aoff[j] + ka : reinterpret_cast<const __bf16*>(zp);
-        const long ps = live ? pps : 0;
-        const u32x4_t h = *reinterpret_cast<const u32x4_t*>(q), m = *reinterpret_cast<const u32x4_t*>(q + ps),
-                      l = *reinterpret_cast<const u32x4_t*>(q + 2 * ps);
-        float v[8];
-#pragma unroll
-        for (int e = 0; e < 4; ++e) {
-          v[2 * e] = (__uint_as_float(h[e] << 16) + __uint_as_float(m[e] << 16)) + __uint_as_float(l[e] << 16);
-          v[2 * e + 1] = (__uint_as_float(h[e] & 0xffff0000u) + __uint_as_float(m[e] & 0xffff0000u)) +
-                         __uint_as_float(l[e] & 0xffff0000u);
-        }
-        ra[set][j][0] = make_float4(v[0], v[1], v[2], v[3]);
-        ra[set][j][1] = make_float4(v[4], v[5], v[6], v[7]);
+      if constexpr (FOLD) {
+        const int a = aoff[j];
+        const bool fd = a < -1;
+        const float* base = fd ? reinterpret_cast<const float*>(fold) : x;
+        const float* p = a == -1 ? zp : base + (fd ? -2 - a : a) + ka;
+        ra[set][j][0] = *reinterpret_cast<const float4*>(p);
+        ra[set][j][1] = *reinterpret_cast<const float4*>(p + 4);
         continue;
       }
       const float* p = (kin && aoff[j] >= 0 && !fake) ? x + (VST_BF_FAKE_ZA == 4 ? 0 : aoff[j]) + ka : zp;
@@ -872,12 +709,21 @@
         const int row = rb + RPP * j;
         const int csrc = (t % T::KC) ^ T::swz(row);
         const int wrow0 = __builtin_amdgcn_readfirstlane(row - (lane / T::KC));
-        const bool live = aoff[j] >= 0;
+        bool live = aoff[j] >= 0;
         const __bf16* src = live ? apl_ + aoff[j] + ksb + 8 * csrc : zb + 8 * csrc;
+        long ps = pps_;
+        if constexpr (FOLD) {
+          const int a = aoff[j];
+          const bool fd = a < -1;
+          const __bf16* base = fd ? reinterpret_cast<const __bf16*>(fold) : apl_;
+          live = a != -1;
+          src = live ? base + (fd ? -2 - a : a) + ksb + 8 * csrc : zb + 8 * csrc;
+          ps = fd ? fps : pps_;
+        }
 #pragma unroll
         for (int p = 0; p < NP; ++p) {
 #if defined(__HIP_DEVICE_COMPILE__)
-          __builtin_amdgcn_global_load_lds(src + (live ? p * pps_ : 0), (lds_void*)(st + p * T::A_PLANE + wrow0 * T::ROWB),
+          __builtin_amdgcn_global_load_lds(src + (live ? p * ps : 0), (lds_void*)(st + p * T::A_PLANE + wrow0 * T::ROWB),
                                            16, 0, 0);
 #endif
         }
@@ -901,7 +747,7 @@
   auto adv = [&](bool go) __attribute__((always_inline)) {
     if (KSL) {
       const int ts1 = ts + 1;
-      const bool w1 = ts1 == Sx;
+      const bool w1 = ts1 == S;
       const int tr1 = tr + (w1 ? 1 : 0);
       const bool w2 = w1 && tr1 == Rk;
       ts = go ? (w1 ? 0 : ts1) : ts;
@@ -1130,19 +976,20 @@
     float* __restrict__ y, int H, int W, int C, int Ho, int Wo, int Cop, int S, int st, int padh,
     int padw, int reflect, int act, float slope, int M, int Ktot, int m_base, double* __restrict__ part,
     int spk = 0, float* __restrict__ slab = nullptr, const float* __restrict__ addend = nullptr, int oph = 0,
-    const __bf16* __restrict__ apl = nullptr, long pps = 0) {
+    const __bf16* __restrict__ apl = nullptr, long pps = 0, const void* __restrict__ fold = nullptr, long fps = 0) {
   conv_fprop_bf_body<T, KSL, REFL, SPLIT, APRE>(blockIdx.x, x, ws, wps, bias, y, H, W, C, Ho, Wo, Cop, S, st, padh,
                                                 padw, reflect, act, slope, M, Ktot, m_base, part, spk, slab, addend, oph,
-                                                InbArgs{}, apl, pps);
+                                                InbArgs{}, apl, pps, fold, fps);
 }
 
 template <class T, bool APRE = false>
 __global__ __launch_bounds__(T::NT, T::MINB) void conv_fprop_bf_inb_k(
     const float* __restrict__ x, const __bf16* __restrict__ ws, long wps, float* __restrict__ y, int H, int W, int C,
-    int Cop, const float* __restrict__ addend, int M, int Ktot, InbArgs inb, const __bf16* __restrict__ apl = nullptr,
-    long pps = 0) {
-  conv_fprop_bf_body<T, true, 0, false, APRE>(blockIdx.x, x, ws, wps, nullptr, y, H, W, C, H, W, Cop, 3, 1, 1, 1, 0,
-                                              VST_ACT_NONE, 0.f, M, Ktot, 0, nullptr, 0, nullptr, addend, 0, inb, apl, pps);
+    int Cop, const float* __restrict__ addend, int M, int Ktot, InbArgs inb, const void* __restrict__ fold, long fps,
+    const __bf16* __restrict__ apl = nullptr, long pps = 0) {
+  conv_fprop_bf_body<T, true, 6, false, APRE>(blockIdx.x, x, ws, wps, nullptr, y, H, W, C, H, W, Cop, 3, 1, 1, 1, 0,
+                                              VST_ACT_NONE, 0.f, M, Ktot, 0, nullptr, 0, nullptr, addend, 0, inb, apl, pps,
+                                              fold, fps);
 }
 
 struct PhaseJobs {
@@ -1909,7 +1756,7 @@
 int bf_fprop_launch(const float* x, const void* wsplit, long wps, const float* bias, float* y, int N,
                     int H, int W, int C, int Ho, int Wo, int Cop, int R, int S, int st, int padh, int padw,
                     int reflect, int act, float slope, int math, int kind, hipStream_t s, double* part,
-                    float* tws, size_t tws_floats, const float* addend, int oph) {
+                    float* tws, size_t tws_floats, const float* addend, int oph, const float* fold) {
   if (oph) tws = nullptr;
   VST_REQUIRE(!(part && addend), "conv fprop: IN partials together with an addend are not supported");
   const int M = N * Ho * Wo, K = R * S * C;
@@ -1918,6 +1765,18 @@
   const __bf16* ws = reinterpret_cast<const __bf16*>(wsplit);
   int kd, m_split, tail_kind;
   bf_plan(M, Cop, math, kind, &kd, &m_split, &tail_kind);
+  if (fold) {
+    VST_REQUIRE(VST_BF_KSLICE && C % 32 == 0 && R == 3 && S == 3 && st == 1 && padh == 1 && padw == 1 && !reflect &&
+                    Ho == H && Wo == W && !oph && !part,
+                "conv fprop: the folded gather is the 3x3 stride-1 pad-1 data gradient's");
+    auto k32 = [&](int k) {
+      const bool deep = k == 5 || (math != VST_MATH_BF16X6 && (k == 4 || k == 8));
+      return (deep && C % 64) ? (k == 4 ? 0 : (k == 5 ? 1 : 6)) : k;
+    };
+    kd = k32(kd);
+    tail_kind = k32(tail_kind);
+    VST_REQUIRE(kd != 10 && tail_kind != 10, "conv fprop: no folded gather on the 256x64 tile");
+  }
   int ks = 0, m_first = 0;
   if (tws) {
     bf_split_plan(M, Cop, C, R, S, math, kind, &m_first, &ks);
@@ -1935,6 +1794,12 @@
       hipLaunchKernelGGL((bf::conv_fprop_bf_k<T, false, 3>), grid, dim3(T::NT), 0, s, x, ws, wps, bias, y, \
                          H, W, C, Ho, Wo, Cop, S, st, padh, padw, reflect, act, slope, Mend, K, mb, part, 0,      \
                          nullptr, addend, oph);                                                          \
+    else if (fold) {                                                                                \
+      if constexpr (!(BM_ == 256 && BN_ == 64))  \
+        hipLaunchKernelGGL((bf::conv_fprop_bf_k<T, true, 6>), grid, dim3(T::NT), 0, s, x, ws, wps, bias, y, \
+                           H, W, C, Ho, Wo, Cop, S, st, padh, padw, reflect, act, slope, Mend, K, mb, part, 0,    \
+                           nullptr, addend, oph, nullptr, 0, fold, 0);                                   \
+    }                                                                                               \
     else if (VST_BF_KSLICE && C % BK_ == 0 && reflect)                                              \
       hipLaunchKernelGGL((bf::conv_fprop_bf_k<T, true, 1>), grid, dim3(T::NT), 0, s, x, ws, wps, bias, y, \
                          H, W, C, Ho, Wo, Cop, S, st, padh, padw, reflect, act, slope, Mend, K, mb, part, 0,      \
@@ -1955,7 +1820,11 @@
       using T = bf::Tile<256, 128, 64, 64, 32, 3>;
       const int nk = (K + T::BK - 1) / T::BK, spk = (nk + ks - 1) / ks;
       const dim3 grid(ceil_div(M - mb, 256) * ceil_div(Cop, 128) * ks);
-      if (reflect)
+      if (fold)
+        hipLaunchKernelGGL((bf::conv_fprop_bf_k<T, true, 6, true>), grid, dim3(T::NT), 0, s, x, ws, wps, bias, y, H,
+                           W, C, Ho, Wo, Cop, S, st, padh, padw, reflect, act, slope, M, K, mb, part, spk, tws,
+                           nullptr, 0, nullptr, 0, fold, 0);
+      else if (reflect)
         hipLaunchKernelGGL((bf::conv_fprop_bf_k<T, true, 1, true>), grid, dim3(T::NT), 0, s, x, ws, wps, bias, y, H,
                            W, C, Ho, Wo, Cop, S, st, padh, padw, reflect, act, slope, M, K, mb, part, spk, tws,
                            nullptr);
@@ -1978,113 +1847,46 @@
 }
 
 
-static void bf_border_plan(int N, int H, int W, int Cy, int Cx, int math, int* ks_out, long* mb_out) {
-  const int NB = bf::dgrad_border_rows(H, W);
-  const long Mb = (long)N * NB;
-  const int bm = math == VST_MATH_BF16X6 ? 256 : 128;
-  const long tiles = ((Mb + bm - 1) / bm) * ((Cx + 127) / 128);
-  const int nk = (9 * Cy + 31) / 32;
-  int ks = (int)(VST_NUM_CUS / (tiles > 0 ? tiles : 1));
-  ks = ks < 1 ? 1 : (ks > 16 ? 16 : ks);
-  while (ks > 1 && (ks - 1) * ((nk + ks - 1) / ks) >= nk) --ks;
-  *ks_out = ks;
-  *mb_out = Mb;
-}
-
-static constexpr bool g_border5 = true;
-static constexpr int g_border_ks = 0;
-static void bf_border5_plan(int N, int H, int W, int Cy, int Cx, int* ks_out, int* lt, int* ll) {
-  *lt = bf::border5_seg_rows(N, W + 2, 128);
-  *ll = bf::border5_seg_rows(N, H, 128);
-  const long tiles = (long)(2 * *lt + 2 * *ll) / 128 * ((Cx + 127) / 128);
-  const int nk = (3 * Cy + 31) / 32;
-  int ks = g_border_ks > 0 ? g_border_ks : (int)(VST_NUM_CUS / (tiles > 0 ? tiles : 1));
-  if (g_border_ks <= 0 && ks > nk / 4) ks = nk / 4;
-  ks = ks < 1 ? 1 : (ks > 16 ? 16 : ks);
-  while (ks > 1 && (ks - 1) * ((nk + ks - 1) / ks) >= nk) --ks;
-  *ks_out = ks;
-}
-
 bool bf_dgrad_refl1_ok(int N, int H, int W, int Cy, int Cx, int math) {
   return math != VST_MATH_F32 && VST_BF_KSLICE && Cy % 32 == 0 && Cx % 4 == 0 && H >= 4 && W >= 4 && N > 0;
 }
 
-size_t bf_dgrad_refl1_slabs(int N, int H, int W, int Cy, int Cx, int math, BorderSlabs* b) {
-  if (g_border5) {
-    bf_border5_plan(N, H, W, Cy, Cx, &b->ks, &b->Lt, &b->Ll);
-    b->Mb = 2 * b->Lt + 2 * b->Ll;
-  } else {
-    long Mb;
-    bf_border_plan(N, H, W, Cy, Cx, math, &b->ks, &Mb);
-    b->Mb = (int)Mb;
-    b->Lt = bf::dgrad_border_rows(H, W);
-    b->Ll = 0;
-  }
-  return bf_fprop_ws_floats((long)N * H * W, Cx, Cy, 3, 3, math);
+static size_t bf_dgrad_fold_floats(int N, int H, int W, int Cy, bool pl) {
+  const size_t e = (size_t)N * dgrad_fold_pixels(H, W) * Cy;
+  return pl ? e + e / 2 : e;
+}
+
+static void bf_dgrad_fold_launch(const float* dy, const __bf16* apl, long pps, float* fold, int N, int H, int W, int Cy,
+                                 hipStream_t s) {
+  const long e = (long)N * dgrad_fold_pixels(H, W) * Cy;
+  const dim3 grid(ceil_div(e / 8, 256));
+  if (apl)
+    hipLaunchKernelGGL(bf::dgrad_fold_k<true>, grid, dim3(256), 0, s, nullptr, apl, pps, nullptr,
+                       reinterpret_cast<__bf16*>(fold), e, N, H, W, Cy);
+  else
+    hipLaunchKernelGGL(bf::dgrad_fold_k<false>, grid, dim3(256), 0, s, dy, nullptr, 0, fold, nullptr, 0, N, H, W, Cy);
 }
 
 size_t bf_dgrad_refl1_ws_floats(int N, int H, int W, int Cy, int Cx, int math) {
-  int ks, ks5, lt, ll;
-  long Mb;
-  bf_border_plan(N, H, W, Cy, Cx, math, &ks, &Mb);
-  bf_border5_plan(N, H, W, Cy, Cx, &ks5, &lt, &ll);
-  const size_t b4 = (size_t)ks * Mb * Cx, b5 = g_border5 ? (size_t)ks5 * (2 * lt + 2 * ll) * Cx : 0;
-  return bf_fprop_ws_floats((long)N * H * W, Cx, Cy, 3, 3, math) + (b4 > b5 ? b4 : b5);
+  return bf_fprop_ws_floats((long)N * H * W, Cx, Cy, 3, 3, math) + bf_dgrad_fold_floats(N, H, W, Cy, false);
 }
 
 int bf_dgrad_refl1_launch(const float* dy, const void* wsplit, long wps, const float* addend, float* dx, int N, int H,
-                          int W, int Cy, int Cx, int math, hipStream_t s, float* ws, size_t ws_floats, bool add_border) {
-  int ks;
-  long Mb;
-  bf_border_plan(N, H, W, Cy, Cx, math, &ks, &Mb);
+                          int W, int Cy, int Cx, int math, hipStream_t s, float* ws, size_t ws_floats) {
   const size_t main_ws = bf_fprop_ws_floats((long)N * H * W, Cx, Cy, 3, 3, math);
-  VST_REQUIRE(ws_floats >= main_ws + (size_t)ks * Mb * Cx, "dgrad_refl: workspace too small");
+  VST_REQUIRE(ws_floats >= main_ws + bf_dgrad_fold_floats(N, H, W, Cy, false), "dgrad_refl: workspace too small");
+  float* fold = ws + main_ws;
+  bf_dgrad_fold_launch(dy, nullptr, 0, fold, N, H, W, Cy, s);
   if (int e = bf_fprop_launch(dy, wsplit, wps, nullptr, dx, N, H, W, Cy, H, W, Cx, 3, 3, 1, 1, 1, 0, VST_ACT_NONE, 0.f,
-                              math, -1, s, nullptr, main_ws ? ws : nullptr, main_ws, addend))
+                              math, -1, s, nullptr, main_ws ? ws : nullptr, main_ws, addend, 0, fold))
     return e;
-  float* slab = ws + main_ws;
-  const __bf16* wb = reinterpret_cast<const __bf16*>(wsplit);
-  if (g_border5) {
-    int ks5, lt, ll;
-    bf_border5_plan(N, H, W, Cy, Cx, &ks5, &lt, &ll);
-    const int Mt = 2 * lt + 2 * ll, K = 3 * Cy;
-    VST_REQUIRE(ws_floats >= main_ws + (size_t)ks5 * Mt * Cx, "dgrad_refl: workspace too small");
-#define VST_B5(NP_)                                                                                            {                                                                                                             using T = bf::Tile<128, 128, 64, 32, 32, NP_>;                                                              const int nk = (K + T::BK - 1) / T::BK, spk = (nk + ks5 - 1) / ks5;                                         const dim3 grid(Mt / 128 * ceil_div(Cx, 128) * ks5);                                                        hipLaunchKernelGGL((bf::conv_fprop_bf_k<T, true, 5, true>), grid, dim3(T::NT), 0, s, dy, wb, wps, nullptr,                          dx, H, W, Cy, lt, ll, Cx, 3, N, 1, 1, 0, VST_ACT_NONE, 0.f, Mt, K, 0, nullptr, spk,                           slab, nullptr);                                                                        }
-    if (math == VST_MATH_BF16X6)
-      VST_B5(3)
-    else
-      VST_B5(2)
-#undef VST_B5
-    const int T = 2 * W + 2 * H;
-    if (add_border)
-      hipLaunchKernelGGL(bf::dgrad_border5_add_k, dim3(ceil_div((long)N * T, 16), ceil_div(Cx, 64)), dim3(256), 0, s,
-                       slab, ks5, Mt, Cx, dx, N, H, W, lt, ll);
-    return check_launch("conv2d_dgrad_refl");
-  }
-  const int NB = bf::dgrad_border_rows(H, W), K = 9 * Cy;
-  if (math == VST_MATH_BF16X6) {
-    using T = bf::Tile<256, 128, 64, 64, 32, 3>;
-    const int nk = (K + T::BK - 1) / T::BK, spk = (nk + ks - 1) / ks;
-    const dim3 grid(ceil_div(Mb, 256) * ceil_div(Cx, 128) * ks);
-    hipLaunchKernelGGL((bf::conv_fprop_bf_k<T, true, 4, true>), grid, dim3(T::NT), 0, s, dy, wb, wps, nullptr, dx, H,
-                       W, Cy, H, NB, Cx, 3, 1, 1, 1, 0, VST_ACT_NONE, 0.f, (int)Mb, K, 0, nullptr, spk, slab, nullptr);
-  } else {
-    using T = bf::Tile<128, 128, 64, 32, 32, 2>;
-    const int nk = (K + T::BK - 1) / T::BK, spk = (nk + ks - 1) / ks;
-    const dim3 grid(ceil_div(Mb, 128) * ceil_div(Cx, 128) * ks);
-    hipLaunchKernelGGL((bf::conv_fprop_bf_k<T, true, 4, true>), grid, dim3(T::NT), 0, s, dy, wb, wps, nullptr, dx, H,
-                       W, Cy, H, NB, Cx, 3, 1, 1, 1, 0, VST_ACT_NONE, 0.f, (int)Mb, K, 0, nullptr, spk, slab, nullptr);
-  }
-  if (add_border)
-    hipLaunchKernelGGL(bf::dgrad_border_add_k, dim3(ceil_div(Mb, 16), ceil_div(Cx, 64)), dim3(256), 0, s, slab, ks,
-                       (int)Mb, Cx, dx, H, W, NB);
   return check_launch("conv2d_dgrad_refl");
 }
 
-int bf_dgrad_refl1_inb_slices(int H, int W) { return H * W / 32 + (2 * W + 2 * H + 15) / 16; }
+int bf_dgrad_refl1_inb_slices(int H, int W) { return H * W / 32; }
 
 bool bf_dgrad_refl1_inb_ok(int N, int H, int W, int Cy, int Cx, int math) {
-  if (math != VST_MATH_BF16X6 || !g_border5 || !bf_dgrad_refl1_ok(N, H, W, Cy, Cx, math) || (H * W) % 32) return false;
+  if (math != VST_MATH_BF16X6 || !bf_dgrad_refl1_ok(N, H, W, Cy, Cx, math) || (H * W) % 32) return false;
   int kd, m_split, tail_kind, m_first, fks;
   const long M = (long)N * H * W;
   if (M > (1L << 30)) return false;
@@ -2092,6 +1894,10 @@
   bf_split_plan(M, Cx, Cy, 3, 3, math, -1, &m_first, &fks);
   if (fks && !m_first) return true;
   return kd == 7 && (!m_split || (fks && m_first == m_split));
+}
+
+size_t bf_dgrad_refl1_inb_ws_floats(int N, int H, int W, int Cy, int Cx, int math) {
+  return bf_fprop_ws_floats((long)N * H * W, Cx, Cy, 3, 3, math) + bf_dgrad_fold_floats(N, H, W, Cy, true);
 }
 
 int bf_dgrad_refl1_inb_launch(const float* dy, const void* wsplit, long wps, const float* addend, float* dx, int N,
@@ -2104,10 +1910,12 @@
   bf_plan(M, Cx, math, -1, &kd, &m_split, &tail_kind);
   bf_split_plan(M, Cx, Cy, 3, 3, math, -1, &m_first, &fks);
   const size_t main_ws = bf_fprop_ws_floats(M, Cx, Cy, 3, 3, math);
-  int ks5, lt, ll;
-  bf_border5_plan(N, H, W, Cy, Cx, &ks5, &lt, &ll);
-  const int Mt = 2 * lt + 2 * ll, K5 = 3 * Cy, K = 9 * Cy;
-  VST_REQUIRE(ws_floats >= main_ws + (size_t)ks5 * Mt * Cx, "conv2d_dgrad_refl_in_epi: workspace too small");
+  const int K = 9 * Cy;
+  VST_REQUIRE(ws_floats >= main_ws + bf_dgrad_fold_floats(N, H, W, Cy, true),
+              "conv2d_dgrad_refl_in_epi: workspace too small");
+  float* fold = ws + main_ws;
+  const long fps = (long)N * dgrad_fold_pixels(H, W) * Cy;
+  bf_dgrad_fold_launch(dy, apl, pps, fold, N, H, W, Cy, s);
   const bf::InbArgs inb{z, st, part, act, slope, bf_dgrad_refl1_inb_slices(H, W)};
   const __bf16* wb = reinterpret_cast<const __bf16*>(wsplit);
   using T = bf::Tile<256, 128, 64, 64, 32, 3>;
@@ -2116,40 +1924,25 @@
     const dim3 grid(ceil_div(mb, 256) * ceil_div(Cx, 128));
     if (apl)
       hipLaunchKernelGGL((bf::conv_fprop_bf_inb_k<T, true>), grid, dim3(T::NT), 0, s, dy, wb, wps, dx, H, W, Cy, Cx,
-                         addend, (int)mb, K, inb, apl, pps);
+                         addend, (int)mb, K, inb, fold, fps, apl, pps);
     else
       hipLaunchKernelGGL((bf::conv_fprop_bf_inb_k<T>), grid, dim3(T::NT), 0, s, dy, wb, wps, dx, H, W, Cy, Cx, addend,
-                         (int)mb, K, inb);
+                         (int)mb, K, inb, fold, 0);
   }
   if (mb < M) {
     const int nk = (K + T::BK - 1) / T::BK, spk = (nk + fks - 1) / fks;
     const dim3 grid(ceil_div(M - mb, 256) * ceil_div(Cx, 128) * fks);
     if (apl)
-      hipLaunchKernelGGL((bf::conv_fprop_bf_k<T, true, 0, true, true>), grid, dim3(T::NT), 0, s, dy, wb, wps, nullptr, dx,
+      hipLaunchKernelGGL((bf::conv_fprop_bf_k<T, true, 6, true, true>), grid, dim3(T::NT), 0, s, dy, wb, wps, nullptr, dx,
                          H, W, Cy, H, W, Cx, 3, 1, 1, 1, 0, VST_ACT_NONE, 0.f, (int)M, K, (int)mb, nullptr, spk, ws,
-                         nullptr, 0, apl, pps);
+                         nullptr, 0, apl, pps, fold, fps);
     else
-      hipLaunchKernelGGL((bf::conv_fprop_bf_k<T, true, 0, true>), grid, dim3(T::NT), 0, s, dy, wb, wps, nullptr, dx, H,
+      hipLaunchKernelGGL((bf::conv_fprop_bf_k<T, true, 6, true>), grid, dim3(T::NT), 0, s, dy, wb, wps, nullptr, dx, H,
                          W, Cy, H, W, Cx, 3, 1, 1, 1, 0, VST_ACT_NONE, 0.f, (int)M, K, (int)mb, nullptr, spk, ws,
-                         nullptr);
+                         nullptr, 0, nullptr, 0, fold, 0);
     hipLaunchKernelGGL(bf::fprop_splitk_reduce_inb_k, dim3(ceil_div(M - mb, 32), ceil_div(Cx, 64)), dim3(256), 0, s, ws,
                        fks, (int)mb, (int)M, Cx, dx, H * W, addend, inb);
   }
-  float* slab = ws + main_ws;
-  {
-    using T5 = bf::Tile<128, 128, 64, 32, 32, 3>;
-    const int nk = (K5 + T5::BK - 1) / T5::BK, spk = (nk + ks5 - 1) / ks5;
-    const dim3 grid(Mt / 128 * ceil_div(Cx, 128) * ks5);
-    if (apl)
-      hipLaunchKernelGGL((bf::conv_fprop_bf_k<T5, true, 5, true, true>), grid, dim3(T5::NT), 0, s, dy, wb, wps, nullptr,
-                         dx, H, W, Cy, lt, ll, Cx, 3, N, 1, 1, 0, VST_ACT_NONE, 0.f, Mt, K5, 0, nullptr, spk, slab,
-                         nullptr, 0, apl, pps);
-    else
-      hipLaunchKernelGGL((bf::conv_fprop_bf_k<T5, true, 5, true>), grid, dim3(T5::NT), 0, s, dy, wb, wps, nullptr, dx,
-                         H, W, Cy, lt, ll, Cx, 3, N, 1, 1, 0, VST_ACT_NONE, 0.f, Mt, K5, 0, nullptr, spk, slab, nullptr);
-  }
-  hipLaunchKernelGGL(bf::dgrad_border5_add_inb_k, dim3(ceil_div(2 * W + 2 * H, 16), N, ceil_div(Cx, 64)), dim3(256), 0,
-                     s, slab, ks5, Mt, Cx, dx, H, W, lt, ll, inb, H * W / 32);
   return check_launch("conv2d_dgrad_refl_in_epi");
 }
 
@@ -2317,5 +2110,5 @@
     return VST_EUNSUPPORTED;
   }
   return bf_dgrad_refl1_launch(dy, wsplit, (long)Cx * 9 * Cy, addend, dx, N, H, W, Cy, Cx, math, (hipStream_t)stream,
-                               ws, ws_bytes / sizeof(float), true);
-}
+                               ws, ws_bytes / sizeof(float));
+}
diff --git a/gan-based-video-style-transfer_amd/csrc/norm.hip b/gan-based-video-style-transfer_amd/csrc/norm.hip
--- a/gan-based-video-style-transfer_amd/csrc/norm.hip
+++ b/gan-based-video-style-transfer_amd/csrc/norm.hip
@@ -1176,7 +1176,7 @@
 
 extern "C" size_t vst_conv2d_dgrad_refl_in_epi_ws_bytes(int N, int H, int W, int Cy, int Cx, int math) {
   if (Cx % 4 || !bf_dgrad_refl1_inb_ok(N, H, W, Cy, Cx, math)) return 0;
-  return in_epi_ws_bytes_al(N, H, W, Cx) + bf_dgrad_refl1_ws_floats(N, H, W, Cy, Cx, math) * sizeof(float);
+  return in_epi_ws_bytes_al(N, H, W, Cx) + bf_dgrad_refl1_inb_ws_floats(N, H, W, Cy, Cx, math) * sizeof(float);
 }
 
 extern "C" int vst_conv2d_dgrad_refl_epi_part(const float* dy, const void* dy_apl, const void* wsplit,
```

Result: no change. 80.17 frames/s (median of 6 runs) (+0.9%).
